# halismai/bpvo

Measured on AMD Instinct MI355X. Metric: GN iterations/s (1241x376 bit-planes 8ch, 4 levels, Tukey; linearise + solve + update = 1, the reference's _num_fun_evals), higher is better.
Workload: dtype f32 (+f64 projection/interpolation); 1 GPU; batch of 1024 independent 1241x376 stereo pairs (1024 per GPU), bitplanes descriptor, 4 pyramid levels, tukey loss, converge with AlgorithmParameters() tolerances; pairs_per_gpu=1024

## Files before the change

bpvo_amd/csrc/context.hip:

```cpp
#include "host_ctx.h"

using namespace bpvo_hip;
using namespace bpvo_hip_host;

namespace bpvo_hip_host {

std::atomic<int> g_live_ctx[64];
thread_local std::string g_create_error;

int fail(bpvo_hip_ctx* c, int code, const char* msg)
{
  c->err = msg;
  return code;
}


void gaussian_kernel5(double sigma, float k[3])
{
  float kk[5];
  const double sigmaX = sigma > 0 ? sigma : ((5 - 1) * 0.5 - 1) * 0.3 + 0.8;
  const double scale2X = -0.5 / (sigmaX * sigmaX);
  double sum = 0;
  for(int i = 0; i < 5; ++i) {
    const double x = i - 2.0;
    kk[i] = (float) std::exp(scale2X * x * x);
    sum += kk[i];
  }
  sum = 1. / sum;
  for(int i = 0; i < 5; ++i) kk[i] = (float) (kk[i] * sum);
  k[0] = kk[2]; k[1] = kk[3]; k[2] = kk[4];
}

void gaussian_taps(int n, double sigma, GaussTaps* g)
{
  *g = GaussTaps();
  if(!(sigma > 0) || n <= 0 || n > kMaxGaussTaps) return;
  g->n = n;
  const double scale2X = -0.5 / (sigma * sigma);
  double sum = 0;
  for(int i = 0; i < n; ++i) {
    const double x = i - (n - 1) * 0.5;
    g->k[i] = (float) std::exp(scale2X * x * x);
    sum += g->k[i];
  }
  sum = 1. / sum;
  for(int i = 0; i < n; ++i) {
    g->k[i] = (float) (g->k[i] * sum);
    g->ki[i] = (int) std::nearbyint((double) g->k[i] * 256.0);
  }
}
int imsmooth_taps(float sigma) { return std::max(5, 2 * (int) std::round((double) sigma) + 1); }
int auto_gauss_taps_f32(float sigma) { return ((int) std::nearbyint((double) sigma * 8.0 + 1.0)) | 1; }

void carve_frame_data(bpvo_hip_ctx* c, FrameSlot& f, unsigned char* base, size_t* total)
{
  Carver cv{base};
  for(int l = 0; l < c->L; ++l) f.img[l] = cv.take<uint8_t>(c->geom[l].npix);
  f.disp = cv.take<float>(c->geom[0].npix);
  for(int l = 0; l < c->L; ++l) f.desc[l] = cv.take<float>(c->geom[l].npix * c->C);
  for(int l = 0; l < c->L; ++l) f.cen[l] = (c->C == 8) ? cv.take<uint8_t>(c->geom[l].npix) : nullptr;
  for(int l = 0; l < c->L; ++l) f.ch0[l] = (c->C == 8) ? cv.take<float>(c->geom[l].npix) : nullptr;
  f.scratch = c->plane_scratch ? cv.take<float>((size_t) c->scratch_planes * c->geom[0].npix) : nullptr;
  if(total) *total = cv.off;
}

void carve_frame_tmpl(bpvo_hip_ctx* c, FrameSlot& f, unsigned char* base, size_t* total)
{
  Carver cv{base};
  for(int l = 0; l < c->L; ++l) {
    const LevelGeom& g = c->geom[l];
    f.sal[l] = cv.take<float>(g.npix);
    const size_t nwords = (size_t) g.rows * ((g.cols + 63) / 64);
    f.flag[l] = (uint8_t*) cv.take<unsigned long long>((std::max(g.npix, nwords * 8) + 7) / 8);
    f.blk_count[l] = cv.take<int>(std::max((size_t) g.nblk, nwords));
    f.pts[l] = cv.take<float4>(g.cap);
    f.ptc[l] = cv.take<float2>(g.cap);
    f.inds[l] = cv.take<int>(g.cap);
    f.pix[l] = cv.take<float>((size_t) g.cap * c->C);
    f.grad[l] = cv.take<float>((size_t) g.cap * c->C * 2);
  }
  f.nrm = cv.take<float>(4 * kMaxLevels);
  f.n_dev = cv.take<int>(kMaxLevels);
  if(total) *total = cv.off;
}

int ensure_template_storage(bpvo_hip_ctx* c, FrameSlot& f)
{
  if(f.tmpl_slab) return BPVO_OK;
  size_t total = 0;
  FrameSlot tmp;
  carve_frame_tmpl(c, tmp, nullptr, &total);
  HIP_CK(c, hipMalloc(&f.tmpl_slab, total));
  HIP_CK(c, hipMemsetAsync(f.tmpl_slab, 0, total, c->stream));
  carve_frame_tmpl(c, f, (unsigned char*) f.tmpl_slab, nullptr);
  return BPVO_OK;
}

FrameJob make_frame_job(bpvo_hip_ctx* c, FrameSlot& f, int l)
{
  const LevelGeom& g = slot_geom(c, f, l);
  FrameJob j;
  std::memset(&j, 0, sizeof(j));
  j.img = f.img[l];
  j.cen = f.cen[l];
  j.ch0 = f.ch0_valid ? f.ch0[l] : nullptr;
  j.scratch = f.scratch;
  j.desc = f.desc[l];
  j.sal = f.sal[l];
  j.flag = f.flag[l];
  j.words = reinterpret_cast<unsigned long long*>(f.flag[l]);
  j.blk_count = f.blk_count[l];
  j.n_out = f.n_dev ? f.n_dev + l : nullptr;
  j.disp = f.disp;
  j.pts = f.pts[l];
  j.ptc = f.ptc[l];
  j.inds = f.inds[l];
  j.pix = f.pix[l];
  j.grad = f.grad[l];
  j.nrm = f.nrm ? f.nrm + 4 * l : nullptr;
  j.rows = g.rows; j.cols = g.cols; j.level = l; j.disp_cols = slot_geom(c, f, 0).cols;
  j.cap = g.cap;
  j.nms_radius = g.nms_radius;
  std::memcpy(j.K, g.K, sizeof(j.K));
  j.b = g.b;
  j.dspace = c->dspace;
  j.lazy = f.lazy[l] ? 1 : 0;
  const bpvo_hip_params& sp = f.seq_params ? *f.seq_params : c->params;
  j.min_saliency = sp.minSaliency; j.min_disp = sp.minValidDisparity; j.max_disp = sp.maxValidDisparity;
  return j;
}

PairJob make_pair_job(bpvo_hip_ctx* c, int ws, int ref, int cur, int l)
{
  FrameSlot& fr = c->frames[ref];
  FrameSlot& fc = c->frames[cur];
  const LevelGeom& g = slot_geom(c, fr, l);
  PairJob j;
  std::memset(&j, 0, sizeof(j));
  j.pts = fr.pts[l];
  j.ptc = fr.ptc[l];
  j.pix = fr.pix[l];
  j.grad = fr.grad[l];
  j.nrm = fr.nrm + 4 * l;
  j.n = fr.n_host[l];
  j.desc = fc.desc[l];
  j.rows = g.rows; j.cols = g.cols;
  std::memcpy(j.K, g.K, sizeof(j.K));
  j.b = g.b;
  j.f_inv[0] = 1.0f / g.K[0]; j.f_inv[1] = 1.0f / g.K[4];
  j.dspace = c->dspace;
  j.r = c->ws[ws].r;
  j.valid = c->ws[ws].valid;
  j.cand = c->ws[ws].cand;
  j.tapkey = c->ws[ws].tapkey;
  j.tapcache_on = c->ws[ws].tapkey != nullptr;
  j.tapcache = c->ws[ws].tapcache;
  j.med_blk = c->ws[ws].med_blk;
  j.partials = c->ws[ws].partials;
  j.st = c->d_states + ws;
  j.cnt = c->d_counters + kWsCounters * (size_t) ws;
  j.ticket = c->d_tickets + ws;
  if(ws == c->trace_ws) { j.trace = c->d_trace; j.trace_cap = c->trace_cap; }
  j.pitch = c->C;
  j.n_groups = c->G;
  j.med_tot = (int) med_totals_at(c);
  pair_job_set_params(j, c->params);
  return j;
}
void pair_job_set_params(PairJob& j, const bpvo_hip_params& p)
{
  j.prm = GNParams{p.maxIterations, kMaxFunEvals, p.parameterTolerance, p.functionTolerance, p.gradientTolerance};
  j.loss = p.lossFunction;
  j.good_thr = p.goodPointThreshold;
}

PairJob group_pair_job(const bpvo_hip_ctx* c, const PairJob& whole, int k)
{
  PairJob j = whole;
  const size_t off = (size_t) k * c->Cg;
  const size_t nblk = (size_t) ((whole.n + kChunkPoints - 1) / kChunkPoints);
  const size_t ntiles = (size_t) std::max(1, (whole.n + gn_pts_per_block(c->Cg) - 1) / gn_pts_per_block(c->Cg));
  j.desc = whole.desc.get() + off;
  j.pix = whole.pix.get() + off;
  j.grad = whole.grad.get() + off;
  j.r = whole.r.get() + off;
  j.cand = whole.cand.get() + (size_t) k * nblk * kChunkPoints * c->Cg;
  j.med_blk = whole.med_blk.get() + (size_t) k * nblk * 4;
  j.partials = whole.partials.get() + (size_t) k * ntiles * kPartialStride;
  j.n_groups = 1;
  return j;
}

hipEvent_t take_event(Lane* ln)
{
  if(!ln->ev_pool.empty()) {
    hipEvent_t e = ln->ev_pool.back();
    ln->ev_pool.pop_back();
    return e;
  }
  hipEvent_t e;
  (void) hipEventCreate(&e);
  return e;
}
void resolve_events(bpvo_hip_ctx* c)
{
  for(auto& ln : c->lanes) {
    for(auto& ep : ln.ev_pending) {
      float ms = 0.0f;
      if(hipEventElapsedTime(&ms, ep.a, ep.b) == hipSuccess) {
        c->kc_ms[ep.kc] += ms;
        c->kc_units[ep.kc] += ep.units;
        c->kc_launches[ep.kc] += 1;
      }
      ln.ev_pool.push_back(ep.a);
      ln.ev_pool.push_back(ep.b);
    }
    ln.ev_pending.clear();
  }
}

int lanes_for(bpvo_hip_ctx* c, int n, int cap)
{
  if(g_live_ctx[c->device & 63].load() > 1) return 1;
  const int want = std::max(1, std::min(std::min(c->max_lanes_now, cap), n / kMinPairsPerLane));
  if(want > (int) c->lanes.size()) {
    const int rc = ensure_lanes(c, want);
    if(rc) return rc;
  }
  return want;
}
int ensure_lanes(bpvo_hip_ctx* c, int n)
{
  const int n_pairs = c->n_pairs;
  while((int) c->lanes.size() < n) {
    c->lanes.emplace_back();
    Lane& ln = c->lanes.back();
    const bool first = c->lanes.size() == 1;
    if(first) { ln.stream = c->stream; ln.owns_stream = false; }
    else { HIP_CK(c, hipStreamCreateWithFlags(&ln.stream, hipStreamNonBlocking)); ln.owns_stream = true; }
    HIP_CK(c, hipMalloc((void**) &ln.d_pjobs, sizeof(PairJob) * (size_t) c->L * n_pairs * job_tables(c)));
    HIP_CK(c, hipMalloc((void**) &ln.d_Tinit, sizeof(float) * 16 * n_pairs));
    HIP_CK(c, hipMalloc((void**) &ln.d_active, 8 * sizeof(int)));
    HIP_CK(c, hipMalloc((void**) &ln.d_list, 3 * sizeof(int) * (size_t) n_pairs));
    for(auto& e : ln.round_ev) HIP_CK(c, hipEventCreateWithFlags(&e, hipEventDisableTiming));
    HIP_CK(c, hipEventCreateWithFlags(&ln.selected_ev, hipEventDisableTiming));
    for(auto& e : ln.staging_ev) HIP_CK(c, hipEventCreateWithFlags(&e, hipEventDisableTiming));
    HIP_CK(c, hipHostMalloc((void**) &ln.h_pjobs, sizeof(PairJob) * std::max((size_t) c->L * n_pairs * job_tables(c), (size_t) (1 + kMaxGroups))));
    HIP_CK(c, hipHostMalloc((void**) &ln.h_T, sizeof(float) * 16 * n_pairs));
    HIP_CK(c, hipHostMalloc((void**) &ln.h_active, 8 * sizeof(int)));
    HIP_CK(c, hipMalloc((void**) &ln.d_pk_ctl, sizeof(unsigned) * kPkCtlWords * kMaxLevels));
    HIP_CK(c, hipHostMalloc((void**) &ln.h_pk_ctl, sizeof(unsigned) * kPkCtlWords * kMaxLevels));
    if(first) {
      HIP_CK(c, hipMalloc((void**) &ln.d_team_ctl, sizeof(unsigned) * (size_t) gn_team_ctl_words(kMaxTeams)));
      HIP_CK(c, hipHostMalloc((void**) &ln.h_team_ctl, sizeof(unsigned) * 64));
      std::memset(ln.h_team_ctl, 0, sizeof(unsigned) * 64);
    }
    HIP_CK(c, hipHostMalloc((void**) &ln.h_states, sizeof(GNState) * (n_pairs + n_pairs)));
  }
  return BPVO_OK;
}

const std::vector<OptionDef>& option_table()
{
#define OPT_INT(key_, field_, lo_, hi_) OptionDef{key_, lo_, hi_, [](bpvo_hip_ctx* c) { return (double) c->field_; }, \
                                                  [](bpvo_hip_ctx* c, double v) { c->field_ = (decltype(c->field_)) v; return BPVO_OK; }}
  static const std::vector<OptionDef> t = {
    OptionDef{"lanes", 1, 8, [](bpvo_hip_ctx* c) { return (double) std::max(1, std::min(c->max_lanes_now, std::max(1, c->n_pairs / kMinPairsPerLane))); },
              [](bpvo_hip_ctx* c, double v) {
                const int n = std::max(1, std::min((int) v, std::max(1, c->n_pairs / kMinPairsPerLane)));
                const int rc = ensure_lanes(c, n);
                if(rc == BPVO_OK) c->max_lanes_now = (int) v;
                return rc;
              }},
    OptionDef{"persistent", 0, 1, [](bpvo_hip_ctx* c) { return (double) c->persistent; },
              [](bpvo_hip_ctx* c, double v) { c->persistent = (int) v; if(c->persistent) c->persistent_failed.store(false); return BPVO_OK; }},
    OPT_INT("persist_max_ws", persist_max_ws, 1, kPersistMaxWs),
    OPT_INT("persist_grid", persist_grid, 1, 128),
    OPT_INT("persist_max_points", persist_max_points, 0, 1 << 30),
    OPT_INT("dense_candidates_from", dense_candidates_from, 0, 1 << 30),
    OPT_INT("persist_timeout_ticks", persist_timeout, 1, 1e15),
    OPT_INT("team", team_mode, 0, 1),
    OPT_INT("team_max_pairs", team_max_pairs, 0, 1 << 20),
    OPT_INT("team_full_pairs", team_full_pairs, 0, 1 << 20),
    OPT_INT("team_size", team_size_env, 0, 256),
    OptionDef{"team_cus", 1, 1 << 16, [](bpvo_hip_ctx* c) { return (double) c->num_cus; },
              [](bpvo_hip_ctx* c, double v) {
                if(c->device_cus > 0 && (int) v > c->device_cus) { c->err = "option team_cus: more CUs than the device has"; return BPVO_ERR_INVALID_ARG; }
                c->num_cus = (int) v;
                return BPVO_OK;
              }},
    OPT_INT("team_local_barriers", team_local_barriers, 0, 1),
    OPT_INT("team_join", team_join, 0, 2),
    OptionDef{"team_joins_seen", 0, 0, [](bpvo_hip_ctx* c) { return (double) c->team_joins.load(); },
              [](bpvo_hip_ctx* c, double) { c->team_joins.store(0); return BPVO_OK; }},
    OPT_INT("team_join_from_pairs", team_join_from_pairs, 0, 1 << 20),
    OPT_INT("team_spares", team_spares, 0, 1),
    OPT_INT("vo_disparity_late", vo_disparity_late, 0, 1),
    OPT_INT("stereo_frames_per_launch", stereo_frames_per_launch, 0, 65535),
    OptionDef{"stereo_frames_per_launch_seen", 0, 0, [](bpvo_hip_ctx* c) { return (double) c->st_frames_per_launch_seen; }, [](bpvo_hip_ctx*, double) { return BPVO_OK; }},
    OptionDef{"stereo_free_mib_seen", 0, 0, [](bpvo_hip_ctx* c) { return (double) (c->st_free_seen >> 20); }, [](bpvo_hip_ctx*, double) { return BPVO_OK; }},
    OPT_INT("normalization_side_stream", nrm_side_stream, 0, 1),
    OPT_INT("normalization_form", nrm_dpp_asm, 0, 4),
    OPT_INT("small_batch_fused", small_batch_fused, 0, 1),
    OPT_INT("levels_in_one_launch_max_frames", merge_levels_max_frames, 0, 1 << 20),
    OPT_INT("normalization_deferred", nrm_defer, 0, 1),
    OPT_INT("team_split_max_pairs", team_split_max_pairs, 0, 1 << 20),
    OPT_INT("fuse_frozen", fuse_frozen, 0, 1),
    OPT_INT("reference_reduction", reference_reduction, 0, 1),
    OPT_INT("step_in_reduce_max_pairs", step_in_reduce_max, 0, 1 << 20),
    OPT_INT("stagger", stagger, 0, 1),
    OPT_INT("stagger_min_pairs", stagger_min_pairs, 0, 1 << 20),
    OPT_INT("upload_workers", up_workers, 0, 32),
    OPT_INT("keep_current_disparity", keep_current_disparity, 0, 1),
    OptionDef{"pose_covariance", 0, 1, [](bpvo_hip_ctx* c) { return (double) c->pose_covariance; },
              [](bpvo_hip_ctx* c, double v) -> int {
                if((int) v) {
                  const int rc = pose_cov_ensure_scratch(c);
                  if(rc) return rc;
                }
                c->pose_covariance = (int) v;
                return BPVO_OK;
              }},
    OPT_INT("lazy_template_descriptor", lazy_template, 0, 1),
    OPT_INT("points_from_compact_stream", points_from_compact, 0, 1),
    OptionDef{"tapcache_max_density", 0.0, 1e9, [](bpvo_hip_ctx* c) { return c->tapcache_max_density; },
              [](bpvo_hip_ctx* c, double v) { c->tapcache_max_density = v; return BPVO_OK; }},
    OptionDef{"upload_plan_first", 0.0, 0.9, [](bpvo_hip_ctx* c) { return c->up_plan[0]; },
              [](bpvo_hip_ctx* c, double v) { if(v + c->up_plan[1] >= 1.0) return BPVO_ERR_INVALID_ARG; c->up_plan[0] = v; return BPVO_OK; }},
    OptionDef{"upload_plan_second", 0.01, 0.99, [](bpvo_hip_ctx* c) { return c->up_plan[1]; },
              [](bpvo_hip_ctx* c, double v) { if(v + c->up_plan[0] >= 1.0) return BPVO_ERR_INVALID_ARG; c->up_plan[1] = v; return BPVO_OK; }},
  };
#undef OPT_INT
  return t;
}
int set_option(bpvo_hip_ctx* c, const std::string& key, double v)
{
  for(const OptionDef& o : option_table())
    if(key == o.key) {
      if(!(v >= o.lo && v <= o.hi)) { c->err = "option " + key + ": value out of range"; return BPVO_ERR_INVALID_ARG; }
      const int rc = o.set(c, v);
      if(rc == BPVO_ERR_INVALID_ARG) c->err = "option " + key + ": invalid value";
      return rc;
    }
  c->err = "unknown option: " + key;
  return BPVO_ERR_INVALID_ARG;
}
int apply_options_string(bpvo_hip_ctx* c, const char* str)
{
  std::string s(str);
  size_t i = 0;
  while(i < s.size()) {
    size_t j = s.find(',', i);
    if(j == std::string::npos) j = s.size();
    const std::string kv = s.substr(i, j - i);
    i = j + 1;
    if(kv.empty()) continue;
    const size_t eq = kv.find('=');
    if(eq == std::string::npos) { c->err = "expected key=value: " + kv; return BPVO_ERR_INVALID_ARG; }
    char* end = nullptr;
    const double v = std::strtod(kv.c_str() + eq + 1, &end);
    if(end == kv.c_str() + eq + 1) { c->err = "not a number: " + kv; return BPVO_ERR_INVALID_ARG; }
    const int rc = set_option(c, kv.substr(0, eq), v);
    if(rc) return rc;
  }
  return BPVO_OK;
}

}

extern "C" {

void bpvo_hip_default_params(bpvo_hip_params* p)
{
  p->numPyramidLevels = -1;
  p->minImageDimensionForPyramid = 40;
  p->sigmaPriorToCensusTransform = -1.0f;
  p->sigmaBitPlanes = 0.5f;
  p->dfSigma1 = 0.75f;
  p->dfSigma2 = 1.75f;
  p->latchNumBytes = 1;
  p->latchRotationInvariance = 0;
  p->latchHalfSsdSize = 1;
  p->centralDifferenceRadius = 3;
  p->centralDifferenceSigmaBefore = 0.75f;
  p->centralDifferenceSigmaAfter = 1.75f;
  p->laplacianKernelSize = 1;
  p->maxIterations = 50;
  p->parameterTolerance = 1e-7f;
  p->functionTolerance = 1e-6f;
  p->gradientTolerance = 1e-8f;
  p->relaxTolerancesForCoarseLevels = 1;
  p->gradientEstimation = BPVO_GRAD_CD3;
  p->interp = BPVO_INTERP_LINEAR;
  p->lossFunction = BPVO_LOSS_TUKEY;
  p->descriptor = BPVO_DESC_INTENSITY;
  p->verbosity = BPVO_VERB_ITERATION;
  p->minTranslationMagToKeyFrame = 0.15f;
  p->minRotationMagToKeyFrame = 5.0f;
  p->maxFractionOfGoodPointsToKeyFrame = 0.6f;
  p->goodPointThreshold = 0.85f;
  p->minNumPixelsForNonMaximaSuppression = 320 * 240;
  p->nonMaxSuppRadius = 1;
  p->minNumPixelsToWork = 256;
  p->minSaliency = 0.1f;
  p->minValidDisparity = 0.001f;
  p->maxValidDisparity = 512.0f;
  p->maxTestLevel = 0;
  p->withNormalization = 1;
}

}

namespace bpvo_hip_host {

const char* level_geometry(const float K[9], float baseline, int rows, int cols, int L, const bpvo_hip_params& p, LevelGeom* geom)
{
  int r = rows, w = cols;
  float Kp[9];
  std::memcpy(Kp, K, sizeof(Kp));
  float bp = baseline;
  for(int l = 0; l < L; ++l) {
    if(l > 0) {
      r = (r + 1) / 2; w = (w + 1) / 2;
      for(int k = 0; k < 9; ++k) Kp[k] *= 0.5f;
      Kp[8] = 1.0f;
      bp *= 2.0f;
    }
    LevelGeom& g = geom[l];
    g.rows = r; g.cols = w; g.npix = (size_t) r * w;
    g.nblk = (int) ((g.npix + 255) / 256);
    const bool nms = (r * w >= p.minNumPixelsForNonMaximaSuppression) && p.nonMaxSuppRadius > 0;
    g.nms_radius = nms ? p.nonMaxSuppRadius : -1;
    const size_t cap = nms ? (size_t) ((r + 1) / 2) * ((w + 1) / 2) : g.npix;
    g.cap = (int) ((cap + kTile - 1) / kTile * kTile);
    std::memcpy(g.K, Kp, sizeof(Kp));
    g.b = bp;
    if(r < 8 || w < 8) return "pyramid level smaller than 8 pixels";
  }
  return nullptr;
}

int create_impl(bpvo_hip_ctx** out, const float K[9], float baseline, int rows, int cols, const bpvo_hip_params* p, int device, int n_frames, int n_pairs,
                const int* min_caps)
{
  if(!out || !K || !p || rows < 8 || cols < 8 || n_frames < 1 || n_pairs < 1) {
    g_create_error = "invalid argument";
    return BPVO_ERR_INVALID_ARG;
  }
  if(rows > 65535 || cols > 65535 || (long long) rows * cols * 8 > 0x7fffffffLL) {
    g_create_error = "image too large (at most 65535 x 65535 and 2^28 pixels)";
    return BPVO_ERR_INVALID_ARG;
  }
  int ndev = 0;
  if(hipGetDeviceCount(&ndev) != hipSuccess || ndev <= 0) {
    g_create_error = "no HIP device: libbpvo_hip has no CPU fallback";
    return BPVO_ERR_NO_DEVICE;
  }
  if(device < 0 || device >= ndev) {
    g_create_error = "bad device ordinal";
    return BPVO_ERR_INVALID_ARG;
  }
  std::unique_ptr<bpvo_hip_ctx> c(new bpvo_hip_ctx);
  pose_cov_none(&c->vo_cov);
  c->params = *p;
  std::memcpy(c->K, K, sizeof(c->K));
  c->baseline = baseline;
  c->rows = rows; c->cols = cols; c->device = device;
  c->n_frames = n_frames; c->n_pairs = n_pairs;
  c->auto_levels = c->params.numPyramidLevels <= 0;
  if(c->params.numPyramidLevels <= 0)
    c->params.numPyramidLevels = auto_pyramid_levels(rows, cols, p->minImageDimensionForPyramid);
  c->L = c->params.numPyramidLevels;
  auto unsupported = [&](const char* m) { g_create_error = m; return BPVO_ERR_UNSUPPORTED; };
  if(c->L < 1 || c->L > kMaxLevels) return unsupported("numPyramidLevels out of range (1..8)");
  if(c->params.maxTestLevel < 0 || c->params.maxTestLevel >= c->L) { g_create_error = "invalid maxTestLevel"; return BPVO_ERR_INVALID_ARG; }
  const bool desc_fields = c->params.descriptor == BPVO_DESC_FIELDS_FIRST_ORDER || c->params.descriptor == BPVO_DESC_FIELDS_SECOND_ORDER;
// ... 278 lines not shown
```

bpvo_amd/csrc/frame_common.h:

```cpp
#pragma once
#include "kernels.h"

namespace bpvo_hip {

__device__ __forceinline__ int reflect101(int p, int len)
{
  if(p < 0) p = -p;
  if(p >= len) p = 2 * len - 2 - p;
  if(p < 0) p = 0;
  return p;
}

__device__ __forceinline__ int reflect101_wide(int p, int len)
{
  if(len == 1) return 0;
  while(p < 0 || p >= len) p = p < 0 ? -p : 2 * len - 2 - p;
  return p;
}

static inline dim3 grid2d(int W, int R, int nz) { return dim3((W + 63) / 64, (R + 3) / 4, nz); }

}
```

bpvo_amd/csrc/frames.hip:

```cpp
#include "host_ctx.h"

using namespace bpvo_hip;
using namespace bpvo_hip_host;

namespace bpvo_hip_host {

FrameRun ctx_run(bpvo_hip_ctx* c) { return FrameRun{c->stream, &c->lanes[0], 0, false, nullptr, nullptr}; }

int upload_frame_jobs_slots(bpvo_hip_ctx* c, const int* slots, int count, const FrameRun& fr, int which, const FrameJob** tab)
{
  const size_t table = (size_t) which * c->L * c->n_frames;
  FR_CK(c, fr, hipEventSynchronize(fr.ln->staging_ev[which]));
  for(int l = 0; l < c->L; ++l) {
    FrameJob* row = c->h_fjobs + table + (size_t) l * c->n_frames + fr.tab;
    for(int i = 0; i < count; ++i) row[i] = make_frame_job(c, c->frames[slots[i]], l);
  }
  const size_t pitch = sizeof(FrameJob) * (size_t) c->n_frames;
  static_assert(sizeof(FrameJob) % 8 == 0 && sizeof(PairJob) % 8 == 0, "copy_rows_kernel moves 8-byte words");
  if(c->ctl_by_kernel.load() || count <= 512)
    launch_copy_rows(fr.stream, c->d_fjobs + table + fr.tab, c->h_fjobs + table + fr.tab, pitch, sizeof(FrameJob) * (size_t) count, c->L);
  else
    FR_CK(c, fr, hipMemcpy2DAsync(c->d_fjobs + table + fr.tab, pitch, c->h_fjobs + table + fr.tab, pitch, sizeof(FrameJob) * (size_t) count, (size_t) c->L,
                                  hipMemcpyHostToDevice, fr.stream));
  FR_CK(c, fr, hipEventRecord(fr.ln->staging_ev[which], fr.stream));
  *tab = c->d_fjobs + table + fr.tab;
  return BPVO_OK;
}
std::vector<int> strided_slots(int first, int stride, int count)
{
  std::vector<int> v((size_t) std::max(count, 0));
  for(int i = 0; i < count; ++i) v[i] = first + i * stride;
  return v;
}
int upload_frame_jobs(bpvo_hip_ctx* c, int first, int stride, int count, const FrameRun& fr, int which, const FrameJob** tab)
{
  const std::vector<int> slots = strided_slots(first, stride, count);
  return upload_frame_jobs_slots(c, slots.data(), count, fr, which, tab);
}

int frames_set_data_slots(bpvo_hip_ctx* c, const int* slots, int count, const uint8_t* images, const float* disps, bool on_device,
                          const FrameRun& fr, int skip_odd_disp, const size_t* offsets)
{
  if(count <= 0) return BPVO_OK;
  const LevelGeom* geom = c->frames[slots[0]].own_geom ? c->frames[slots[0]].geom : c->geom;
  for(int i = 1; i < count; ++i)
    if(slot_geom(c, c->frames[slots[i]], 0).rows != geom[0].rows || slot_geom(c, c->frames[slots[i]], 0).cols != geom[0].cols)
      return fail(c, BPVO_ERR_INVALID_ARG, "frame stage over slots of different sizes");
  const size_t npix = geom[0].npix;
  hipStream_t s = fr.stream;
  if(!on_device) {
    for(int i = 0; i < count; ++i) {
      FrameSlot& f = c->frames[slots[i]];
      const size_t at = offsets ? offsets[i] : (size_t) i * npix;
      FR_CK(c, fr, hipMemcpyAsync(f.img[0], images + at, npix, hipMemcpyHostToDevice, s));
      if(!(skip_odd_disp && (i & 1)) && !fr.skip_disparity_upload)
        FR_CK(c, fr, hipMemcpyAsync(f.disp, disps + at, npix * sizeof(float), hipMemcpyHostToDevice, s));
    }
  }
  for(int i = 0; i < count; ++i) c->frames[slots[i]].ch0_valid = !(skip_odd_disp && (i & 1));
  const bool lazy_ok = skip_odd_disp != 0 && c->lazy_template && c->params.descriptor == BPVO_DESC_BITPLANES && c->C == 8 &&
                       !(c->params.sigmaPriorToCensusTransform > 0.0f) && c->params.sigmaBitPlanes > 0.0f && c->params.gradientEstimation == BPVO_GRAD_CD3;
  for(int i = 0; i < count; ++i)
    for(int l = 0; l < c->L; ++l) c->frames[slots[i]].lazy[l] = lazy_ok && !(i & 1) && geom[l].nms_radius > 0;
  const FrameJob* tab = nullptr;
  int rc = upload_frame_jobs_slots(c, slots, count, fr, 0, &tab);
  if(rc) return rc;
  const int NF = c->n_frames;
  if(on_device && offsets) {
    size_t* h_off = c->h_seq_off + fr.tab;
    for(int i = 0; i < count; ++i) h_off[i] = offsets[i];
    FR_CK(c, fr, hipMemcpyAsync(c->d_seq_off + fr.tab, h_off, sizeof(size_t) * (size_t) count, hipMemcpyHostToDevice, s));
    launch_ingest_at(s, tab, images, disps, c->d_seq_off + fr.tab, npix, count);
  } else if(on_device) {
    launch_ingest(s, tab, images, disps, npix, count, skip_odd_disp);
  }
  {
    double px = 0;
    for(int l = 1; l < c->L; ++l) px += (double) geom[l].npix * count;
    ScopedTimer t(c, KC_PYRAMID, px, fr.ln);
    bool grouped = count <= c->merge_levels_max_frames;
    for(int l = 0; l < c->L; ++l) grouped = grouped && geom[l].cols >= 8 && geom[l].rows >= 8;
    for(int l = 1; l < c->L;) {
      const int steps = grouped ? std::min(3, c->L - l) : 0;
      if(steps >= 2) {
        launch_pyramid_levels(s, tab + (size_t) (l - 1) * NF, NF, steps, geom[l + steps - 1].cols, geom[l + steps - 1].rows, count);
        l += steps;
      } else {
        launch_pyrdown(s, tab + (size_t) (l - 1) * NF, tab + (size_t) l * NF, geom[l].cols, geom[l].rows, count);
        l += 1;
      }
    }
  }
  {
    double px = 0;
    for(int l = c->L - 1; l >= c->params.maxTestLevel; --l) px += (double) geom[l].npix * count;
    ScopedTimer t(c, KC_DESCRIPTOR, px, fr.ln);
    const bool fused_bp = c->C == 8 && c->params.descriptor == BPVO_DESC_BITPLANES && !(c->params.sigmaPriorToCensusTransform > 0.0f) && c->params.sigmaBitPlanes > 0.0f;
    const int l_lo = c->params.maxTestLevel;
    const bool smoothed_bp = c->C == 8 && c->params.descriptor == BPVO_DESC_BITPLANES && c->params.sigmaPriorToCensusTransform > 0.0f && c->params.sigmaBitPlanes > 0.0f;
    const bool plain_intensity = c->C == 1 && c->params.descriptor != BPVO_DESC_LAPLACIAN;
    const bool one_launch = (fused_bp || smoothed_bp || plain_intensity) && count <= c->merge_levels_max_frames && c->L - l_lo > 1;
    if(one_launch && fused_bp) {
      launch_bitplanes(s, tab + (size_t) l_lo * NF, geom[l_lo].cols, geom[l_lo].rows, count, c->params.sigmaBitPlanes, c->gauss_k, 1, c->L - l_lo, NF);
    } else if(one_launch && smoothed_bp) {
      launch_census(s, tab + (size_t) l_lo * NF, geom[l_lo].cols, geom[l_lo].rows, count, c->census_taps, c->L - l_lo, NF);
      launch_bitplanes(s, tab + (size_t) l_lo * NF, geom[l_lo].cols, geom[l_lo].rows, count, c->params.sigmaBitPlanes, c->gauss_k, 0, c->L - l_lo, NF);
    } else if(one_launch) {
      launch_intensity(s, tab + (size_t) l_lo * NF, geom[l_lo].cols, geom[l_lo].rows, count, c->L - l_lo, NF);
    }
    for(int l = c->L - 1; l >= c->params.maxTestLevel && !one_launch; --l) {
      const FrameJob* jobs = tab + (size_t) l * NF;
      const LevelGeom& g = geom[l];
      if(c->params.descriptor == BPVO_DESC_CENTRAL_DIFFERENCE) {
        launch_central_difference(s, jobs, g.cols, g.rows, count, c->params.centralDifferenceRadius, c->cd_before, c->cd_after);
      } else if(c->params.descriptor == BPVO_DESC_LATCH) {
        launch_latch(s, jobs, g.cols, g.rows, count, c->params.latchNumBytes, c->params.latchHalfSsdSize, c->d_latch_off, c->latch_taps[0], c->latch_taps[1],
                     c->latch_after);
      } else if(c->C == 5 || c->C == 10) {
        launch_descriptor_fields(s, jobs, g.cols, g.rows, count, c->C == 10, c->df_g1, c->df_g2);
      } else if(c->C == 3) {
        launch_gradient_descriptor(s, jobs, g.cols, g.rows, count, c->grad_pre);
      } else if(c->C == 1) {
        if(c->params.descriptor == BPVO_DESC_LAPLACIAN) launch_laplacian(s, jobs, g.cols, g.rows, count, c->params.laplacianKernelSize);
        else launch_intensity(s, jobs, g.cols, g.rows, count);
      } else {
        const bool fused_census = !(c->params.sigmaPriorToCensusTransform > 0.0f) && c->params.sigmaBitPlanes > 0.0f;
        if(!fused_census)
          launch_census(s, jobs, g.cols, g.rows, count, c->params.sigmaPriorToCensusTransform > 0.0f ? c->census_taps : nullptr);
        launch_bitplanes(s, jobs, g.cols, g.rows, count, c->params.sigmaBitPlanes, c->gauss_k, fused_census ? 1 : 0);
      }
    }
  }
  FR_CK(c, fr, hipGetLastError());
  for(int i = 0; i < count; ++i) {
    FrameSlot& f = c->frames[slots[i]];
    f.has_data = true;
    f.has_disp = !(skip_odd_disp && (i & 1));
  }
  return BPVO_OK;
}
int frames_set_data(bpvo_hip_ctx* c, int first, int stride, int count, const uint8_t* images, const float* disps, bool on_device,
                    const FrameRun& fr, int skip_odd_disp)
{
  const std::vector<int> slots = strided_slots(first, stride, count);
  return frames_set_data_slots(c, slots.data(), count, images, disps, on_device, fr, skip_odd_disp);
}
int upload_disparity(bpvo_hip_ctx* c, int slot, const float* disparity)
{
  if(!c->copy_stream) {
    HIP_CK(c, hipStreamCreateWithFlags(&c->copy_stream, hipStreamNonBlocking));
    HIP_CK(c, hipEventCreateWithFlags(&c->copy_ev, hipEventDisableTiming));
  }
  HIP_CK(c, hipMemcpyAsync(c->frames[slot].disp, disparity, slot_geom(c, c->frames[slot], 0).npix * sizeof(float), hipMemcpyHostToDevice, c->copy_stream));
  HIP_CK(c, hipEventRecord(c->copy_ev, c->copy_stream));
  HIP_CK(c, hipStreamWaitEvent(c->stream, c->copy_ev, 0));
  return BPVO_OK;
}
int frames_set_data(bpvo_hip_ctx* c, int first, int stride, int count, const uint8_t* images, const float* disps, bool on_device, int skip_odd_disp)
{
  if(count <= 0) return BPVO_OK;
  if(first < 0 || stride < 1 || first + (count - 1) * stride >= c->n_frames) return fail(c, BPVO_ERR_INVALID_ARG, "bad frame slot range");
  if(!images || !disps) return fail(c, BPVO_ERR_INVALID_ARG, "nullptr image/disparity");
  return frames_set_data(c, first, stride, count, images, disps, on_device, ctx_run(c), skip_odd_disp);
}

int frames_set_template_slots(bpvo_hip_ctx* c, const int* slots, int count, const FrameRun& fr)
{
  if(count <= 0) return BPVO_OK;
  const LevelGeom* geom = c->frames[slots[0]].own_geom ? c->frames[slots[0]].geom : c->geom;
  for(int i = 1; i < count; ++i)
    if(slot_geom(c, c->frames[slots[i]], 0).rows != geom[0].rows || slot_geom(c, c->frames[slots[i]], 0).cols != geom[0].cols)
      return fail(c, BPVO_ERR_INVALID_ARG, "frame stage over slots of different sizes");
  hipStream_t s = fr.stream;
  for(int i = 0; i < count; ++i) {
    FrameSlot& f = c->frames[slots[i]];
    if(f.tmpl_slab) continue;
    size_t total = 0;
    FrameSlot tmp;
    carve_frame_tmpl(c, tmp, nullptr, &total);
    FR_CK(c, fr, hipMalloc(&f.tmpl_slab, total));
    FR_CK(c, fr, hipMemsetAsync(f.tmpl_slab, 0, total, s));
    carve_frame_tmpl(c, f, (unsigned char*) f.tmpl_slab, nullptr);
  }
  const FrameJob* tab = nullptr;
  int rc = upload_frame_jobs_slots(c, slots, count, fr, 1, &tab);
  if(rc) return rc;
  const int NF = c->n_frames;
  int* const h_ints = c->h_ints + (size_t) fr.tab * kMaxLevels;
  int* const d_ints = c->d_ints + (size_t) fr.tab * kMaxLevels;
  const bpvo_hip_params& p = c->params;
  const int border = std::max(p.nonMaxSuppRadius, 3);
  bool tiled = true;
  for(int l = p.maxTestLevel; l < c->L; ++l) tiled = tiled && geom[l].nms_radius <= 1;
  const bool one_launch = tiled && count <= c->merge_levels_max_frames && c->L - p.maxTestLevel > 1;
  hipEvent_t counts_ev = fr.ln ? fr.ln->round_ev[0] : nullptr;
  hipStream_t side = nullptr;
  if(c->nrm_side_stream && !fr.own_thread && fr.ln == &c->lanes[0] && counts_ev) {
    if(!c->side_stream) {
      FR_CK(c, fr, hipStreamCreateWithFlags(&c->side_stream, hipStreamNonBlocking));
      FR_CK(c, fr, hipStreamCreateWithFlags(&c->side_stream2, hipStreamNonBlocking));
      for(auto& e : c->side_ev) FR_CK(c, fr, hipEventCreateWithFlags(&e, hipEventDisableTiming));
    }
    side = c->side_stream;
  }
  const int with_nrm = c->dspace ? 0 : p.withNormalization;
  const bool defer = side && fr.defer_finest_nrm && c->nrm_defer && c->L - p.maxTestLevel > 1 && !c->nrm_pending && !c->nrm_pending_finest;
  if(one_launch) {
    double px = 0;
    for(int l = p.maxTestLevel; l < c->L; ++l) px += (double) geom[l].npix * count;
    ScopedTimer t(c, KC_SALIENCY_SELECT, px, fr.ln);
    const LevelGeom& g = geom[p.maxTestLevel];
    launch_saliency_select(s, tab + (size_t) p.maxTestLevel * NF, c->C, g.cols, g.rows, count, 1, border,
                           c->L - p.maxTestLevel, NF);
  }
  for(int l = c->L - 1; l >= p.maxTestLevel && !one_launch; --l) {
    const FrameJob* jobs = tab + (size_t) l * NF;
    const LevelGeom& g = geom[l];
    ScopedTimer t(c, KC_SALIENCY_SELECT, (double) g.npix * count, fr.ln);
    launch_saliency_select(s, jobs, c->C, g.cols, g.rows, count, g.nms_radius, border);
  }
  if(side) {
    FR_CK(c, fr, hipEventRecord(c->side_ev[0], s));
    FR_CK(c, fr, hipStreamWaitEvent(side, c->side_ev[0], 0));
    if(defer && templates_may_be_dense(c)) {
      hipStream_t side2 = c->side_stream2;
      FR_CK(c, fr, hipStreamWaitEvent(side2, c->side_ev[0], 0));
      { ScopedTimer t(c, KC_NORMALIZATION, 0.0, fr.ln, true, side2); launch_normalization(side2, tab, NF, count, p.maxTestLevel, p.maxTestLevel + 1, with_nrm, c->nrm_dpp_asm); }
      FR_CK(c, fr, hipEventRecord(c->side_ev[3], side2));
      c->nrm_pending_finest = c->side_ev[3];
      { ScopedTimer t(c, KC_NORMALIZATION, 0.0, fr.ln, true, side); launch_normalization(side, tab, NF, count, c->L - 1, c->L, with_nrm, c->nrm_dpp_asm); }
      FR_CK(c, fr, hipEventRecord(c->side_ev[1], side));
      if(c->L - 1 > p.maxTestLevel + 1) {
        { ScopedTimer t(c, KC_NORMALIZATION, 0.0, fr.ln, true, side); launch_normalization(side, tab, NF, count, p.maxTestLevel + 1, c->L - 1, with_nrm, c->nrm_dpp_asm); }
        FR_CK(c, fr, hipEventRecord(c->side_ev[2], side));
        c->nrm_pending = c->side_ev[2];
      }
    } else if(defer) {
      { ScopedTimer t(c, KC_NORMALIZATION, 0.0, fr.ln, true, side); launch_normalization(side, tab, NF, count, c->L - 1, c->L, with_nrm, c->nrm_dpp_asm); }
      FR_CK(c, fr, hipEventRecord(c->side_ev[1], side));
      { ScopedTimer t(c, KC_NORMALIZATION, 0.0, fr.ln, true, side); launch_normalization(side, tab, NF, count, p.maxTestLevel, c->L - 1, with_nrm, c->nrm_dpp_asm); }
      FR_CK(c, fr, hipEventRecord(c->side_ev[2], side));
      c->nrm_pending = c->side_ev[2];
    } else {
      { ScopedTimer t(c, KC_NORMALIZATION, 0.0, fr.ln, true, side); launch_normalization(side, tab, NF, count, p.maxTestLevel, c->L, with_nrm, c->nrm_dpp_asm); }
      FR_CK(c, fr, hipEventRecord(c->side_ev[1], side));
    }
  }
  launch_gather_counts(s, tab, NF, count, p.maxTestLevel, c->L, d_ints);
  FR_CK(c, fr, hipMemcpyAsync(h_ints, d_ints, sizeof(int) * kMaxLevels * (size_t) count, hipMemcpyDeviceToHost, s));
  if(counts_ev) FR_CK(c, fr, hipEventRecord(counts_ev, s));
  if(fr.selected_ev) FR_CK(c, fr, hipEventRecord(fr.selected_ev, s));
  if(fr.on_selected) fr.on_selected();
  if(!side) {
    ScopedTimer t(c, KC_NORMALIZATION, 0.0, fr.ln);
    launch_normalization(s, tab, NF, count, p.maxTestLevel, c->L, with_nrm, c->nrm_dpp_asm);
  }
  if(counts_ev) FR_CK(c, fr, hipEventSynchronize(counts_ev));
  else FR_CK(c, fr, hipStreamSynchronize(s));
  std::vector<int> max_n(c->L, 0);
  double pts = 0;
  for(int i = 0; i < count; ++i) {
    FrameSlot& f = c->frames[slots[i]];
    for(int l = 0; l < c->L; ++l) {
      f.n_host[l] = (l >= p.maxTestLevel) ? h_ints[(size_t) i * kMaxLevels + l] : 0;
      max_n[l] = std::max(max_n[l], f.n_host[l]);
      pts += f.n_host[l];
    }
  }
  if(c->profiling) {
    std::lock_guard<std::mutex> lk(c->units_mu);
    c->kc_units[KC_TEMPLATE] += pts;
    c->kc_units[KC_NORMALIZATION] += pts;
  }
  if(count <= c->merge_levels_max_frames && c->L - p.maxTestLevel > 1) {
    ScopedTimer t(c, KC_TEMPLATE, 0.0, fr.ln);
    int most = 0;
    for(int l = p.maxTestLevel; l < c->L; ++l) most = std::max(most, max_n[l]);
    launch_template_build(s, tab + (size_t) p.maxTestLevel * NF, c->C, most, count, p.gradientEstimation == BPVO_GRAD_CD5, c->gauss_k, c->L - p.maxTestLevel, NF);
  } else {
    for(int l = c->L - 1; l >= p.maxTestLevel; --l) {
      ScopedTimer t(c, KC_TEMPLATE, 0.0, fr.ln);
      launch_template_build(s, tab + (size_t) l * NF, c->C, max_n[l], count, p.gradientEstimation == BPVO_GRAD_CD5, c->gauss_k);
    }
  }
  if(side) FR_CK(c, fr, hipStreamWaitEvent(s, c->side_ev[1], 0));
  if(!fr.own_thread && !fr.no_final_sync) {
    FR_CK(c, fr, hipStreamSynchronize(s));
    FR_CK(c, fr, hipGetLastError());
    resolve_events(c);
  }
  for(int i = 0; i < count; ++i) c->frames[slots[i]].has_template = true;
  return BPVO_OK;
}
int frames_set_template(bpvo_hip_ctx* c, int first, int stride, int count, const FrameRun& fr)
{
  const std::vector<int> slots = strided_slots(first, stride, count);
  return frames_set_template_slots(c, slots.data(), count, fr);
}
int frames_set_template(bpvo_hip_ctx* c, int first, int stride, int count)
{
  if(count <= 0) return BPVO_OK;
  if(first < 0 || stride < 1 || first + (count - 1) * stride >= c->n_frames) return fail(c, BPVO_ERR_INVALID_ARG, "bad frame slot range");
  for(int i = 0; i < count; ++i) {
    if(!c->frames[first + i * stride].has_data) return fail(c, BPVO_ERR_NO_DATA, "no data in frame");
    if(!c->frames[first + i * stride].has_disp) return fail(c, BPVO_ERR_NO_DATA, "no disparity in frame (the current frame of a pair batch)");
  }
  return frames_set_template(c, first, stride, count, ctx_run(c));
}

int ensure_dense_descriptor(bpvo_hip_ctx* c, int slot)
{
  FrameSlot& f = c->frames[slot];
  bool any = false;
  for(int l = 0; l < c->L; ++l) any = any || f.lazy[l];
  if(!any) return BPVO_OK;
  bool was[kMaxLevels];
  for(int l = 0; l < c->L; ++l) { was[l] = f.lazy[l]; f.lazy[l] = false; }
  auto restore = [&]() { for(int l = 0; l < c->L; ++l) f.lazy[l] = was[l]; };
  const FrameRun fr = ctx_run(c);
  const FrameJob* tab = nullptr;
  const int rc = upload_frame_jobs(c, slot, 1, 1, fr, 0, &tab);
  if(rc) { restore(); return rc; }
  for(int l = c->L - 1; l >= c->params.maxTestLevel; --l)
    launch_bitplanes(c->stream, tab + (size_t) l * c->n_frames, c->geom[l].cols, c->geom[l].rows, 1, c->params.sigmaBitPlanes, c->gauss_k, 1);
  if(hipGetLastError() != hipSuccess || hipStreamSynchronize(c->stream) != hipSuccess) {
    restore();
    return fail(c, BPVO_ERR_DEVICE, "ensure_dense_descriptor: descriptor kernels failed");
  }
  return BPVO_OK;
}

}

extern "C" {

int bpvo_hip_frame_set_data(bpvo_hip_ctx* c, int slot, const uint8_t* image, const float* disparity)
{
  CHECK_CTX(c); CHECK_SLOT(c, slot);
  (void) hipSetDevice(c->device);
  int rc = frames_set_data(c, slot, 1, 1, image, disparity, false);
  if(rc) return rc;
  HIP_CK(c, hipStreamSynchronize(c->stream));
  resolve_events(c);
  return BPVO_OK;
}
int bpvo_hip_frame_set_data_device(bpvo_hip_ctx* c, int slot, const uint8_t* d_image, const float* d_disparity)
{
  CHECK_CTX(c); CHECK_SLOT(c, slot);
  (void) hipSetDevice(c->device);
  int rc = frames_set_data(c, slot, 1, 1, d_image, d_disparity, true);
  if(rc) return rc;
  HIP_CK(c, hipStreamSynchronize(c->stream));
  resolve_events(c);
  return BPVO_OK;
}
int bpvo_hip_frames_set_data(bpvo_hip_ctx* c, int first_slot, int slot_stride, int count, const uint8_t* images,
                             const float* disparities, int on_device)
{
  CHECK_CTX(c);
  (void) hipSetDevice(c->device);
  int rc = frames_set_data(c, first_slot, slot_stride, count, images, disparities, on_device != 0);
  if(rc) return rc;
  HIP_CK(c, hipStreamSynchronize(c->stream));
  resolve_events(c);
  return BPVO_OK;
}
int bpvo_hip_frame_set_template(bpvo_hip_ctx* c, int slot)
{
  CHECK_CTX(c); CHECK_SLOT(c, slot);
  (void) hipSetDevice(c->device);
  return frames_set_template(c, slot, 1, 1);
}
int bpvo_hip_frames_set_template(bpvo_hip_ctx* c, int first_slot, int slot_stride, int count)
{
  CHECK_CTX(c);
  (void) hipSetDevice(c->device);
  return frames_set_template(c, first_slot, slot_stride, count);
}
int bpvo_hip_frame_clear(bpvo_hip_ctx* c, int slot)
{
  CHECK_CTX(c); CHECK_SLOT(c, slot);
  c->frames[slot].has_data = false;
  c->frames[slot].has_template = false;
  return BPVO_OK;
}
int bpvo_hip_frame_state(const bpvo_hip_ctx* c, int slot, int* has_data, int* has_template)
{
  if(!c || slot < 0 || slot >= c->n_frames) return BPVO_ERR_INVALID_ARG;
  *has_data = c->frames[slot].has_data;
  *has_template = c->frames[slot].has_template;
  return BPVO_OK;
}

int bpvo_hip_get_image(bpvo_hip_ctx* c, int slot, int level, uint8_t* out)
{
  CHECK_CTX(c); CHECK_SLOT(c, slot);
  if(level < 0 || level >= c->L) return fail(c, BPVO_ERR_INVALID_ARG, "bad level");
  if(!c->frames[slot].has_data) return fail(c, BPVO_ERR_NO_DATA, "no data in frame");
  (void) hipSetDevice(c->device);
  HIP_CK(c, hipMemcpyAsync(out, c->frames[slot].img[level], c->geom[level].npix, hipMemcpyDeviceToHost, c->stream));
  HIP_CK(c, hipStreamSynchronize(c->stream));
  return BPVO_OK;
}
int bpvo_hip_get_descriptor_channel(bpvo_hip_ctx* c, int slot, int level, int channel, float* out)
{
  CHECK_CTX(c); CHECK_SLOT(c, slot); CHECK_LEVEL(c, level);
  if(channel < 0 || channel >= c->C) return fail(c, BPVO_ERR_INVALID_ARG, "bad channel");
  if(!c->frames[slot].has_data) return fail(c, BPVO_ERR_NO_DATA, "no data in frame");
  (void) hipSetDevice(c->device);
  if(int rc = ensure_dense_descriptor(c, slot)) return rc;
  const size_t npix = c->geom[level].npix;
  HIP_CK(c, hipMemcpy2DAsync(out, sizeof(float), c->frames[slot].desc[level] + channel, sizeof(float) * c->C, sizeof(float), npix,
                             hipMemcpyDeviceToHost, c->stream));
  HIP_CK(c, hipStreamSynchronize(c->stream));
  return BPVO_OK;
}
int bpvo_hip_get_saliency(bpvo_hip_ctx* c, int slot, int level, float* out)
{
  CHECK_CTX(c); CHECK_SLOT(c, slot); CHECK_LEVEL(c, level);
  if(!c->frames[slot].has_template) return fail(c, BPVO_ERR_NO_TEMPLATE, "no template");
  (void) hipSetDevice(c->device);
  HIP_CK(c, hipMemcpyAsync(out, c->frames[slot].sal[level], c->geom[level].npix * sizeof(float), hipMemcpyDeviceToHost, c->stream));
  HIP_CK(c, hipStreamSynchronize(c->stream));
  return BPVO_OK;
}
#define TMPL(c, slot, level)                                                                    \
  CHECK_CTX(c); CHECK_SLOT(c, slot); CHECK_LEVEL(c, level);                                     \
  if(!(c)->frames[slot].has_template) return fail(c, BPVO_ERR_NO_TEMPLATE, "no template");      \
  (void) hipSetDevice((c)->device);                                                             \
  FrameSlot& f = (c)->frames[slot];                                                             \
  const int n = f.n_host[level]

int bpvo_hip_num_points(bpvo_hip_ctx* c, int slot, int level, int* n_out) { TMPL(c, slot, level); *n_out = n; return BPVO_OK; }
int bpvo_hip_get_points(bpvo_hip_ctx* c, int slot, int level, float* xyzw)
{
  TMPL(c, slot, level);
  if(n && c->points_from_compact) {
    float4* d_out = nullptr;
    HIP_CK(c, hipMalloc((void**) &d_out, sizeof(float4) * n));
    launch_rebuild_points(c->stream, make_pair_job(c, 0, slot, slot, level), d_out);
    hipError_t e = hipMemcpyAsync(xyzw, d_out, sizeof(float4) * n, hipMemcpyDeviceToHost, c->stream);
    if(e == hipSuccess) e = hipStreamSynchronize(c->stream);
    (void) hipFree(d_out);
    HIP_CK(c, e);
    return BPVO_OK;
  }
  if(n) HIP_CK(c, hipMemcpyAsync(xyzw, f.pts[level], sizeof(float4) * n, hipMemcpyDeviceToHost, c->stream));
  HIP_CK(c, hipStreamSynchronize(c->stream));
  return BPVO_OK;
}
int bpvo_hip_get_point_indices(bpvo_hip_ctx* c, int slot, int level, int* inds)
{
  TMPL(c, slot, level);
  if(n) HIP_CK(c, hipMemcpyAsync(inds, f.inds[level], sizeof(int) * n, hipMemcpyDeviceToHost, c->stream));
  HIP_CK(c, hipStreamSynchronize(c->stream));
  return BPVO_OK;
}
int bpvo_hip_get_pixels(bpvo_hip_ctx* c, int slot, int level, float* pixels)
{
  TMPL(c, slot, level);
  const int C = c->C;
  std::vector<float> t(tiled_floats(n, C));
  if(n) HIP_CK(c, hipMemcpyAsync(t.data(), f.pix[level], t.size() * sizeof(float), hipMemcpyDeviceToHost, c->stream));
  HIP_CK(c, hipStreamSynchronize(c->stream));
  detile_to_channel_major(t.data(), n, C, 1, C == 8 ? 4 : C, pixels);
  return BPVO_OK;
}
int bpvo_hip_get_jacobians(bpvo_hip_ctx* c, int slot, int level, float* J)
{
  TMPL(c, slot, level);
  if(n == 0) return BPVO_OK;
  const size_t bytes = sizeof(float) * 6 * (size_t) n * c->C;
  float* d_out = nullptr;
  HIP_CK(c, hipMalloc((void**) &d_out, bytes));
  HIP_CK(c, hipStreamSynchronize(c->stream));
  c->h_fjobs[0] = make_frame_job(c, f, level);
  hipError_t e = hipMemcpyAsync(c->d_fjobs, c->h_fjobs, sizeof(FrameJob), hipMemcpyHostToDevice, c->stream);
  if(e == hipSuccess) {
    launch_export_jacobians(c->stream, c->d_fjobs, c->C, n, d_out);
    e = hipMemcpyAsync(J, d_out, bytes, hipMemcpyDeviceToHost, c->stream);
  }
  if(e == hipSuccess) e = hipStreamSynchronize(c->stream);
  (void) hipFree(d_out);
  HIP_CK(c, e);
  return BPVO_OK;
}
int bpvo_hip_get_normalization(bpvo_hip_ctx* c, int slot, int level, float T[16], float T_inv[16])
{
  TMPL(c, slot, level);
  M44 t = m44_identity(), ti = m44_identity();
  if(!c->params.withNormalization || c->dspace || n == 0) {
    std::memcpy(T, t.m, 64);
    std::memcpy(T_inv, ti.m, 64);
    return BPVO_OK;
  }
  float nrm[4];
  HIP_CK(c, hipMemcpyAsync(nrm, f.nrm + 4 * level, sizeof(nrm), hipMemcpyDeviceToHost, c->stream));
  HIP_CK(c, hipStreamSynchronize(c->stream));
  t.m[0] = t.m[5] = t.m[10] = nrm[0];
  t.m[3] = -nrm[0] * nrm[1]; t.m[7] = -nrm[0] * nrm[2]; t.m[11] = -nrm[0] * nrm[3];
  ti.m[0] = ti.m[5] = ti.m[10] = 1.0f / nrm[0];
  ti.m[3] = nrm[1]; ti.m[7] = nrm[2]; ti.m[11] = nrm[3];
  std::memcpy(T, t.m, 64);
  std::memcpy(T_inv, ti.m, 64);
  return BPVO_OK;
}

}
```

bpvo_amd/csrc/host_ctx.h:

```cpp
#pragma once
#include <hip/hip_runtime.h>

#include <algorithm>
#include <atomic>
#include <chrono>
#include <cmath>
#include <cstdio>
#include <cstdlib>
#include <cstring>
#include <functional>
#include <condition_variable>
#include <memory>
#include <mutex>
#include <string>
#include <thread>
#include <vector>

#include "kernels.h"
#include "latch_table.h"
#include "rig_math.h"
#include "vo_state.h"

using namespace bpvo_hip;
#include "latch_table.h"

namespace bpvo_hip_host {

using namespace bpvo_hip;


extern std::atomic<int> g_live_ctx[64];
extern thread_local std::string g_create_error;

struct LevelGeom {
  int rows, cols;
  size_t npix;
  int nblk;
  int cap;
  int nms_radius;
  float K[9];
  float b;
};

struct FrameSlot {
  bool has_data = false, has_template = false;
  bool has_disp = false;
  void* data_slab = nullptr;
  void* tmpl_slab = nullptr;
  uint8_t* img[kMaxLevels] = {};
  uint8_t* cen[kMaxLevels] = {};
  float* ch0[kMaxLevels] = {};
  bool lazy[kMaxLevels] = {};
  bool ch0_valid = true;
  float* desc[kMaxLevels] = {};
  float* disp = nullptr;
  float* scratch = nullptr;
  float* sal[kMaxLevels] = {};
  uint8_t* flag[kMaxLevels] = {};
  int* blk_count[kMaxLevels] = {};
  float4* pts[kMaxLevels] = {};
  float2* ptc[kMaxLevels] = {};
  int* inds[kMaxLevels] = {};
  float* pix[kMaxLevels] = {};
  float* grad[kMaxLevels] = {};
  float* nrm = nullptr;
  int* n_dev = nullptr;
  int n_host[kMaxLevels] = {};
  bool own_geom = false;
  LevelGeom geom[kMaxLevels];
  const bpvo_hip_params* seq_params = nullptr;
};

struct Workspace {
  float* r = nullptr;
  uint8_t* valid = nullptr;
  uint32_t* cand = nullptr;
  uint32_t* med_blk = nullptr;
  uint32_t* tapkey = nullptr;
  float* tapcache = nullptr;
  float* partials = nullptr;
  int last_ref = -1, last_cur = -1, last_level = -1;
  bool has_estimate = false;
};

struct CovScratch {
  int group = 0;
  void* d_slab = nullptr;
  float* d_r = nullptr; size_t r_floats = 0;
  uint8_t* d_valid = nullptr; size_t valid_bytes = 0;
  float* d_partials = nullptr; size_t partial_floats = 0;
  unsigned long long* d_cnt = nullptr;
  GNState* d_states = nullptr;
  unsigned char* d_tables = nullptr;
  unsigned char* h_tables = nullptr;
  size_t tables_bytes = 0, off_members = 0, off_T = 0, off_sigma = 0, off_X = 0;
  bpvo_hip_pose_covariance* d_out = nullptr;
  bpvo_hip_pose_covariance* h_out = nullptr;
  float* d_sums = nullptr;
};

enum KernelClass { KC_PYRAMID = 0, KC_DESCRIPTOR, KC_SALIENCY_SELECT, KC_NORMALIZATION, KC_TEMPLATE, KC_WARP_RESIDUAL, KC_MEDIAN,
                   KC_IRLS_REDUCE, KC_GN_STEP, KC_COUNT };
static const char* const kKernelNames[KC_COUNT] = {"pyramid", "descriptor", "saliency_select", "normalization", "template_build", "warp_residual",
                                      "median", "irls_reduce", "gn_step"};

struct EventPair { hipEvent_t a, b; int kc; double units; };

struct Lane {
  hipStream_t stream = nullptr;
  bool owns_stream = false;
  PairJob* h_pjobs = nullptr;
  PairJob* d_pjobs = nullptr;
  float* h_T = nullptr;
  float* d_Tinit = nullptr;
  int* d_active = nullptr;
  int* d_list = nullptr;
  int* h_active = nullptr;
  hipEvent_t round_ev[3] = {};
  hipEvent_t staging_ev[2] = {};
  hipEvent_t selected_ev = nullptr;
  unsigned* d_pk_ctl = nullptr;
  unsigned* h_pk_ctl = nullptr;
  unsigned* d_team_ctl = nullptr;
  unsigned* h_team_ctl = nullptr;
  GNState* h_states = nullptr;
  std::vector<EventPair> ev_pending;
  std::vector<hipEvent_t> ev_pool;
  unsigned k6_seq = 0;
  std::string err;
};
constexpr int kDefaultLanes = 3;
constexpr int kDefaultLanesNarrow = 2;
constexpr int kMinPairsPerLane = 8;
constexpr int kPkCtlWords = 32;
constexpr int kMaxTeams = 1024;
constexpr int kMaxFunEvals = 6 * 200;

}

using namespace bpvo_hip;
using namespace bpvo_hip_host;

struct bpvo_hip_ctx {

  bpvo_hip_params params;
  float K[9];
  float baseline;
  int rows, cols, L, C, device;
  bool auto_levels = false;
  int n_frames, n_pairs;
  LevelGeom geom[kMaxLevels];
  float gauss_k[3];
  GaussTaps df_g1, df_g2;
  GaussTaps cd_before, cd_after;
  GaussTaps grad_pre;
  GaussTaps latch_after;
  int latch_taps[2] = {0, 0};
  signed char* d_latch_off = nullptr;
  int scratch_planes = kDfPlanes;
  bool plane_scratch = false;
  hipStream_t stream = nullptr;
  std::vector<FrameSlot> frames;
  std::vector<Workspace> ws;
  GNState* d_states = nullptr;
  FrameJob* d_fjobs = nullptr;
  std::vector<Lane> lanes;
  PairJob* d_job1 = nullptr;
  float* d_records = nullptr;
  float* d_wtmp = nullptr;
  unsigned int* d_count = nullptr;
  unsigned* d_tickets = nullptr;
  unsigned long long* d_counters = nullptr;
  FrameJob* h_fjobs = nullptr;
  int* h_ints = nullptr;
  int* d_ints = nullptr;
  int cap_max = 0;
  SeqState vo;
  bpvo_hip_point_with_info* d_cloud = nullptr;
  size_t d_cloud_cap = 0;
  int vo_mode = 0;
  std::vector<SeqState> seqs;
  bpvo_hip_point_with_info* d_seq_cloud = nullptr;
  PairJob* h_seq_jobs = nullptr;
  PairJob* d_seq_jobs = nullptr;
  CloudJob* h_cloud_jobs = nullptr;
  CloudJob* d_cloud_jobs = nullptr;
  unsigned* h_seq_cnt = nullptr;
  unsigned* d_seq_cnt = nullptr;
  size_t* h_seq_off = nullptr;
  size_t* d_seq_off = nullptr;
  std::vector<RigState> rigs;
  float* d_rig_X = nullptr;
  char* d_rig_stage = nullptr; char* h_rig_stage = nullptr;
  int* d_rig_active = nullptr; int* h_rig_active = nullptr;
  int pose_covariance = 0;
  CovScratch cov;
  bpvo_hip_pose_covariance vo_cov;
  std::vector<bpvo_hip_pose_covariance> seq_cov;
  double points_fused = 0;
  int fast_warp = 0;
  int dspace = 0;
  int fuse_frozen = 1;
  int G = 1, Cg = 0;
  int reference_reduction = 0;
  int step_in_reduce_max = 128;
  int persistent = 1, persist_max_ws = 1, persist_grid = 64;
  int persist_max_points = 32768;
  int dense_candidates_from = 32768;
  long long persist_timeout = 50000000ll;
  int team_mode = 1, team_max_pairs = 128, team_full_pairs = 80, team_size_env = 0, num_cus = 0, device_cus = 0;
  int team_join = 2;
  int merge_levels_max_frames = 8;
  int small_batch_fused = 1;
  int nrm_dpp_asm = 4;
  int nrm_side_stream = 1;
  int nrm_defer = 1;
  int team_split_max_pairs = 4;
  hipStream_t side_stream = nullptr, side_stream2 = nullptr;
  hipStream_t copy_stream = nullptr;
  hipEvent_t copy_ev = nullptr;
  std::function<int()> before_final_sync;
  int vo_disparity_late = 1;
  hipEvent_t side_ev[4] = {nullptr, nullptr, nullptr, nullptr};
  hipEvent_t nrm_pending = nullptr;
  hipEvent_t nrm_pending_finest = nullptr;
  int team_spares = 1;
  int team_join_from_pairs = 48;
  int team_local_barriers = 1;
  std::atomic<uint64_t> team_launches{0};
  std::atomic<uint64_t> team_joins{0};
  std::atomic<bool> persistent_failed{false};
  std::atomic<uint64_t> persistent_levels{0};
  float* d_trace = nullptr;
  int trace_cap = 0, trace_ws = -1;
  int max_lanes_now = 1 << 30;
  uint8_t* st_left = nullptr; uint8_t* st_right = nullptr; uint8_t* st_left_pre = nullptr; uint8_t* st_right_pre = nullptr;
  float* st_disp = nullptr;
  size_t st_pixels = 0;
  void* st_sgm = nullptr;
  size_t st_sgm_bytes = 0;
  StereoFrame* h_st_frames = nullptr; StereoFrame* d_st_frames = nullptr;
  int st_tab_cap = 0;
  hipEvent_t st_tab_ev = nullptr;
  int stereo_frames_per_launch = 0;
  size_t st_sgm_budget = 0, st_free_seen = 0;
  int st_frames_per_launch_seen = 0;
  int up_workers = 6;
  std::atomic<bool> ctl_by_kernel{false};
  std::vector<hipStream_t> up_streams;
  std::vector<uint8_t*> up_pinned;
  std::vector<hipEvent_t> up_slot_free;
  std::vector<hipEvent_t> up_chunk_done;
  size_t up_slot_bytes = 0;
  uint8_t* up_d_img = nullptr;
  float* up_d_disp = nullptr;
  int up_cap_pairs = 0;
  double up_plan[2] = {0.19, 0.50};
  int points_from_compact = 0;
  int lazy_template = 1;
  int keep_current_disparity = 0;
  double up_last_seconds = 0.0;
  size_t up_last_bytes = 0;
  bool counted_live = false;
  float prefetch_frac_thr = -1.0f;
  bool frac_valid = false; int frac_ws = -1; float frac_thr = 0.0f; unsigned frac_cnt = 0; int frac_n = 0;
  double tapcache_max_density = 0.5;
  bool stagger = true;
  int stagger_min_pairs = 192;
  int census_taps[2] = {0, 0};
  bool profiling = false;
  bool profile_all = false;
  bool profile_k6_all = false;
  double kc_ms[KC_COUNT] = {};
  double kc_units[KC_COUNT] = {};
  uint64_t kc_launches[KC_COUNT] = {};
  uint64_t total_lin = 0, median_bracketed = 0, median_full = 0;
  uint64_t tap_counts[4] = {};
  std::mutex units_mu;
  std::string err;
};

namespace bpvo_hip_host {

#define HIP_CK(ctx_, expr)                                                                  \
  do {                                                                                      \
    hipError_t e_ = (expr);                                                                 \
    if(e_ != hipSuccess) {                                                                  \
      (ctx_)->err = std::string(#expr) + ": " + hipGetErrorString(e_);                      \
      return BPVO_ERR_DEVICE;                                                               \
    }                                                                                       \
  } while(0)

#define LANE_CK(ln_, expr)                                                                  \
  do {                                                                                      \
    hipError_t e_ = (expr);                                                                 \
    if(e_ != hipSuccess) {                                                                  \
      (ln_)->err = std::string(#expr) + ": " + hipGetErrorString(e_);                       \
      (void) hipStreamSynchronize((ln_)->stream);                                           \
      return BPVO_ERR_DEVICE;                                                               \
    }                                                                                       \
  } while(0)

inline size_t align_up(size_t v, size_t a = 256) { return (v + a - 1) / a * a; }
inline int auto_pyramid_levels(int rows, int cols, int minImageDimensionForPyramid)
{
  return 1 + (int) std::round(std::log2(std::min(rows, cols) / (double) minImageDimensionForPyramid));
}

struct Carver {
  unsigned char* base;
  size_t off = 0;
  template <typename T>
  T* take(size_t count)
  {
    T* p = base ? reinterpret_cast<T*>(base + off) : nullptr;
    off += align_up(count * sizeof(T));
    return p;
  }
};

hipEvent_t take_event(Lane* ln);
struct ScopedTimer {
  Lane* ln;
  EventPair ep;
  bool on;
  hipStream_t st;
  ScopedTimer(bpvo_hip_ctx* c_, int kc, double units, Lane* lane = nullptr, bool sampled = true, hipStream_t stream = nullptr)
      : ln(lane ? lane : &c_->lanes[0]), on(c_->profiling && sampled), st(stream ? stream : (lane ? lane : &c_->lanes[0])->stream)
  {
    if(!on) return;
    ep.kc = kc; ep.units = units;
    ep.a = take_event(ln); ep.b = take_event(ln);
    (void) hipEventRecord(ep.a, st);
  }
  ~ScopedTimer()
  {
    if(!on) return;
    (void) hipEventRecord(ep.b, st);
    ln->ev_pending.push_back(ep);
  }
};

struct FrameRun {
  hipStream_t stream;
  Lane* ln;
  int tab;
  bool own_thread;
  hipEvent_t selected_ev;
  std::function<void()> on_selected;
  bool defer_finest_nrm = false;
  bool no_final_sync = false;
  bool skip_disparity_upload = false;
};
#define FR_CK(c_, fr_, expr)                                                                \
  do {                                                                                      \
    hipError_t e_ = (expr);                                                                 \
    if(e_ != hipSuccess) {                                                                  \
      ((fr_).own_thread ? (fr_).ln->err : (c_)->err) = std::string(#expr) + ": " + hipGetErrorString(e_); \
      return BPVO_ERR_DEVICE;                                                               \
    }                                                                                       \
  } while(0)

const char* level_geometry(const float K[9], float baseline, int rows, int cols, int L, const bpvo_hip_params& p, LevelGeom* g);
int create_impl(bpvo_hip_ctx** out, const float K[9], float baseline, int rows, int cols, const bpvo_hip_params* p, int device, int n_frames, int n_pairs,
                const int* min_caps);
inline const LevelGeom& slot_geom(const bpvo_hip_ctx* c, const FrameSlot& f, int l) { return f.own_geom ? f.geom[l] : c->geom[l]; }

int fail(bpvo_hip_ctx* c, int code, const char* msg);
void gaussian_kernel5(double sigma, float k[3]);
void gaussian_taps(int n, double sigma, GaussTaps* g);
int imsmooth_taps(float sigma);
int auto_gauss_taps_f32(float sigma);
void carve_frame_data(bpvo_hip_ctx* c, FrameSlot& f, unsigned char* base, size_t* total);
void carve_frame_tmpl(bpvo_hip_ctx* c, FrameSlot& f, unsigned char* base, size_t* total);
int ensure_template_storage(bpvo_hip_ctx* c, FrameSlot& f);
FrameJob make_frame_job(bpvo_hip_ctx* c, FrameSlot& f, int l);
PairJob make_pair_job(bpvo_hip_ctx* c, int ws, int ref, int cur, int l);
void pair_job_set_params(PairJob& j, const bpvo_hip_params& p);
void resolve_events(bpvo_hip_ctx* c);
FrameRun ctx_run(bpvo_hip_ctx* c);
int upload_frame_jobs(bpvo_hip_ctx* c, int first, int stride, int count, const FrameRun& fr, int which, const FrameJob** tab);
std::vector<int> strided_slots(int first, int stride, int count);
int upload_frame_jobs_slots(bpvo_hip_ctx* c, const int* slots, int count, const FrameRun& fr, int which, const FrameJob** tab);
int frames_set_data_slots(bpvo_hip_ctx* c, const int* slots, int count, const uint8_t* images, const float* disps, bool on_device, const FrameRun& fr,
                          int skip_odd_disp = 0, const size_t* offsets = nullptr);
int frames_set_template_slots(bpvo_hip_ctx* c, const int* slots, int count, const FrameRun& fr);
int frames_set_data(bpvo_hip_ctx* c, int first, int stride, int count, const uint8_t* images, const float* disps, bool on_device, const FrameRun& fr,
                    int skip_odd_disp = 0);
int frames_set_data(bpvo_hip_ctx* c, int first, int stride, int count, const uint8_t* images, const float* disps, bool on_device, int skip_odd_disp = 0);
int frames_set_template(bpvo_hip_ctx* c, int first, int stride, int count, const FrameRun& fr);
int upload_disparity(bpvo_hip_ctx* c, int slot, const float* disparity);
int frames_set_template(bpvo_hip_ctx* c, int first, int stride, int count);
bool team_serves(const bpvo_hip_ctx* c, int n);
PairJob group_pair_job(const bpvo_hip_ctx* c, const PairJob& whole, int k);
inline int job_tables(const bpvo_hip_ctx* c) { return c->G > 1 ? 1 + c->G : 1; }
template <class F>
inline void for_each_group(const bpvo_hip_ctx* c, const bpvo_hip::GNLaunch& g, size_t stride, F&& f)
{
  if(c->G <= 1) { f(g); return; }
  for(int k = 0; k < c->G; ++k) {
    bpvo_hip::GNLaunch gg = g;
    gg.jobs = g.jobs + (size_t) (1 + k) * stride;
    gg.C = c->Cg;
    f(gg);
  }
}
inline size_t med_totals_at(const bpvo_hip_ctx* c) { return (((size_t) ((c->cap_max + bpvo_hip::kChunkPoints - 1) / bpvo_hip::kChunkPoints) * (size_t) c->G) + 7) / 8 * 8; }
inline hipError_t join_pending_normalization(bpvo_hip_ctx* c, hipStream_t s)
{
  hipError_t e = hipSuccess;
  if(c->nrm_pending) { e = hipStreamWaitEvent(s, c->nrm_pending, 0); c->nrm_pending = nullptr; }
  if(c->nrm_pending_finest) { const hipError_t e2 = hipStreamWaitEvent(s, c->nrm_pending_finest, 0); c->nrm_pending_finest = nullptr; if(e == hipSuccess) e = e2; }
  return e;
}
inline bool templates_may_be_dense(const bpvo_hip_ctx* c)
{
  for(int l = c->params.maxTestLevel; l < c->L; ++l)
    if(c->geom[l].nms_radius <= 0 && c->geom[l].npix > (size_t) std::max(0, c->persist_max_points)) return true;
  return false;
}
inline bool single_pair_is_queued_at_once(const bpvo_hip_ctx* c)
{
  return c->persistent && !c->persistent_failed.load() && !c->profile_all && !c->reference_reduction && (c->C == 8 || c->C == 1) &&
         c->params.interp == BPVO_INTERP_LINEAR && !c->fast_warp && !templates_may_be_dense(c);
}
inline int dense_candidates(const bpvo_hip_ctx* c, int max_points) { return (c->G == 1 && max_points >= c->dense_candidates_from) ? 1 : 0; }
inline bpvo_hip::GNLaunch median_launch(const bpvo_hip_ctx* c, bpvo_hip::GNLaunch g) { if(c->G > 1) g.C = c->Cg; return g; }
int estimate_group(bpvo_hip_ctx* c, Lane* ln, int n, const int* wss, const int* refs, const int* curs, const float* T_init, float* poses,
                   bpvo_hip_stats* stats, float* d_records_out, bool allow_persistent, const bpvo_hip_params* const* prms = nullptr);
int estimate_batch(bpvo_hip_ctx* c, int n, const int* wss, const int* refs, const int* curs, const float* T_init, float* poses, bpvo_hip_stats* stats,
                   const bpvo_hip_params* const* prms = nullptr);
int estimate_rig(bpvo_hip_ctx* c, int n, const int* wss, const int* refs, const int* curs, const float* X, const float* T_init, float* T_est, bpvo_hip_stats* stats);
struct RigProblem {
  int n;
  const int* wss; const int* refs; const int* curs;
  const float* X;
  const float* T_init;
  float* T_est;
  bpvo_hip_stats* stats;
  const bpvo_hip_params* prm;
};
int estimate_rigs(bpvo_hip_ctx* c, int R, const RigProblem* rigs);
inline size_t rig_stage_X_at(const bpvo_hip_ctx* c) { return (sizeof(bpvo_hip::RigEntry) * (size_t) c->n_pairs + 63) / 64 * 64; }
inline size_t rig_stage_bytes(const bpvo_hip_ctx* c) { return rig_stage_X_at(c) + 2 * sizeof(float) * 16 * (size_t) c->n_pairs; }
void detile_to_channel_major(const float* src, int n, int C, int E, int V, float* out);
size_t tiled_floats(int n, int floats_per_point);
int refresh_counters(bpvo_hip_ctx* c);
int upload_single_job(bpvo_hip_ctx* c, int ws, int ref, int cur, int level);
int ensure_residuals(bpvo_hip_ctx* c, int ws);
int fraction_good(bpvo_hip_ctx* c, int ws, float thr, float* frac);
int get_weights_host(bpvo_hip_ctx* c, int ws, std::vector<float>& w_cm, int* n_out);
int check_template_not_empty(bpvo_hip_ctx* c, int ref_slot);
int ensure_lanes(bpvo_hip_ctx* c, int n);
int lanes_for(bpvo_hip_ctx* c, int n, int cap);
int ensure_dense_descriptor(bpvo_hip_ctx* c, int slot);
int pose_cov_pass(bpvo_hip_ctx* c, int n_records, int members, const int* wss, const int* refs, const int* curs, const float* X, int level,
                  const float* T, const float* sigma, const bpvo_hip_params* const* prms, bpvo_hip_pose_covariance* out);
int pose_cov_ensure_scratch(bpvo_hip_ctx* c);
void pose_cov_none(bpvo_hip_pose_covariance* r);
void pose_cov_free(bpvo_hip_ctx* c);
int set_option(bpvo_hip_ctx* c, const std::string& key, double v);
int apply_options_string(bpvo_hip_ctx* c, const char* str);
struct OptionDef { const char* key; double lo, hi; std::function<double(bpvo_hip_ctx*)> get; std::function<int(bpvo_hip_ctx*, double)> set; };
const std::vector<OptionDef>& option_table();

}

#define CHECK_CTX(c) if(!(c)) return BPVO_ERR_INVALID_ARG
#define CHECK_SLOT(c, s) if((s) < 0 || (s) >= (c)->n_frames) return fail(c, BPVO_ERR_INVALID_ARG, "bad frame slot")
#define CHECK_WS(c, w) if((w) < 0 || (w) >= (c)->n_pairs) return fail(c, BPVO_ERR_INVALID_ARG, "bad workspace")
#define CHECK_LEVEL(c, l) if((l) < (c)->params.maxTestLevel || (l) >= (c)->L) return fail(c, BPVO_ERR_INVALID_ARG, "bad level")
```

bpvo_amd/csrc/kernels.h:

```cpp
#pragma once

#include <hip/hip_runtime.h>

#include "types.h"

#include <type_traits>

template <class F>
static inline void dispatch_channels(int C, F&& f)
{
  switch(C) {
    case 1: f(std::integral_constant<int, 1>()); break;
    case 3: f(std::integral_constant<int, 3>()); break;
    case 5: f(std::integral_constant<int, 5>()); break;
    case 10: f(std::integral_constant<int, 10>()); break;
    case 16: f(std::integral_constant<int, 16>()); break;
    case 32: f(std::integral_constant<int, 32>()); break;
    case 24: f(std::integral_constant<int, 24>()); break;
    case 48: f(std::integral_constant<int, 48>()); break;
    default: f(std::integral_constant<int, 8>()); break;
  }
}

template <class F>
static inline bool dispatch_wide_channels(int C, F&& f)
{
  switch(C) {
    case 64: f(std::integral_constant<int, 64>()); return true;
    case 80: f(std::integral_constant<int, 80>()); return true;
    case 120: f(std::integral_constant<int, 120>()); return true;
    case 128: f(std::integral_constant<int, 128>()); return true;
    case 168: f(std::integral_constant<int, 168>()); return true;
    case 224: f(std::integral_constant<int, 224>()); return true;
    case 256: f(std::integral_constant<int, 256>()); return true;
    case 288: f(std::integral_constant<int, 288>()); return true;
    case 360: f(std::integral_constant<int, 360>()); return true;
    case 512: f(std::integral_constant<int, 512>()); return true;
    default: return false;
  }
}

namespace bpvo_hip {

constexpr int kMaxGaussTaps = 31;
struct GaussTaps { int n = 0; float k[kMaxGaussTaps] = {}; int ki[kMaxGaussTaps] = {}; };

void launch_ingest(hipStream_t s, const FrameJob* jobs_level0, const uint8_t* d_images, const float* d_disps, size_t npix, int nframes, int skip_odd_disp = 0);
void launch_ingest_at(hipStream_t s, const FrameJob* jobs_level0, const uint8_t* d_images, const float* d_disps, const size_t* d_offsets, size_t npix, int nframes);
void launch_pyrdown(hipStream_t s, const FrameJob* src, const FrameJob* dst, int dW, int dR, int nframes);
void launch_pyramid_levels(hipStream_t s, const FrameJob* src_row, int job_pitch, int steps, int dW, int dR, int nframes);
void launch_intensity(hipStream_t s, const FrameJob* jobs, int W, int R, int nframes, int nlevels = 1, int job_pitch = 0);
void launch_gradient_descriptor(hipStream_t s, const FrameJob* jobs, int W, int R, int nframes, const GaussTaps& pre);
void launch_descriptor_fields(hipStream_t s, const FrameJob* jobs, int W, int R, int nframes, int second_order, const GaussTaps& g1,
                              const GaussTaps& g2);
void launch_central_difference(hipStream_t s, const FrameJob* jobs, int W, int R, int nframes, int radius, const GaussTaps& before,
                               const GaussTaps& after);
void launch_latch(hipStream_t s, const FrameJob* jobs, int W, int R, int nframes, int bytes, int half_ssd, const signed char* d_offsets, int kc, int ks,
                  const GaussTaps& after);
void launch_laplacian(hipStream_t s, const FrameJob* jobs, int W, int R, int nframes, int ksize );
void launch_census(hipStream_t s, const FrameJob* jobs, int W, int R, int nframes, const int* blur_taps , int nlevels = 1, int job_pitch = 0);
void launch_bitplanes(hipStream_t s, const FrameJob* jobs, int W, int R, int nframes, float sigma, const float k[3], int from_image, int nlevels = 1,
                      int job_pitch = 0);
void launch_saliency_select(hipStream_t s, const FrameJob* jobs, int C, int W, int R, int nframes, int nms_radius, int border, int nlevels = 1, int job_pitch = 0);
void launch_copy_rows(hipStream_t s, void* dst, const void* src_host_pinned, size_t pitch_bytes, size_t width_bytes, int rows);
void launch_gather_counts(hipStream_t s, const FrameJob* jobs , int job_pitch, int nframes, int first_level, int num_levels,
                          int* out );
void launch_normalization(hipStream_t s, const FrameJob* jobs , int job_pitch, int nframes, int first_level,
                          int num_levels, int with_normalization, int form = 1);
void launch_export_jacobians(hipStream_t s, const FrameJob* job , int C, int n, float* out );
void launch_template_build(hipStream_t s, const FrameJob* jobs, int C, int max_points, int nframes, int grad_cd5, const float gauss_k[3], int nlevels = 1,
                           int job_pitch = 0);

struct StereoFrame { int rows, cols; size_t offset; };
struct StereoLaunch {
  const uint8_t* left_pre;
  const uint8_t* right_pre;
  float* disp;
  int rows, cols, nframes;
  const StereoFrame* frames = nullptr;
  size_t total_pixels = 0;
  int wsz, ndisp, mindisp, cap, texture_threshold, uniqueness_ratio;
};
void launch_stereo_prefilter(hipStream_t s, const uint8_t* src, uint8_t* dst, int rows, int cols, int cap, int nframes);
void launch_stereo_prefilter_frames(hipStream_t s, const uint8_t* src, uint8_t* dst, const StereoFrame* frames , int max_rows, int max_cols,
                                    int cap, int nframes);
bool launch_stereo_bm(hipStream_t s, const StereoLaunch& g);

struct SgmLaunch {
  const uint8_t* left;
  const uint8_t* right;
  float* disp;
  void* scratch;
  int rows, cols, nframes;
  int frames_per_launch = 1;
  int ndisp, sobel_cap, census_radius, window_radius, P1, P2, consistency_threshold;
  double disparity_factor, census_weight;
};
size_t sgm_scratch_bytes(int rows, int cols, int ndisp);
bool launch_stereo_sgm(hipStream_t s, const SgmLaunch& g);
void launch_speckle_filter_u16(hipStream_t s, uint16_t* img, int* lab, int* size, int rows, int cols, int max_diff, int max_size, int nframes = 1,
                               size_t frame_bytes = 0);

struct SgbmLaunch {
  const uint8_t* left; const uint8_t* right;
  float* disp;
  void* scratch;
  int rows, cols, nframes;
  int min_disp, ndisp, sad_window, P1, P2, disp12_max_diff, pre_filter_cap, uniqueness_ratio, speckle_window, speckle_range, full_dp;
};
size_t sgbm_scratch_bytes(int rows, int cols, int min_disp, int ndisp);
bool sgbm_serves(const SgbmLaunch& g, const char** why);
bool launch_stereo_sgbm(hipStream_t s, const SgbmLaunch& g);

constexpr int kDenseRuns = 64;
constexpr int kChunkPoints = 256;
struct ActiveSet {
  const int* list = nullptr;
};

struct GNLaunch {
  const PairJob* jobs;
  int npairs;
  ActiveSet active;
  int max_points;
  int C;
  int loss;
  int interp = 0;
  int fuse_frozen = 0;
  int dense_candidates = 0;
  int fast_warp = 0;
  int step_in_reduce = 0;
  int begin_level = -1, begin_moot = 0;
  const PairJob* next_jobs = nullptr;
  int reference_reduction = 0;
};
int  gn_num_blocks(int max_points);
void launch_set_pose(hipStream_t s, const PairJob* jobs, const float* T_init, int n, unsigned* clear = nullptr, int clear_words = 0);
void launch_level_begin(hipStream_t s, const PairJob* jobs, int npairs, int max_points, int level, int scale_is_moot = 0);
void launch_reset_tapkeys(hipStream_t s, const GNLaunch& g);
void launch_compact_active(hipStream_t s, const PairJob* jobs, ActiveSet in, int n_in, int* out_list, int* out_count);
void launch_warp_residual(hipStream_t s, const GNLaunch& g);
void launch_refresh_residuals(hipStream_t s, const GNLaunch& g);
void launch_median(hipStream_t s, const GNLaunch& g);
void launch_irls_reduce(hipStream_t s, const GNLaunch& g);
void launch_reference_reduce(hipStream_t s, const GNLaunch& g);
void launch_gn_step(hipStream_t s, const GNLaunch& g, int mode);
constexpr int kPersistMaxWs = 8;
bool gn_persistent_serves(const GNLaunch& g);
int  gn_persistent_grid(const GNLaunch& g, int max_grid);
hipError_t launch_gn_persistent(hipStream_t s, const GNLaunch& g, unsigned* ctl, int grid, long long timeout_ticks);
struct GNTeamLaunch {
  const PairJob* jobs_all;
  int job_pitch, n_pairs, level_hi, level_lo;
  int C, loss, fuse_frozen, scale_is_moot;
  int team_size, n_teams;
  unsigned* ctl;
  long long timeout_ticks;
  int local_barriers = 1;
  int spare_workgroups = 0;
  int join_mode = 2;
};
int  gn_team_ctl_words(int n_teams);
void launch_team_ctl_reset_keep_abort(hipStream_t s, unsigned* ctl, int n_teams);
int  gn_team_max_size();
hipError_t launch_gn_team(hipStream_t s, const GNTeamLaunch& t);
struct RigStepArgs {
  const PairJob* jobs;
  int n;
  const float* X;
  GNState* body;
  int mode, level;
  const float* T_init;
  int reference;
};
void launch_rig_step(hipStream_t s, const RigStepArgs& a);
struct RigEntry {
  int first, n;
  const float* X;
  GNState* body;
  const float* T_init;
};
struct RigStepsArgs {
  const PairJob* jobs;
  const RigEntry* rigs;
  int n_rigs;
  int mode, level;
  int with_init;
  int reference;
  int* active_out;
};
void launch_rig_steps(hipStream_t s, const RigStepsArgs& b);
struct CovMember {
  const GNState* src;
  float* sums;
};
struct CovLaunch {
  const PairJob* jobs;
  const CovMember* members_tab;
  int n_records, members;
  const float* T;
  const float* sigma;
  const float* X;
  int level;
  int max_points, C, loss;
  bpvo_hip_pose_covariance* out;
};
int  pose_cov_partials_floats(int cap, int C);
void launch_pose_cov_prepare(hipStream_t s, const CovLaunch& g);
void launch_pose_cov_reduce(hipStream_t s, const CovLaunch& g);
void launch_pose_cov_finish(hipStream_t s, const CovLaunch& g);
void launch_prepare_linearize(hipStream_t s, const PairJob* job, const float* T , int reset_scale, int level, float given_scale = 0.0f);
int  gn_pts_per_block(int C);
int  gn_partials_entries(int cap, int C);
void launch_weights(hipStream_t s, const PairJob* job, int n, int C, int loss, float* w_out );
void launch_count_good(hipStream_t s, const PairJob* job, int n, int C, int loss, float thr, unsigned int* count);
void launch_rebuild_points(hipStream_t s, const PairJob& job, float4* out);
// ... 20 lines not shown
```

bpvo_amd/csrc/kernels_frame.hip:

```cpp
#include <algorithm>
#include <cstdlib>

#include "frame_common.h"

namespace bpvo_hip {

__device__ __forceinline__ const FrameJob& level_job(const FrameJob* jobs, unsigned z, int nframes, int job_pitch)
{
  const unsigned lvl = z / (unsigned) nframes;
  return jobs[(size_t) lvl * job_pitch + (z - lvl * (unsigned) nframes)];
}

template <bool AT>
__global__ __launch_bounds__(256) void ingest_kernel(const FrameJob* jobs, const uint8_t* images, const float* disps, size_t npix, int skip_odd_disp,
                                                     const size_t* __restrict__ offs)
{
  const FrameJob& j = jobs[blockIdx.z];
  const uint8_t* __restrict__ si = images + (AT ? offs[blockIdx.z] : (size_t) blockIdx.z * npix);
  const float* __restrict__ sd = disps + (AT ? offs[blockIdx.z] : (size_t) (skip_odd_disp == 2 ? blockIdx.z / 2 : blockIdx.z) * npix);
  uint8_t* __restrict__ di = const_cast<uint8_t*>(j.img.get());
  float* __restrict__ dd = const_cast<float*>(j.disp.get());
  const size_t t = (size_t) blockIdx.x * 256 + threadIdx.x, stride = (size_t) gridDim.x * 256;
  const bool w4 = (npix % 4 == 0) && (((uintptr_t) si | (uintptr_t) di) % 4 == 0);
  if(w4) {
    const uint32_t* s4 = reinterpret_cast<const uint32_t*>(si);
    uint32_t* d4 = reinterpret_cast<uint32_t*>(di);
    for(size_t k = t; k < npix / 4; k += stride) d4[k] = s4[k];
  } else {
    for(size_t k = t; k < npix; k += stride) di[k] = si[k];
  }
  if(skip_odd_disp && (blockIdx.z & 1)) return;
  const bool f4 = (npix % 4 == 0) && (((uintptr_t) sd | (uintptr_t) dd) % 16 == 0);
  if(f4) {
    const float4* s4 = reinterpret_cast<const float4*>(sd);
    float4* d4 = reinterpret_cast<float4*>(dd);
    for(size_t k = t; k < npix / 4; k += stride) d4[k] = load_stream(s4 + k);
  } else {
    for(size_t k = t; k < npix; k += stride) dd[k] = sd[k];
  }
}

constexpr int PDT_W = 64, PDT_H = 16;
constexpr int PDS_W = 2 * PDT_W + 3, PDS_H = 2 * PDT_H + 3;
constexpr int PDS_DW = (PDS_W + 3 + 3) / 4;
constexpr int PDS_PITCH = 4 * (PDS_DW + 2);
constexpr int PD_STACK = 4;
constexpr int PD_NPRE = (PDS_H * PDS_DW + 255) / 256;
__global__ __launch_bounds__(256) void pyrdown_u8_lds_kernel(const FrameJob* src_jobs, const FrameJob* dst_jobs)
{
  __shared__ __attribute__((aligned(16))) uint8_t s_src[PDS_H][PDS_PITCH];
  __shared__ __attribute__((aligned(8))) uint16_t s_h[PDS_H][PDT_W];
  __shared__ int s_off[PDS_H];
  const FrameJob& sj = src_jobs[blockIdx.z];
  const FrameJob& dj = dst_jobs[blockIdx.z];
  const int sw = sj.cols, sh = sj.rows, dw = dj.cols, dh = dj.rows;
  const int dx0 = blockIdx.x * PDT_W;
  const int lane = threadIdx.x & 63, wave = threadIdx.x >> 6;
  const uint8_t* __restrict__ s = sj.img;
  uint8_t* __restrict__ const d = const_cast<uint8_t*>(dj.img.get());
  const int c_first = 2 * dx0 - 2;
  const bool fast = c_first >= 3 && c_first + PDS_W + 3 <= sw;
  auto row_ptr = [&](int dy0, int r) { return s + (size_t) reflect101(min(2 * dy0 - 2 + r, sh + 1), sh) * sw + c_first; };
  uint32_t pre[PD_NPRE];
  auto prefetch = [&](int dy0) {
#pragma unroll
    for(int k = 0; k < PD_NPRE; ++k) {
      const int i = min((int) threadIdx.x + k * 256, PDS_H * PDS_DW - 1);
      const int r = i / PDS_DW, l = i - r * PDS_DW;
      const uintptr_t a = reinterpret_cast<uintptr_t>(row_ptr(dy0, r));
      const unsigned ll = min((unsigned) l, ((unsigned) (a & 3u) + PDS_W - 1) / 4u);
      pre[k] = *reinterpret_cast<const uint32_t*>(a - (a & 3u) + 4u * ll);
    }
  };
  const int dy_first = blockIdx.y * (PDT_H * PD_STACK);
  if(fast) prefetch(dy_first);
  for(int t = 0; t < PD_STACK; ++t) {
    const int dy0 = dy_first + t * PDT_H;
    if(dy0 >= dh) break;
    if(fast) {
#pragma unroll
      for(int k = 0; k < PD_NPRE; ++k) {
        const int i = (int) threadIdx.x + k * 256;
        if(i < PDS_H * PDS_DW) { const int r = i / PDS_DW, l = i - r * PDS_DW; reinterpret_cast<uint32_t*>(&s_src[r][0])[l] = pre[k]; }
      }
      if(t + 1 < PD_STACK && dy0 + PDT_H < dh) prefetch(dy0 + PDT_H);
    } else {
      for(int r = wave; r < PDS_H; r += 4) {
        const uint8_t* row = s + (size_t) reflect101(min(2 * dy0 - 2 + r, sh + 1), sh) * sw;
#pragma unroll
        for(int c0 = 0; c0 < PDS_W; c0 += 64) {
          const int c = c0 + lane;
          if(c < PDS_W) s_src[r][c] = row[reflect101(min(c_first + c, sw + 1), sw)];
        }
      }
    }
    if(threadIdx.x < PDS_H) s_off[threadIdx.x] = fast ? (int) (reinterpret_cast<uintptr_t>(row_ptr(dy0, threadIdx.x)) & 3u) : 0;
    __syncthreads();
    for(int idx = threadIdx.x; idx < PDS_H * (PDT_W / 4); idx += 256) {
      const int r = idx >> 4, xq = idx & 15;
      const uint2* q = reinterpret_cast<const uint2*>(&s_src[r][8 * xq]);
      const uint2 lo = q[0], hi = q[1];
      const unsigned off = (unsigned) s_off[r];
      const unsigned d0 = __builtin_amdgcn_alignbyte(lo.y, lo.x, off), d1 = __builtin_amdgcn_alignbyte(hi.x, lo.y, off),
                     d2 = __builtin_amdgcn_alignbyte(hi.y, hi.x, off);
      const unsigned kW = 0x04060401u;
      const unsigned h0 = __builtin_amdgcn_udot4(d0, kW, d1 & 0xffu, false);
      const unsigned h1 = __builtin_amdgcn_udot4(__builtin_amdgcn_alignbyte(d1, d0, 2), kW, (d1 >> 16) & 0xffu, false);
      const unsigned h2 = __builtin_amdgcn_udot4(d1, kW, d2 & 0xffu, false);
      const unsigned h3 = __builtin_amdgcn_udot4(__builtin_amdgcn_alignbyte(d2, d1, 2), kW, (d2 >> 16) & 0xffu, false);
      *reinterpret_cast<uint2*>(&s_h[r][4 * xq]) = make_uint2(h0 | (h1 << 16), h2 | (h3 << 16));
    }
    __syncthreads();
    const int ty = threadIdx.x >> 4, xq = threadIdx.x & 15;
    const int y = dy0 + ty, x = dx0 + 4 * xq;
    if(y < dh && x < dw) {
      unsigned v[4];
      uint2 tt[5];
#pragma unroll
      for(int k = 0; k < 5; ++k) tt[k] = *reinterpret_cast<const uint2*>(&s_h[2 * ty + k][4 * xq]);
#pragma unroll
      for(int e = 0; e < 4; ++e) {
        unsigned a[5];
#pragma unroll
        for(int k = 0; k < 5; ++k) { const unsigned w = (e < 2) ? tt[k].x : tt[k].y; a[k] = (e & 1) ? (w >> 16) : (w & 0xffffu); }
        v[e] = (a[0] + 4u * a[1] + 6u * a[2] + 4u * a[3] + a[4] + 128u) >> 8;
      }
      uint8_t* o = d + (size_t) y * dw + x;
      if(x + 3 < dw) {
        typedef uint32_t __attribute__((aligned(1))) u32_unaligned;
        *reinterpret_cast<u32_unaligned*>(o) = v[0] | (v[1] << 8) | (v[2] << 16) | (v[3] << 24);
      } else {
        for(int e = 0; e < 4 && x + e < dw; ++e) o[e] = (uint8_t) v[e];
      }
    }
    __syncthreads();
  }
}

constexpr int PA_T = 8;
constexpr int pa_edge(int steps) { return steps == 0 ? PA_T : 2 * pa_edge(steps - 1) + 3; }
template <int NL>
__global__ __launch_bounds__(256) void pyramid_levels_kernel(const FrameJob* jobs , int job_pitch)
{
  constexpr int E0 = pa_edge(NL), E1 = pa_edge(NL - 1);
  __shared__ uint8_t s_a[E0 * E0];
  __shared__ uint8_t s_b[E1 * E1];
  __shared__ uint16_t s_h[E0 * E1];
  int W[NL + 1], H[NL + 1], xlo[NL + 1], xhi[NL + 1], ylo[NL + 1], yhi[NL + 1];
#pragma unroll
  for(int k = 0; k <= NL; ++k) { const FrameJob& j = jobs[(size_t) k * job_pitch + blockIdx.z]; W[k] = j.cols; H[k] = j.rows; }
  xlo[NL] = blockIdx.x * PA_T; xhi[NL] = min(xlo[NL] + PA_T, W[NL]) - 1;
  ylo[NL] = blockIdx.y * PA_T; yhi[NL] = min(ylo[NL] + PA_T, H[NL]) - 1;
#pragma unroll
  for(int k = NL - 1; k >= 0; --k) {
    xlo[k] = max(0, 2 * xlo[k + 1] - 2); xhi[k] = min(W[k] - 1, 2 * xhi[k + 1] + 2);
    ylo[k] = max(0, 2 * ylo[k + 1] - 2); yhi[k] = min(H[k] - 1, 2 * yhi[k + 1] + 2);
  }
  const int tid = threadIdx.x;
  {
    const uint8_t* __restrict__ src = jobs[blockIdx.z].img;
    const int nx = xhi[0] - xlo[0] + 1, ny = yhi[0] - ylo[0] + 1;
    for(int i = tid; i < nx * ny; i += 256) {
      const int r = i / nx, c = i - r * nx;
      s_a[r * E0 + c] = src[(size_t) (ylo[0] + r) * W[0] + xlo[0] + c];
    }
  }
  __syncthreads();
  uint8_t* cur = s_a;
  uint8_t* nxt = s_b;
  int pc = E0, pn = E1;
#pragma unroll
  for(int k = 0; k < NL; ++k) {
    const int snx = xhi[k] - xlo[k] + 1, sny = yhi[k] - ylo[k] + 1;
    const int dnx = xhi[k + 1] - xlo[k + 1] + 1, dny = yhi[k + 1] - ylo[k + 1] + 1;
    (void) snx;
    for(int i = tid; i < sny * dnx; i += 256) {
      const int r = i / dnx, c = i - r * dnx;
      const int x2 = 2 * (xlo[k + 1] + c);
      const uint8_t* row = cur + r * pc - xlo[k];
      const unsigned a0 = row[reflect101(x2 - 2, W[k])], a1 = row[reflect101(x2 - 1, W[k])], a2 = row[x2], a3 = row[reflect101(x2 + 1, W[k])],
                     a4 = row[reflect101(x2 + 2, W[k])];
      s_h[r * E1 + c] = (uint16_t) (a0 + 4u * a1 + 6u * a2 + 4u * a3 + a4);
    }
    __syncthreads();
    const int sh = NL - (k + 1);
    const int ox0 = (blockIdx.x * PA_T) << sh, ox1 = min(((blockIdx.x + 1) * PA_T) << sh, W[k + 1]);
    const int oy0 = (blockIdx.y * PA_T) << sh, oy1 = min(((blockIdx.y + 1) * PA_T) << sh, H[k + 1]);
    uint8_t* __restrict__ dst = const_cast<uint8_t*>(jobs[(size_t) (k + 1) * job_pitch + blockIdx.z].img.get());
    for(int i = tid; i < dny * dnx; i += 256) {
      const int r = i / dnx, c = i - r * dnx;
      const int y = ylo[k + 1] + r, x = xlo[k + 1] + c, y2 = 2 * y;
      const uint16_t* col = s_h + c - ylo[k] * E1;
      const unsigned b0 = col[reflect101(y2 - 2, H[k]) * E1], b1 = col[reflect101(y2 - 1, H[k]) * E1], b2 = col[y2 * E1],
                     b3 = col[reflect101(y2 + 1, H[k]) * E1], b4 = col[reflect101(y2 + 2, H[k]) * E1];
      const uint8_t v = (uint8_t) ((b0 + 4u * b1 + 6u * b2 + 4u * b3 + b4 + 128u) >> 8);
      nxt[r * pn + c] = v;
      if(x >= ox0 && x < ox1 && y >= oy0 && y < oy1) dst[(size_t) y * W[k + 1] + x] = v;
    }
    __syncthreads();
    { uint8_t* t = cur; cur = nxt; nxt = t; }
    { const int t = pc; pc = pn; pn = t; }
  }
}
void launch_pyramid_levels(hipStream_t s, const FrameJob* src_row, int job_pitch, int steps, int dW, int dR, int nframes)
{
  const dim3 grid((dW + PA_T - 1) / PA_T, (dR + PA_T - 1) / PA_T, nframes);
  if(steps == 3) hipLaunchKernelGGL(pyramid_levels_kernel<3>, grid, dim3(256), 0, s, src_row, job_pitch);
  else if(steps == 2) hipLaunchKernelGGL(pyramid_levels_kernel<2>, grid, dim3(256), 0, s, src_row, job_pitch);
  else hipLaunchKernelGGL(pyramid_levels_kernel<1>, grid, dim3(256), 0, s, src_row, job_pitch);
}

__global__ __launch_bounds__(256) void intensity_kernel(const FrameJob* jobs, int nframes, int job_pitch)
{
  const FrameJob& j = level_job(jobs, blockIdx.z, nframes, job_pitch);
  const int n = j.rows * j.cols;
  const int i = (blockIdx.x * 256 + threadIdx.x) * 4;
  if(i >= n) return;
  if(i + 3 < n && ((uintptr_t) (j.img + i) & 3) == 0) {
    const uchar4 v = *reinterpret_cast<const uchar4*>(j.img + i);
    *reinterpret_cast<float4*>(j.desc + i) = make_float4((float) v.x, (float) v.y, (float) v.z, (float) v.w);
  } else {
    for(int k = i; k < n && k < i + 4; ++k) j.desc[k] = (float) j.img[k];
  }
}

constexpr int ROWS_PER_THREAD = 4;
constexpr int CENSUS_ROWS = 8;
__global__ __launch_bounds__(256) void census_kernel(const FrameJob* jobs)
{
  const FrameJob& j = jobs[blockIdx.z];
  const int x = blockIdx.x * 64 + (threadIdx.x & 63);
  const int y0 = (blockIdx.y * 4 + (threadIdx.x >> 6)) * CENSUS_ROWS;
  const int W = j.cols, R = j.rows;
  if(x >= W || y0 >= R) return;
  const bool xin = x > 0 && x < W - 1;
  const int xm = max(x - 1, 0), xp = min(x + 1, W - 1);
  uint8_t w[CENSUS_ROWS + 2][3];
#pragma unroll
  for(int k = 0; k < CENSUS_ROWS + 2; ++k) {
    const uint8_t* p = j.img + (size_t) min(max(y0 - 1 + k, 0), R - 1) * W;
    w[k][0] = p[xm]; w[k][1] = p[x]; w[k][2] = p[xp];
  }
#pragma unroll
  for(int k = 0; k < CENSUS_ROWS; ++k) {
    const int y = y0 + k;
    if(y < R) {
      uint8_t out = 0;
      if(xin && y > 0 && y < R - 1) {
        const uint8_t ctr = w[k + 1][1];
        out = (uint8_t) (((w[k][0] >= ctr) << 0) | ((w[k][1] >= ctr) << 1) | ((w[k][2] >= ctr) << 2) | ((w[k + 1][0] >= ctr) << 3) |
                         ((w[k + 1][2] >= ctr) << 4) | ((w[k + 2][0] >= ctr) << 5) | ((w[k + 2][1] >= ctr) << 6) | ((w[k + 2][2] >= ctr) << 7));
      }
      j.cen[(size_t) y * W + x] = out;
    }
  }
}

constexpr int CB_TW = 64, CB_TH = 4;
__global__ __launch_bounds__(256) void census_blur_kernel(const FrameJob* jobs, int kc, int ks, int nframes, int job_pitch)
{
  __shared__ uint8_t s_src[(CB_TH + 4) * (CB_TW + 4)];
  __shared__ int s_tmp[(CB_TH + 4) * (CB_TW + 2)];
  __shared__ uint8_t s_b[(CB_TH + 2) * (CB_TW + 2)];
  const FrameJob& j = level_job(jobs, blockIdx.z, nframes, job_pitch);
  const int W = j.cols, R = j.rows;
  const int x0 = blockIdx.x * CB_TW, y0 = blockIdx.y * CB_TH;
  if(x0 >= W || y0 >= R) return;
  const int tid = threadIdx.x;
  for(int i = tid; i < (CB_TH + 4) * (CB_TW + 4); i += 256) {
    const int ly = i / (CB_TW + 4), lx = i - ly * (CB_TW + 4);
    const int gy = reflect101(min(y0 + ly - 2, R + 1), R), gx = reflect101(min(x0 + lx - 2, W + 1), W);
    s_src[i] = j.img[(size_t) gy * W + gx];
  }
  __syncthreads();
  for(int i = tid; i < (CB_TH + 4) * (CB_TW + 2); i += 256) {
    const int ly = i / (CB_TW + 2), lx = i - ly * (CB_TW + 2);
    const uint8_t* p = s_src + ly * (CB_TW + 4) + lx + 1;
    s_tmp[i] = (int) p[0] * kc + ((int) p[-1] + (int) p[1]) * ks;
  }
  __syncthreads();
  for(int i = tid; i < (CB_TH + 2) * (CB_TW + 2); i += 256) {
    const int ly = i / (CB_TW + 2), lx = i - ly * (CB_TW + 2);
    const int* t = s_tmp + (ly + 1) * (CB_TW + 2) + lx;
    const int v = (t[0] * kc + (t[-(CB_TW + 2)] + t[CB_TW + 2]) * ks + (1 << 15)) >> 16;
    s_b[i] = (uint8_t) min(255, max(0, v));
  }
  __syncthreads();
  const int lx = tid & 63, ly = tid >> 6;
  const int x = x0 + lx, y = y0 + ly;
  if(x >= W || y >= R) return;
  uint8_t out = 0;
  if(x > 0 && x < W - 1 && y > 0 && y < R - 1) {
    constexpr int P = CB_TW + 2;
    const uint8_t* p = s_b + (ly + 1) * P + lx + 1;
    const uint8_t c = p[0];
    out = (uint8_t) (((p[-P - 1] >= c) << 0) | ((p[-P] >= c) << 1) | ((p[-P + 1] >= c) << 2) | ((p[-1] >= c) << 3) |
                     ((p[1] >= c) << 4) | ((p[P - 1] >= c) << 5) | ((p[P] >= c) << 6) | ((p[P + 1] >= c) << 7));
  }
  j.cen[(size_t) y * W + x] = out;
}

#ifndef BP_TW_VALUE
#define BP_TW_VALUE 64
#define BP_TH_VALUE 8
#endif
constexpr int BP_TW = BP_TW_VALUE, BP_TH = BP_TH_VALUE, BP_HALO = 2;
constexpr int BP_PLANE = (BP_TH + 2 * BP_HALO) * BP_TW + 8;
__device__ __forceinline__ uint2 spread_planes(unsigned c)
{
  unsigned lo = c & 0xFu, hi = (c >> 4) & 0xFu;
  lo = (lo | (lo << 14)) & 0x00030003u; lo = (lo | (lo << 7)) & 0x01010101u;
  hi = (hi | (hi << 14)) & 0x00030003u; hi = (hi | (hi << 7)) & 0x01010101u;
  return make_uint2(lo, hi);
}

template <bool FROM_IMAGE>
__global__ __launch_bounds__(256) void bitplanes_blur_kernel(const FrameJob* jobs, float k0, float k1, float k2, int stack, int nframes, int job_pitch)
{
  constexpr int CR = BP_TH + 2 * BP_HALO, CC = BP_TW + 2 * BP_HALO;
  constexpr int CW = CC + 4;
  constexpr int IR = CR + 2, IC = CC + 2, IW = IC + 2;
  constexpr int NSRC = FROM_IMAGE ? IR * IC : CR * CC;
  constexpr int NPRE = (NSRC + 255) / 256;
  __shared__ uint2 s_cen[CR * CW];
  __shared__ uint8_t s_img[FROM_IMAGE ? IR * IW : 4];
  __shared__ float s_row[(BP_PLANE + CR * BP_TW) * 4];
  __shared__ float s_lut[18];
  const FrameJob& j = level_job(jobs, blockIdx.z, nframes, job_pitch);
  const int W = j.cols, R = j.rows;
  const int x0 = blockIdx.x * BP_TW;
  if(x0 >= W || (int) blockIdx.y * BP_TH * stack >= R) return;
  const int tid = threadIdx.x;
  const uint8_t* __restrict__ cen = FROM_IMAGE ? j.img : j.cen;
  float* __restrict__ const desc = j.desc;
  float* __restrict__ const ch0 = j.ch0;
  const bool lazy_level = FROM_IMAGE && j.lazy != 0;
  const bool lazy = lazy_level && x0 + BP_TW + 8 <= (W & ~3) && !(x0 == 0 && (W & 3) == 0);
  uint8_t* __restrict__ const cen_out = j.cen;
  if(tid < 18) {
    const float S0 = (float) (tid / 9), A = (float) (tid % 3), B = (float) ((tid / 3) % 3);
    s_lut[tid] = S0 * k0 + A * k1 + B * k2;
  }

  uint8_t pre[NPRE];
  auto prefetch = [&](int y0) {
#pragma unroll
    for(int k = 0; k < NPRE; ++k) {
      const int i = min(tid + k * 256, NSRC - 1);
      if constexpr(FROM_IMAGE) {
        const int ly = i / IC, lx = i - ly * IC;
        const int gy = min(max(y0 + ly - BP_HALO - 1, 0), R - 1), gx = min(max(x0 + lx - BP_HALO - 1, 0), W - 1);
        pre[k] = cen[(size_t) gy * W + gx];
      } else {
        const int ly = i / CC, lx = i - ly * CC;
        const int gy = reflect101(min(y0 + ly - BP_HALO, R + 1), R), gx = reflect101(min(x0 + lx - BP_HALO, W + 1), W);
        pre[k] = cen[(size_t) gy * W + gx];
      }
    }
  };
  auto stage = [&]() {
#pragma unroll
    for(int k = 0; k < NPRE; ++k) {
      const int i = tid + k * 256;
      if constexpr(FROM_IMAGE) {
        if(i < IR * IC) { const int ly = i / IC, lx = i - ly * IC; s_img[ly * IW + lx] = pre[k]; }
      } else {
        if(i < CR * CC) { const int ly = i / CC, lx = i - ly * CC; s_cen[ly * CW + lx] = spread_planes(pre[k]); }
      }
    }
  };
  const int ybase = blockIdx.y * BP_TH * stack;
  prefetch(ybase);
  stage();
  __syncthreads();
  for(int t = 0; t < stack; ++t) {
    const int y0 = ybase + t * BP_TH;
    if(y0 >= R) break;
    if constexpr(FROM_IMAGE) {
      for(int i = tid; i < CR * CC; i += 256) {
        const int ly = i / CC, lx = i - ly * CC;
        const int gy = reflect101(min(y0 + ly - BP_HALO, R + 1), R), gx = reflect101(min(x0 + lx - BP_HALO, W + 1), W);
        uint8_t out = 0;
        if(gx > 0 && gx < W - 1 && gy > 0 && gy < R - 1) {
          const uint8_t* p = s_img + (gy - (y0 - BP_HALO - 1)) * IW + (gx - (x0 - BP_HALO - 1));
          const uint8_t c = p[0];
          out = (uint8_t) (((p[-IW - 1] >= c) << 0) | ((p[-IW] >= c) << 1) | ((p[-IW + 1] >= c) << 2) | ((p[-1] >= c) << 3) |
                           ((p[1] >= c) << 4) | ((p[IW - 1] >= c) << 5) | ((p[IW] >= c) << 6) | ((p[IW + 1] >= c) << 7));
        }
        s_cen[ly * CW + lx] = spread_planes(out);
        if(lazy_level && ly >= BP_HALO && ly < BP_HALO + BP_TH && lx >= BP_HALO && lx < BP_HALO + BP_TW && y0 + ly - BP_HALO < R && x0 + lx - BP_HALO < W)
          cen_out[(size_t) (y0 + ly - BP_HALO) * W + (x0 + lx - BP_HALO)] = out;
      }
      __syncthreads();
    }
    const bool more = t + 1 < stack && y0 + BP_TH < R;
    if(more) prefetch(y0 + BP_TH);

    if(lazy) {
      for(int i = tid; i < CR * BP_TW; i += 256) {
        const int ly = i / BP_TW, lx = i - ly * BP_TW;
        const uint2* c = s_cen + ly * CW + lx;
        const unsigned ilo = (c[1].x + c[3].x) + 3u * (c[0].x + c[4].x) + 9u * c[2].x;
        s_row[i] = s_lut[ilo & 0xffu];
      }
      __syncthreads();
      if(more) stage();
      for(int i = tid; i < BP_TH * BP_TW; i += 256) {
        const int ly = i / BP_TW, lx = i - ly * BP_TW;
        const int gx = x0 + lx, gy = y0 + ly;
        if(gx >= W || gy >= R) continue;
        const float* Th = s_row + ly * BP_TW + lx;
        constexpr int pitch = BP_TW;
        float o = k0 * Th[2 * pitch]; o += k1 * (Th[3 * pitch] + Th[pitch]); o += k2 * (Th[4 * pitch] + Th[0]);
        ch0[(size_t) gy * W + gx] = o;
      }
      __syncthreads();
      continue;
    }
    for(int i = tid; i < CR * BP_TW; i += 256) {
      const int ly = i / BP_TW, lx = i - ly * BP_TW;
      const uint2* c = s_cen + ly * CW + lx;
      const uint2 cm2 = c[0], cm1 = c[1], c0 = c[2], cp1 = c[3], cp2 = c[4];
      const unsigned ilo = (cm1.x + cp1.x) + 3u * (cm2.x + cp2.x) + 9u * c0.x;
      const unsigned ihi = (cm1.y + cp1.y) + 3u * (cm2.y + cp2.y) + 9u * c0.y;
      float tt[8];
#pragma unroll
      for(int b = 0; b < 4; ++b) {
        tt[b] = s_lut[(ilo >> (8 * b)) & 0xffu];
        tt[4 + b] = s_lut[(ihi >> (8 * b)) & 0xffu];
      }
      float4* o = reinterpret_cast<float4*>(s_row);
      o[i] = make_float4(tt[0], tt[1], tt[2], tt[3]);
      o[BP_PLANE + i] = make_float4(tt[4], tt[5], tt[6], tt[7]);
    }
    __syncthreads();
    if(more) stage();

    for(int u = tid; u < 2 * BP_TH * BP_TW; u += 256) {
      const int i = u >> 1, h = u & 1;
      const int ly = i / BP_TW, lx = i - ly * BP_TW;
      const int gx = x0 + lx, gy = y0 + ly;
      if(gx >= W || gy >= R) continue;
      const float4* Th = reinterpret_cast<const float4*>(s_row) + h * BP_PLANE + ly * BP_TW + lx;
      constexpr int pitch = BP_TW;
      const float4 Tm2 = Th[0], Tm1 = Th[pitch], T0 = Th[2 * pitch], Tp1 = Th[3 * pitch], Tp2 = Th[4 * pitch];
      float4 o4;
      o4.x = k0 * T0.x; o4.x += k1 * (Tp1.x + Tm1.x); o4.x += k2 * (Tp2.x + Tm2.x);
      o4.y = k0 * T0.y; o4.y += k1 * (Tp1.y + Tm1.y); o4.y += k2 * (Tp2.y + Tm2.y);
      o4.z = k0 * T0.z; o4.z += k1 * (Tp1.z + Tm1.z); o4.z += k2 * (Tp2.z + Tm2.z);
      o4.w = k0 * T0.w; o4.w += k1 * (Tp1.w + Tm1.w); o4.w += k2 * (Tp2.w + Tm2.w);
      store_stream(reinterpret_cast<float4*>(desc + ((size_t) gy * W + gx) * 8) + h, o4);
      if(h == 0 && ch0) ch0[(size_t) gy * W + gx] = o4.x;
    }
    __syncthreads();
  }
}

__global__ __launch_bounds__(256) void bitplanes_noblur_kernel(const FrameJob* jobs)
{
  const FrameJob& j = jobs[blockIdx.z];
  const int n = j.rows * j.cols;
  const int i = blockIdx.x * 256 + threadIdx.x;
  if(i >= n) return;
  const unsigned c = j.cen[i];
  float4* d = reinterpret_cast<float4*>(j.desc + (size_t) i * 8);
  if(j.ch0) j.ch0[i] = (float) (c & 1u);
  d[0] = make_float4((float) (c & 1u), (float) ((c >> 1) & 1u), (float) ((c >> 2) & 1u), (float) ((c >> 3) & 1u));
  d[1] = make_float4((float) ((c >> 4) & 1u), (float) ((c >> 5) & 1u), (float) ((c >> 6) & 1u), (float) ((c >> 7) & 1u));
}

template <int C>
__device__ __forceinline__ float grad_abs(const float* __restrict__ I, size_t p, int W, int c)
{
  const float Ix = fabsf(I[(p - 1) * C + c] - I[(p + 1) * C + c]);
  const float Iy = fabsf(I[(p - W) * C + c] - I[(p + W) * C + c]);
  return Ix + Iy;
}
template <int C>
__device__ __forceinline__ float grad_tail(const float* __restrict__ I, size_t p, int W, int c)
{
  return fabsf(I[(p + 1) * C + c] - I[(p - 1) * C + c]) + fabsf(I[(p + W) * C + c] + I[(p - W) * C + c]);
}

template <int C>
__global__ __launch_bounds__(256) void saliency_kernel(const FrameJob* jobs)
{
  const FrameJob& j = jobs[blockIdx.z];
  const int W = j.cols, R = j.rows;
  const int x = blockIdx.x * 64 + (threadIdx.x & 63);
  const int y0 = (blockIdx.y * 4 + (threadIdx.x >> 6)) * ROWS_PER_THREAD;
  if(x >= W || y0 >= R) return;
  const float* __restrict__ I = j.desc;
  const int n = W & ~3;
#pragma unroll
  for(int k = 0; k < ROWS_PER_THREAD; ++k) {
    const int y = min(y0 + k, R - 1);
    float S = 0.0f;
    if(y >= 1 && y <= R - 2 && x != W - 1) {
      const size_t row = (size_t) y * W;
      if(x >= n) {
        S = grad_tail<C>(I, row + x, W, 0);
        for(int c = 1; c < C; ++c) S += grad_tail<C>(I, row + x, W, c);
      } else if(C == 1) {
        S = grad_abs<C>(I, row + x, W, 0);
      } else if(x >= 4) {
        if(C == 8 && j.ch0) S = grad_abs<1>(j.ch0, row + x, W, 0);
        else S = grad_abs<C>(I, row + x, W, 0);
      } else {
        const int xs = n - 4 + x;
        const float S0 = (xs == W - 1) ? 0.0f : grad_abs<C>(I, row + xs, W, 0);
        S = S0 + grad_abs<C>(I, row + xs, W, C - 1);
      }
    }
    j.sal[(size_t) y * W + x] = S;
  }
}

__device__ __forceinline__ bool is_local_max(const float* __restrict__ S, int W, int radius, int y, int x)
{
  if(radius <= 0) return true;
  const float* p = S + (size_t) y * W + x;
  const float v = p[0];
  if(radius == 1) {
    float a[4], b[4], c[4];
#pragma unroll
    for(int k = 0; k < 4; ++k) { a[k] = p[k - 1 - W]; b[k] = p[k - 1]; c[k] = p[k - 1 + W]; }
    bool ok = true;
#pragma unroll
    for(int k = 0; k < 4; ++k) {
      if(k != 1) ok = ok & (v > b[k]);
      ok = ok & (v > a[k]) & (v > c[k]);
    }
    return ok;
  }
  for(int r = -radius; r <= radius; ++r)
    for(int c = -radius; c <= radius; ++c)
      if(!(r == 0 && c == 0) && p[r * W + c] >= v) return false;
  return true;
}

#ifndef SEL_PX_VALUE
#define SEL_PX_VALUE 4
#endif
constexpr int SEL_PX = SEL_PX_VALUE;
constexpr int SEL_BLOCK_PX = 256 * SEL_PX;
constexpr int SEL_GROUP = 256 / SEL_PX;
__global__ __launch_bounds__(256) void select_flag_kernel(const FrameJob* jobs, int border)
{
  const FrameJob& j = jobs[blockIdx.z];
  const float min_saliency = j.min_saliency, min_disp = j.min_disp, max_disp = j.max_disp;
  const int W = j.cols, R = j.rows;
  const int npix = W * R;
  const int p0 = blockIdx.x * SEL_BLOCK_PX + threadIdx.x * SEL_PX;
  const float* __restrict__ S = j.sal;
  bool f[SEL_PX];
#pragma unroll
  for(int e = 0; e < SEL_PX; ++e) f[e] = false;
  if(p0 < npix) {
    const int y0 = p0 / W, x0 = p0 - y0 * W;
    const bool one_row = x0 + SEL_PX <= W && p0 + SEL_PX <= npix;
    const bool inner = one_row && j.nms_radius == 1 && y0 >= border && y0 < R - border - 1 && x0 >= border && x0 + SEL_PX - 1 < W - border - 1;
    if(inner) {
      float a[SEL_PX + 3], b[SEL_PX + 3], c[SEL_PX + 3];
      const float* q = S + (size_t) y0 * W + x0 - 1;
#pragma unroll
      for(int k = 0; k < SEL_PX + 3; ++k) { a[k] = q[k - W]; b[k] = q[k]; c[k] = q[k + W]; }
#pragma unroll
      for(int e = 0; e < SEL_PX; ++e) {
        const float v = b[e + 1];
        bool ok = v >= min_saliency;
#pragma unroll
        for(int k = 0; k < 4; ++k) {
          if(k != 1) ok = ok & (v > b[e + k]);
          ok = ok & (v > a[e + k]) & (v > c[e + k]);
        }
        f[e] = ok;
      }
    } else {
#pragma unroll
      for(int e = 0; e < SEL_PX; ++e) {
        const int p = p0 + e;
        if(p < npix) {
          const int y = p / W, x = p - y * W;
          if(y >= border && y < R - border - 1 && x >= border && x < W - border - 1)
            f[e] = S[p] >= min_saliency && is_local_max(S, W, j.nms_radius, y, x);
        }
      }
    }
#pragma unroll
    for(int e = 0; e < SEL_PX; ++e) {
      if(!f[e]) continue;
      const int p = p0 + e;
      const int y = p / W, x = p - y * W;
      const float d = j.disp[(size_t) (1 << j.level) * ((size_t) y * j.disp_cols + x)];
      f[e] = (d >= min_disp && d <= max_disp);
    }
    if(p0 + SEL_PX <= npix) {
#pragma unroll
      for(int e = 0; e < SEL_PX; e += 4)
        *reinterpret_cast<uchar4*>(j.flag + p0 + e) = make_uchar4(f[e], f[e + 1], f[e + 2], f[e + 3]);
    } else {
      for(int e = 0; e < SEL_PX && p0 + e < npix; ++e) j.flag[p0 + e] = f[e] ? 1 : 0;
    }
  }
  int cnt = 0;
#pragma unroll
  for(int e = 0; e < SEL_PX; ++e) cnt += (int) f[e];
#pragma unroll
  for(int o = SEL_GROUP / 2; o >= 1; o >>= 1) cnt += __shfl_xor(cnt, o);
  const int chunk = p0 / 256;
  if((threadIdx.x & (SEL_GROUP - 1)) == 0 && chunk * 256 < npix) j.blk_count[chunk] = cnt;
}

__global__ __launch_bounds__(1024) void select_scan_kernel(const FrameJob* jobs)
{
  const FrameJob& j = jobs[blockIdx.x];
  const int nblk = (j.rows * j.cols + 255) / 256;
  __shared__ int s_wave[16];
  __shared__ int s_carry;
  if(threadIdx.x == 0) s_carry = 0;
  __syncthreads();
  const int lane = threadIdx.x & 63, wave = threadIdx.x >> 6;
  for(int base = 0; base < nblk; base += 1024) {
    const int i = base + threadIdx.x;
    const int v = (i < nblk) ? j.blk_count[i] : 0;
    int incl = v;
#pragma unroll
    for(int o = 1; o < 64; o <<= 1) {
      const int t = __shfl_up(incl, o);
      if(lane >= o) incl += t;
    }
    if(lane == 63) s_wave[wave] = incl;
    __syncthreads();
    int woff = 0;
    for(int w = 0; w < wave; ++w) woff += s_wave[w];
    const int carry = s_carry;
    if(i < nblk) j.blk_count[i] = carry + woff + incl - v;
    __syncthreads();
    if(threadIdx.x == 1023) s_carry = carry + woff + incl;
    __syncthreads();
  }
  if(threadIdx.x == 0) {
    int total = s_carry;
    if(total > j.cap) total = j.cap;
    *j.n_out = total & ~15;
  }
}

__global__ __launch_bounds__(256) void select_write_kernel(const FrameJob* jobs)
{
  const FrameJob& j = jobs[blockIdx.z];
  const int W = j.cols;
  const int npix = W * j.rows;
  const int p0 = blockIdx.x * SEL_BLOCK_PX + threadIdx.x * SEL_PX;
  const int wave_p0 = blockIdx.x * SEL_BLOCK_PX + (threadIdx.x & ~63) * SEL_PX;
  if(wave_p0 >= npix) return;
  const int chunk = p0 / 256;
  unsigned char fe[SEL_PX];
#pragma unroll
  for(int e = 0; e < SEL_PX; ++e) fe[e] = 0;
  if(p0 + SEL_PX <= npix) {
#pragma unroll
    for(int e = 0; e < SEL_PX; e += 4) {
      const uchar4 v = *reinterpret_cast<const uchar4*>(j.flag + p0 + e);
      fe[e] = v.x; fe[e + 1] = v.y; fe[e + 2] = v.z; fe[e + 3] = v.w;
    }
  } else {
    for(int e = 0; e < SEL_PX && p0 + e < npix; ++e) fe[e] = j.flag[p0 + e];
  }
  int mine = 0;
#pragma unroll
  for(int e = 0; e < SEL_PX; ++e) mine += (int) fe[e];
  const int gl = threadIdx.x & (SEL_GROUP - 1);
  int incl = mine;
#pragma unroll
  for(int o = 1; o < SEL_GROUP; o <<= 1) {
    const int t = __shfl_up(incl, o);
    if(gl >= o) incl += t;
  }
  if(!mine) return;
  int rank = j.blk_count[chunk] + incl - mine;
  const int N = *j.n_out;
  const float fx = j.K[0], fy = j.K[4], cx = j.K[2], cy = j.K[5];
  const float Bf = j.b * fx;
#pragma unroll
  for(int e = 0; e < SEL_PX; ++e) {
    if(!fe[e]) continue;
    const int r = rank++;
    if(r >= N) break;
    const int p = p0 + e;
    const int y = p / W, x = p - y * W;
    const float d = j.disp[(size_t) (1 << j.level) * ((size_t) y * j.disp_cols + x)];
    const float Z = (float) ((double) Bf * (1.0 / (double) d));
    const float X = ((float) x - cx) * Z * (1.0f / fx);
    const float Y = ((float) y - cy) * Z * (1.0f / fy);
    j.pts[r] = j.dspace ? make_float4((float) x - cx, (float) y - cy, d, 1.0f) : make_float4(X, Y, Z, 1.0f);
    j.ptc[r] = compact_point(j.dspace ? d : Z, x, y);
    j.inds[r] = p;
  }
}

constexpr int ST_W = 64, ST_H = 32, ST_ROWS_PER_WAVE = ST_H / 4;
constexpr int ST_CH_ROWS = ST_H + 4, ST_CH_COLS = ST_W + 5, ST_CH_PITCH = 72;
constexpr int ST_S_ROWS = ST_H + 2, ST_S_COLS = ST_W + 3, ST_S_PITCH = 68;

template <int C>
__device__ __forceinline__ float saliency_generic(const FrameJob& j, int x, int y)
{
  const int W = j.cols, R = j.rows, n = W & ~3;
  if(!(y >= 1 && y <= R - 2 && x != W - 1)) return 0.0f;
  const float* __restrict__ I = j.desc;
  const size_t row = (size_t) y * W;
  if(x >= n) {
    float S = grad_tail<C>(I, row + x, W, 0);
    for(int c = 1; c < C; ++c) S += grad_tail<C>(I, row + x, W, c);
    return S;
  }
  if(C == 1 || x >= 4) return grad_abs<C>(I, row + x, W, 0);
  const int xs = n - 4 + x;
  const float S0 = (xs == W - 1) ? 0.0f : grad_abs<C>(I, row + xs, W, 0);
  return S0 + grad_abs<C>(I, row + xs, W, C - 1);
}

template <int C>
__global__ __launch_bounds__(256) void saliency_select_tile_kernel(const FrameJob* jobs, int border, int nframes, int job_pitch)
{
  __shared__ float s_ch[ST_CH_ROWS][ST_CH_PITCH];
  __shared__ float s_sal[ST_S_ROWS][ST_S_PITCH];
  const FrameJob& j = level_job(jobs, blockIdx.z, nframes, job_pitch);
  const int W = j.cols, R = j.rows, n = W & ~3;
  const int x0 = blockIdx.x * ST_W, y0 = blockIdx.y * ST_H;
  if(x0 >= W || y0 >= R) return;
  const int lane = threadIdx.x & 63, wave = threadIdx.x >> 6;
  const bool compact = C == 8 && j.ch0;
  const float* __restrict__ ch = compact ? j.ch0.get() : j.desc.get();
  const int CS = compact ? 1 : C;
  for(int i = threadIdx.x; i < ST_CH_ROWS * ST_CH_PITCH; i += 256) {
    const int r = i / ST_CH_PITCH, cc = i - r * ST_CH_PITCH;
    if(cc < ST_CH_COLS) {
      const int y = min(max(y0 - 2 + r, 0), R - 1), xx = min(max(x0 - 2 + cc, 0), W - 1);
      s_ch[r][cc] = ch[((size_t) y * W + xx) * CS];
    }
  }
  __syncthreads();
  for(int i = threadIdx.x; i < ST_S_ROWS * ST_S_PITCH; i += 256) {
    const int r = i / ST_S_PITCH, cc = i - r * ST_S_PITCH;
    if(cc >= ST_S_COLS) continue;
    const int y = y0 - 1 + r, xx = x0 - 1 + cc;
    float S = fabsf(s_ch[r + 1][cc] - s_ch[r + 1][cc + 2]) + fabsf(s_ch[r][cc + 1] - s_ch[r + 2][cc + 1]);
    const bool inside = xx >= 0 && xx < W && y >= 0 && y < R;
    if(!(xx >= 4 && xx < n && xx != W - 1 && y >= 1 && y <= R - 2)) S = (inside && (xx < 4 || xx >= n)) ? saliency_generic<C>(j, xx, y) : 0.0f;
    s_sal[r][cc] = S;
  }
  __syncthreads();
  const int x = x0 + lane, c = lane + 1;
  const int radius = j.nms_radius;
  const bool col_ok = x >= border && x < W - border - 1;
  const int ry0 = wave * ST_ROWS_PER_WAVE;
  float vrow[ST_ROWS_PER_WAVE + 2], side[ST_ROWS_PER_WAVE + 2], full[ST_ROWS_PER_WAVE + 2];
#pragma unroll
  for(int q = 0; q < ST_ROWS_PER_WAVE + 2; ++q) {
    const float* t = &s_sal[ry0 + q][c - 1];
    vrow[q] = t[1];
    side[q] = fmaxf(fmaxf(t[0], t[2]), t[3]);
    full[q] = fmaxf(side[q], t[1]);
  }
  bool ok[ST_ROWS_PER_WAVE];
  const float min_saliency = j.min_saliency;
#pragma unroll
  for(int q = 0; q < ST_ROWS_PER_WAVE; ++q) {
    const int y = y0 + ry0 + q;
    const float v = vrow[q + 1];
    bool t = col_ok && y >= border && y < R - border - 1 && v >= min_saliency;
    if(radius == 1) t = t & (v > fmaxf(fmaxf(full[q], side[q + 1]), full[q + 2]));
    ok[q] = t;
  }
  float dv[ST_ROWS_PER_WAVE];
#pragma unroll
  for(int q = 0; q < ST_ROWS_PER_WAVE; ++q)
    dv[q] = ok[q] ? j.disp[(size_t) (1 << j.level) * ((size_t) (y0 + ry0 + q) * j.disp_cols + x)] : 0.0f;
  unsigned long long words = 0;
  const float min_disp = j.min_disp, max_disp = j.max_disp;
#pragma unroll
  for(int q = 0; q < ST_ROWS_PER_WAVE; ++q) {
    const unsigned long long m = __ballot(ok[q] && dv[q] >= min_disp && dv[q] <= max_disp);
    if(lane == q) words = m;
  }
  const int y = y0 + ry0 + lane;
  if(lane < ST_ROWS_PER_WAVE && y < R) j.words[(size_t) y * ((W + 63) / 64) + blockIdx.x] = words;
  if(x < W) {
    float* __restrict__ sal_out = j.sal;
#pragma unroll
    for(int q = 0; q < ST_ROWS_PER_WAVE; ++q) {
      const int yy = y0 + ry0 + q;
      if(yy < R) sal_out[(size_t) yy * W + x] = vrow[q + 1];
    }
  }
}

__global__ __launch_bounds__(1024) void select_words_scan_kernel(const FrameJob* jobs, int nframes, int job_pitch)
{
  const FrameJob& j = level_job(jobs, blockIdx.x, nframes, job_pitch);
  const int nw = j.rows * ((j.cols + 63) / 64);
  __shared__ int s_wave[16];
  __shared__ int s_carry;
  if(threadIdx.x == 0) s_carry = 0;
  __syncthreads();
  const int lane = threadIdx.x & 63, wave = threadIdx.x >> 6;
  for(int base = 0; base < nw; base += 1024) {
    const int i = base + threadIdx.x;
    const int v = (i < nw) ? __popcll(j.words[i]) : 0;
    int incl = v;
#pragma unroll
    for(int o = 1; o < 64; o <<= 1) {
      const int t = __shfl_up(incl, o);
      if(lane >= o) incl += t;
    }
    if(lane == 63) s_wave[wave] = incl;
    __syncthreads();
    int woff = 0;
    for(int w = 0; w < wave; ++w) woff += s_wave[w];
    const int carry = s_carry;
    if(i < nw) j.blk_count[i] = carry + woff + incl - v;
    __syncthreads();
    if(threadIdx.x == 1023) s_carry = carry + woff + incl;
    __syncthreads();
  }
  if(threadIdx.x == 0) {
    int total = s_carry;
    if(total > j.cap) total = j.cap;
    *j.n_out = total & ~15;
  }
}

constexpr int SW_WORDS = 8;
__device__ __forceinline__ int nth_set_bit(unsigned long long m, int n)
{
  int pos = 0;
#pragma unroll
  for(int w = 32; w >= 1; w >>= 1) {
    const int cnt = __popcll(m & ((1ull << w) - 1ull));
    if(n >= cnt) { n -= cnt; m >>= w; pos += w; }
  }
  return pos;
}
__global__ __launch_bounds__(256) void select_words_write_kernel(const FrameJob* jobs, int nframes, int job_pitch)
{
  const FrameJob& j = level_job(jobs, blockIdx.z, nframes, job_pitch);
  const int W = j.cols, WPR = (W + 63) / 64;
  const int nw = j.rows * WPR;
  const int lane = threadIdx.x & 63;
  const int w0 = (blockIdx.x * 4 + (threadIdx.x >> 6)) * SW_WORDS;
  if(w0 >= nw) return;
  unsigned long long m[SW_WORDS];
  int before[SW_WORDS + 1];
  before[0] = 0;
#pragma unroll
  for(int k = 0; k < SW_WORDS; ++k) {
    m[k] = (w0 + k < nw) ? j.words[w0 + k] : 0ull;
    before[k + 1] = before[k] + __popcll(m[k]);
  }
  const int total = before[SW_WORDS];
  if(total == 0) return;
  const int off = j.blk_count[w0];
  const int N = *j.n_out;
  const float fx = j.K[0], fy = j.K[4], cx = j.K[2], cy = j.K[5];
  const float Bf = j.b * fx;
  int px[SW_WORDS], py[SW_WORDS];
  float dd[SW_WORDS];
#pragma unroll
  for(int it = 0; it < SW_WORDS; ++it) {
    const int t = lane + 64 * it;
    px[it] = -1; py[it] = 0; dd[it] = 1.0f;
    if(t < total && off + t < N) {
      int k = 0;
      unsigned long long mk = m[0];
      int first = 0;
#pragma unroll
      for(int q = 1; q < SW_WORDS; ++q)
        if(t >= before[q]) { k = q; mk = m[q]; first = before[q]; }
      const int bit = nth_set_bit(mk, t - first);
      const int w = w0 + k;
      py[it] = w / WPR; px[it] = (w - py[it] * WPR) * 64 + bit;
      dd[it] = j.disp[(size_t) (1 << j.level) * ((size_t) py[it] * j.disp_cols + px[it])];
    }
  }
#pragma unroll
  for(int it = 0; it < SW_WORDS; ++it) {
    if(px[it] < 0) continue;
    const int r = off + lane + 64 * it, x = px[it], y = py[it];
    const float d = dd[it];
    const float Z = (float) ((double) Bf * (1.0 / (double) d));
    const float X = ((float) x - cx) * Z * (1.0f / fx);
    const float Y = ((float) y - cy) * Z * (1.0f / fy);
    j.pts[r] = j.dspace ? make_float4((float) x - cx, (float) y - cy, d, 1.0f) : make_float4(X, Y, Z, 1.0f);
    j.ptc[r] = compact_point(j.dspace ? d : Z, x, y);
    j.inds[r] = y * W + x;
  }
}

#ifndef NRM_DPP_ASM
#if defined(__gfx950__) || !defined(__HIP_DEVICE_COMPILE__)
#define NRM_DPP_ASM 1
#else
#define NRM_DPP_ASM 0
#endif
#endif
#define NRM_ROW_(I) \
  "v_add_f32_dpp %0, %1, %0 row_shl:" #I " row_mask:0xf bank_mask:0xf bound_ctrl:0\n" \
  "v_add_f32_dpp %0, %2, %0 row_shl:" #I " row_mask:0xf bank_mask:0xf bound_ctrl:0\n" \
  "v_add_f32_dpp %0, %3, %0 row_shl:" #I " row_mask:0xf bank_mask:0xf bound_ctrl:0\n" \
  "v_add_f32_dpp %0, %4, %0 row_shl:" #I " row_mask:0xf bank_mask:0xf bound_ctrl:0\n"
template <int I>
__device__ __forceinline__ float nrm_row_lane(float v)
{
  if constexpr(I == 0) return v;
  else return __int_as_float(__builtin_amdgcn_update_dpp(0, __float_as_int(v), 0x100 + I , 0xf, 0xf, true));
}
template <int I>
__device__ __forceinline__ void nrm_add_row_c(float& acc, const float (&v)[4])
{
  if constexpr(I < 16) {
#pragma unroll
    for(int q = 0; q < 4; ++q) acc += nrm_row_lane<I>(v[q]);
    nrm_add_row_c<I + 1>(acc, v);
  }
}
template <bool ASM>
__device__ __forceinline__ void nrm_add_batch(float& acc, const float (&v)[4])
{
#if NRM_DPP_ASM
  if constexpr(ASM) {
  asm volatile("v_add_f32 %0, %0, %1\n v_add_f32 %0, %0, %2\n v_add_f32 %0, %0, %3\n v_add_f32 %0, %0, %4\n"
               NRM_ROW_(1) NRM_ROW_(2) NRM_ROW_(3) NRM_ROW_(4) NRM_ROW_(5) NRM_ROW_(6) NRM_ROW_(7) NRM_ROW_(8)
               NRM_ROW_(9) NRM_ROW_(10) NRM_ROW_(11) NRM_ROW_(12) NRM_ROW_(13) NRM_ROW_(14) NRM_ROW_(15)
               : "+v"(acc) : "v"(v[0]), "v"(v[1]), "v"(v[2]), "v"(v[3]));
  return;
  }
#endif
  nrm_add_row_c<0>(acc, v);
}
constexpr int NRM_THREADS = 256, NRM_CHUNK = 512;
template <int FORM>
__device__ __forceinline__ void nrm_chain_b128(float& acc, const float4* __restrict__ sp, int n4)
// ... 65 lines not shown
  const int wt = tid - W0;
  auto mine = [&](int q) { return wt >= 0 && q * NW + wt < NRM_CHUNK; };
  const int nchunks = (N + NRM_CHUNK - 1) / NRM_CHUNK;
  const int row = (tid >> 4) & 3, li = tid & 15;
  float4 pre[PER];
  auto fetch = [&](int chunk) {
    const int base = chunk * NRM_CHUNK;
#pragma unroll
    for(int q = 0; q < PER; ++q) {
      const int k = base + q * NW + wt;
      pre[q] = (mine(q) && k < N) ? j.pts[k] : make_float4(0.0f, 0.0f, 0.0f, 0.0f);
    }
  };
  fetch(0);
#pragma unroll
  for(int q = 0; q < PER; ++q) if(mine(q)) stage(0, q * NW + wt, pre[q]);
  __syncthreads();
  float c = 0.0f;
  float4 pa[PER], pb[PER];
  auto fetch_to = [&](int chunk, float4 (&dst)[PER]) {
    const int base = chunk * NRM_CHUNK;
#pragma unroll
    for(int q = 0; q < PER; ++q) {
      const int k = base + q * NW + wt;
      dst[q] = (mine(q) && k < N) ? j.pts[k] : make_float4(0.0f, 0.0f, 0.0f, 0.0f);
    }
  };
  auto chunk_cnt = [&](int chunk) { return min(NRM_CHUNK, N - chunk * NRM_CHUNK); };
  if constexpr(FORM == 3) {
    auto stage_from = [&](int buf, const float4 (&src)[PER]) {
#pragma unroll
      for(int q = 0; q < PER; ++q) if(mine(q)) stage(buf, q * NW + wt, src[q]);
    };
    fetch_to(1, pa);
    for(int ch = 0; ch < nchunks; ch += 2) {
      fetch_to(ch + 2, pb);
      if(tid < 64) nrm_chain_asm(c, reinterpret_cast<const float4*>(s_comp[0][row]), chunk_cnt(ch));
      if(ch + 1 < nchunks) stage_from(1, pa);
      __syncthreads();
      if(ch + 1 >= nchunks) break;
      fetch_to(ch + 3, pa);
      if(tid < 64) nrm_chain_asm(c, reinterpret_cast<const float4*>(s_comp[1][row]), chunk_cnt(ch + 1));
      if(ch + 2 < nchunks) stage_from(0, pb);
      __syncthreads();
    }
  }
  for(int ch = 0; ch < nchunks && FORM != 3; ++ch) {
    const int cur = ch & 1;
    const int cnt = min(NRM_CHUNK, N - ch * NRM_CHUNK);
    if(ch + 1 < nchunks) fetch(ch + 1);
    if constexpr(FORM == 2) {
      if(tid < 64) nrm_chain_b128<FORM>(c, reinterpret_cast<const float4*>(s_comp[cur][row]), cnt / 4);
    } else if(tid < 64) {
      const float* sp = reinterpret_cast<const float*>(s_pts[cur]) + row + 16 * li;
      float v[4], nx[4] = {0.0f, 0.0f, 0.0f, 0.0f};
#pragma unroll
      for(int q = 0; q < 4; ++q) v[q] = sp[4 * q];
      __builtin_amdgcn_s_waitcnt(0xc07f);
      for(int b = 0; b < cnt; b += 64) {
        if(b + 64 < cnt) {
#pragma unroll
          for(int q = 0; q < 4; ++q) nx[q] = sp[4 * (b + 64 + q)];
        }
        nrm_add_batch<ASM>(c, v);
#pragma unroll
        for(int q = 0; q < 4; ++q) v[q] = nx[q];
      }
    }
    if(ch + 1 < nchunks) {
#pragma unroll
      for(int q = 0; q < PER; ++q) if(mine(q)) stage(cur ^ 1, q * NW + wt, pre[q]);
    }
    __syncthreads();
  }
  const float fN = (float) N;
  if(tid < 64 && li == 0) s_c[row] = c / fN;
  __syncthreads();
  const float c0 = s_c[0], c1 = s_c[1], c2 = s_c[2], c3 = s_c[3];
  float dpre[PER];
  auto dists = [&](int chunk) {
    const int base = chunk * NRM_CHUNK;
#pragma unroll
    for(int q = 0; q < PER; ++q) {
      const int k = base + q * NW + wt;
      const bool in = mine(q) && k < N;
      const float4 p = in ? j.pts[k] : make_float4(0.0f, 0.0f, 0.0f, 0.0f);
      const float d0 = p.x - c0, d1 = p.y - c1, d2 = p.z - c2, d3 = p.w - c3;
      dpre[q] = in ? sqrtf((d0 * d0 + d1 * d1) + (d2 * d2 + d3 * d3)) : 0.0f;
    }
  };
  dists(0);
#pragma unroll
  for(int q = 0; q < PER; ++q) if(mine(q)) s_dist[0][q * NW + wt] = dpre[q];
  __syncthreads();
  float m = 0.0f;
  if constexpr(FORM == 3) {
    auto dist_store = [&](int buf, const float4 (&src)[PER], int chunk) {
      const int base = chunk * NRM_CHUNK;
#pragma unroll
      for(int q = 0; q < PER; ++q) {
        if(!mine(q)) continue;
        const float4 p = src[q];
        const float d0 = p.x - c0, d1 = p.y - c1, d2 = p.z - c2, d3 = p.w - c3;
        s_dist[buf][q * NW + wt] = (base + q * NW + wt < N) ? sqrtf((d0 * d0 + d1 * d1) + (d2 * d2 + d3 * d3)) : 0.0f;
      }
    };
    fetch_to(1, pa);
    for(int ch = 0; ch < nchunks; ch += 2) {
      fetch_to(ch + 2, pb);
      if(tid < 64) nrm_chain_asm(m, reinterpret_cast<const float4*>(s_dist[0]), chunk_cnt(ch));
      if(ch + 1 < nchunks) dist_store(1, pa, ch + 1);
      __syncthreads();
      if(ch + 1 >= nchunks) break;
      fetch_to(ch + 3, pa);
      if(tid < 64) nrm_chain_asm(m, reinterpret_cast<const float4*>(s_dist[1]), chunk_cnt(ch + 1));
      if(ch + 2 < nchunks) dist_store(0, pb, ch + 2);
      __syncthreads();
    }
  }
  for(int ch = 0; ch < nchunks && FORM != 3; ++ch) {
    const int cur = ch & 1;
    const int cnt = min(NRM_CHUNK, N - ch * NRM_CHUNK);
    if(ch + 1 < nchunks) dists(ch + 1);
    if constexpr(FORM == 2) {
      if(tid < 64) nrm_chain_b128<FORM>(m, reinterpret_cast<const float4*>(s_dist[cur]), cnt / 4);
    } else if(tid < 64) {
      float4 d4 = *reinterpret_cast<const float4*>(&s_dist[cur][4 * li]), n4 = make_float4(0.0f, 0.0f, 0.0f, 0.0f);
      __builtin_amdgcn_s_waitcnt(0xc07f);
      for(int b = 0; b < cnt; b += 64) {
        if(b + 64 < cnt) n4 = *reinterpret_cast<const float4*>(&s_dist[cur][b + 64 + 4 * li]);
        const float v[4] = {d4.x, d4.y, d4.z, d4.w};
        nrm_add_batch<ASM>(m, v);
        d4 = n4;
      }
    }
    if(ch + 1 < nchunks) {
#pragma unroll
      for(int q = 0; q < PER; ++q) if(mine(q)) s_dist[cur ^ 1][q * NW + wt] = dpre[q];
    }
    __syncthreads();
  }
  if(tid == 0) {
    m /= fN;
    const float s = (float) (sqrt(3.0) / (double) fmaxf(m, 1e-6f));
    j.nrm[0] = s; j.nrm[1] = c0; j.nrm[2] = c1; j.nrm[3] = c2;
  }
}

__device__ __forceinline__ void bp_row_from_census(const uint8_t* __restrict__ cen, int W, int R, int px, int r, const float* __restrict__ lut, float (&T)[8])
{
  const uint8_t* row = cen + (size_t) reflect101(r, R) * W;
  const uint2 cm2 = spread_planes(row[reflect101(px - 2, W)]), cm1 = spread_planes(row[reflect101(px - 1, W)]), c0 = spread_planes(row[reflect101(px, W)]),
              cp1 = spread_planes(row[reflect101(px + 1, W)]), cp2 = spread_planes(row[reflect101(px + 2, W)]);
  const unsigned ilo = (cm1.x + cp1.x) + 3u * (cm2.x + cp2.x) + 9u * c0.x;
  const unsigned ihi = (cm1.y + cp1.y) + 3u * (cm2.y + cp2.y) + 9u * c0.y;
#pragma unroll
  for(int b = 0; b < 4; ++b) {
    T[b] = lut[(ilo >> (8 * b)) & 0xffu];
    T[4 + b] = lut[(ihi >> (8 * b)) & 0xffu];
  }
}
__device__ __forceinline__ void bp_col_pass(const float (&Tm2)[8], const float (&Tm1)[8], const float (&T0)[8], const float (&Tp1)[8], const float (&Tp2)[8],
                                            float k0, float k1, float k2, float (&out)[8])
{
#pragma unroll
  for(int c = 0; c < 8; ++c) {
    float o = k0 * T0[c];
    o += k1 * (Tp1[c] + Tm1[c]);
    o += k2 * (Tp2[c] + Tm2[c]);
    out[c] = o;
  }
}

template <int C>
__global__ __launch_bounds__(256) void template_build_kernel(const FrameJob* jobs, int grad_cd5, float k0, float k1, float k2, int nframes, int job_pitch)
{
  const FrameJob& j = level_job(jobs, blockIdx.z, nframes, job_pitch);
  __shared__ float s_lut[18];
  if(C == 8 && j.lazy) {
    if(threadIdx.x < 18) {
      const float S0 = (float) (threadIdx.x / 9), A = (float) (threadIdx.x % 3), B = (float) ((threadIdx.x / 3) % 3);
      s_lut[threadIdx.x] = S0 * k0 + A * k1 + B * k2;
    }
    __syncthreads();
  }
  const int N = *j.n_out;
  const int i = blockIdx.x * 256 + threadIdx.x;
  if(i >= N) return;
  const int W = j.cols;
  const int ii = j.inds[i];
  const float fx = j.dspace ? 1.0f : j.K[0], fy = j.dspace ? 1.0f : j.K[4];
  const float* __restrict__ D = j.desc;
  float pixv[C], Ix[C], Iy[C];
  const float NN = 1.0f / 18.0f;
  if constexpr(C == 8) {
    const float4* __restrict__ rec = reinterpret_cast<const float4*>(D) + (size_t) ii * 2;
    const ptrdiff_t rs = (ptrdiff_t) W * 2;
    auto load8 = [&](ptrdiff_t off, float (&v)[8]) {
      const float4 a = rec[off], b = rec[off + 1];
      v[0] = a.x; v[1] = a.y; v[2] = a.z; v[3] = a.w; v[4] = b.x; v[5] = b.y; v[6] = b.z; v[7] = b.w;
    };
    float xp[8], xm[8], yp[8], ym[8];
    if(j.lazy) {
      const int R = j.rows, x = ii % W, y = ii / W;
      const uint8_t* __restrict__ cen = j.cen;
      {
        float Tc[7][8];
#pragma unroll
        for(int r = 0; r < 7; ++r) bp_row_from_census(cen, W, R, x, y - 3 + r, s_lut, Tc[r]);
        bp_col_pass(Tc[0], Tc[1], Tc[2], Tc[3], Tc[4], k0, k1, k2, ym);
        bp_col_pass(Tc[1], Tc[2], Tc[3], Tc[4], Tc[5], k0, k1, k2, pixv);
        bp_col_pass(Tc[2], Tc[3], Tc[4], Tc[5], Tc[6], k0, k1, k2, yp);
      }
#pragma unroll
      for(int side = 0; side < 2; ++side) {
        float Ts[5][8];
#pragma unroll
        for(int r = 0; r < 5; ++r) bp_row_from_census(cen, W, R, x + (side ? 1 : -1), y - 2 + r, s_lut, Ts[r]);
        if(side) bp_col_pass(Ts[0], Ts[1], Ts[2], Ts[3], Ts[4], k0, k1, k2, xp);
        else bp_col_pass(Ts[0], Ts[1], Ts[2], Ts[3], Ts[4], k0, k1, k2, xm);
      }
    } else {
      load8(0, pixv);
      load8(2, xp); load8(-2, xm); load8(rs, yp); load8(-rs, ym);
    }
    if(!grad_cd5) {
#pragma unroll
      for(int c = 0; c < 8; ++c) {
        Ix[c] = fx * (0.5f * (xp[c] - xm[c]));
        Iy[c] = fy * (0.5f * (yp[c] - ym[c]));
      }
    } else {
      float xp2[8], xm2[8], yp2[8], ym2[8];
      load8(4, xp2); load8(-4, xm2); load8(2 * rs, yp2); load8(-2 * rs, ym2);
#pragma unroll
      for(int c = 0; c < 8; ++c) {
        Ix[c] = fx * (NN * (1.0f * xm2[c] - 8.0f * xm[c] + 8.0f * xp[c] - 1.0f * xp2[c]));
        Iy[c] = fy * (NN * (1.0f * ym2[c] - 8.0f * ym[c] + 8.0f * yp[c] - 1.0f * yp2[c]));
      }
    }
  } else {
#pragma unroll
    for(int c = 0; c < C; ++c) {
      const float* cc = D + (size_t) ii * C + c;
      float gx, gy;
      if(!grad_cd5) {
        gx = 0.5f * (cc[C] - cc[-C]);
        gy = 0.5f * (cc[(size_t) W * C] - cc[-(ptrdiff_t) W * C]);
      } else {
        gx = NN * (1.0f * cc[-2 * C] - 8.0f * cc[-C] + 8.0f * cc[C] - 1.0f * cc[2 * C]);
        gy = NN * (1.0f * cc[-2 * (ptrdiff_t) W * C] - 8.0f * cc[-(ptrdiff_t) W * C] + 8.0f * cc[(ptrdiff_t) W * C] - 1.0f * cc[2 * (ptrdiff_t) W * C]);
      }
      pixv[c] = cc[0];
      Ix[c] = fx * gx;
      Iy[c] = fy * gy;
    }
  }
  if constexpr(C == 8) {
    float4* pv = reinterpret_cast<float4*>(j.pix.get());
    store_stream(pv + tile_index<2>(i, 0), make_float4(pixv[0], pixv[1], pixv[2], pixv[3]));
    store_stream(pv + tile_index<2>(i, 1), make_float4(pixv[4], pixv[5], pixv[6], pixv[7]));
    float4* gv = reinterpret_cast<float4*>(j.grad.get());
    store_stream(gv + tile_index<4>(i, 0), make_float4(Ix[0], Ix[1], Ix[2], Ix[3]));
    store_stream(gv + tile_index<4>(i, 1), make_float4(Ix[4], Ix[5], Ix[6], Ix[7]));
    store_stream(gv + tile_index<4>(i, 2), make_float4(Iy[0], Iy[1], Iy[2], Iy[3]));
    store_stream(gv + tile_index<4>(i, 3), make_float4(Iy[4], Iy[5], Iy[6], Iy[7]));
  } else {
#pragma unroll
    for(int c = 0; c < C; ++c) {
      j.pix[(size_t) i * C + c] = pixv[c];
      j.grad[((size_t) i * 2 + 0) * C + c] = Ix[c];
      j.grad[((size_t) i * 2 + 1) * C + c] = Iy[c];
    }
  }
}

__global__ __launch_bounds__(256) void template_build_wide_kernel(const FrameJob* jobs, int C, int grad_cd5, int nframes, int job_pitch)
{
  const FrameJob& j = level_job(jobs, blockIdx.z, nframes, job_pitch);
  const int N = *j.n_out;
  const int i = blockIdx.x * 256 + threadIdx.x;
  if(i >= N) return;
  const int W = j.cols;
  const int ii = j.inds[i];
  const float fx = j.dspace ? 1.0f : j.K[0], fy = j.dspace ? 1.0f : j.K[4];
  const float* __restrict__ D = j.desc;
  const float NN = 1.0f / 18.0f;
  const ptrdiff_t sx = C, sy = (ptrdiff_t) W * C;
#pragma unroll 4
  for(int c = 0; c < C; ++c) {
    const float* cc = D + (size_t) ii * C + c;
    float gx, gy;
    if(!grad_cd5) {
      gx = 0.5f * (cc[sx] - cc[-sx]);
      gy = 0.5f * (cc[sy] - cc[-sy]);
    } else {
      gx = NN * (1.0f * cc[-2 * sx] - 8.0f * cc[-sx] + 8.0f * cc[sx] - 1.0f * cc[2 * sx]);
      gy = NN * (1.0f * cc[-2 * sy] - 8.0f * cc[-sy] + 8.0f * cc[sy] - 1.0f * cc[2 * sy]);
    }
    j.pix[(size_t) i * C + c] = cc[0];
    j.grad[((size_t) i * 2 + 0) * C + c] = fx * gx;
    j.grad[((size_t) i * 2 + 1) * C + c] = fy * gy;
  }
}

__global__ void gather_counts_kernel(const FrameJob* jobs, int job_pitch, int nframes, int first_level, int num_levels, int* out )
{
  const int t = blockIdx.x * blockDim.x + threadIdx.x;
  if(t >= nframes * kMaxLevels) return;
  const int i = t / kMaxLevels, l = t - i * kMaxLevels;
  out[t] = (l >= first_level && l < num_levels) ? *jobs[(size_t) l * job_pitch + i].n_out : 0;
}

template <int C>
__global__ __launch_bounds__(256) void export_jacobians_kernel(const FrameJob* job, float* out)
{
  const FrameJob& j = *job;
  const int N = *j.n_out;
  const int i = blockIdx.x * 256 + threadIdx.x;
  if(i >= N) return;
  const float4 P = j.pts[i];
  const JacPoint jp = jac_point(P.x, P.y, P.z, j.nrm);
  float Ix[C], Iy[C];
  if constexpr(C == 8) {
    const float4* gv = reinterpret_cast<const float4*>(j.grad.get());
    const float4 a = gv[tile_index<4>(i, 0)], b = gv[tile_index<4>(i, 1)], c = gv[tile_index<4>(i, 2)], d = gv[tile_index<4>(i, 3)];
    Ix[0] = a.x; Ix[1] = a.y; Ix[2] = a.z; Ix[3] = a.w; Ix[4] = b.x; Ix[5] = b.y; Ix[6] = b.z; Ix[7] = b.w;
    Iy[0] = c.x; Iy[1] = c.y; Iy[2] = c.z; Iy[3] = c.w; Iy[4] = d.x; Iy[5] = d.y; Iy[6] = d.z; Iy[7] = d.w;
  } else {
#pragma unroll
    for(int c = 0; c < C; ++c) { Ix[c] = j.grad[((size_t) i * 2 + 0) * C + c]; Iy[c] = j.grad[((size_t) i * 2 + 1) * C + c]; }
  }
#pragma unroll
  for(int c = 0; c < C; ++c) {
    float J[6];
    if(j.dspace) dspace_jac_row(P.x, P.y, P.z, j.K[0], j.K[4], 1.0f / j.K[0], 1.0f / j.K[4], 1.0f / j.b, Ix[c], Iy[c], J);
    else jac_row(jp, Ix[c], Iy[c], J);
    float* o = out + ((size_t) c * N + i) * 6;
#pragma unroll
    for(int k = 0; k < 6; ++k) o[k] = J[k];
  }
}

__global__ __launch_bounds__(256) void export_jacobians_wide_kernel(const FrameJob* job, int C, float* out)
{
  const FrameJob& j = *job;
  const int N = *j.n_out;
  const size_t k = (size_t) blockIdx.x * 256 + threadIdx.x;
  if(k >= (size_t) N * C) return;
  const int c = (int) (k / N), i = (int) (k - (size_t) c * N);
  const float4 P = j.pts[i];
  const float Ix = j.grad[((size_t) i * 2 + 0) * C + c], Iy = j.grad[((size_t) i * 2 + 1) * C + c];
  float J[6];
  if(j.dspace) dspace_jac_row(P.x, P.y, P.z, j.K[0], j.K[4], 1.0f / j.K[0], 1.0f / j.K[4], 1.0f / j.b, Ix, Iy, J);
  else jac_row(jac_point(P.x, P.y, P.z, j.nrm), Ix, Iy, J);
  float* o = out + k * 6;
#pragma unroll
  for(int q = 0; q < 6; ++q) o[q] = J[q];
}

static inline dim3 grid2d_rows(int W, int R, int nz) { return dim3((W + 63) / 64, (R + 4 * ROWS_PER_THREAD - 1) / (4 * ROWS_PER_THREAD), nz); }

void launch_ingest(hipStream_t s, const FrameJob* jobs_level0, const uint8_t* d_images, const float* d_disps, size_t npix, int nframes, int skip_odd_disp)
{
  const int blocks = (int) std::min<size_t>(256, (npix / 4 + 255) / 256);
  hipLaunchKernelGGL(ingest_kernel<false>, dim3(blocks, 1, nframes), dim3(256), 0, s, jobs_level0, d_images, d_disps, npix, skip_odd_disp, nullptr);
}
void launch_ingest_at(hipStream_t s, const FrameJob* jobs_level0, const uint8_t* d_images, const float* d_disps, const size_t* d_offsets, size_t npix, int nframes)
{
  const int blocks = (int) std::min<size_t>(256, (npix / 4 + 255) / 256);
  hipLaunchKernelGGL(ingest_kernel<true>, dim3(blocks, 1, nframes), dim3(256), 0, s, jobs_level0, d_images, d_disps, npix, 0, d_offsets);
}
void launch_pyrdown(hipStream_t s, const FrameJob* src, const FrameJob* dst, int dW, int dR, int nframes)
{
  hipLaunchKernelGGL(pyrdown_u8_lds_kernel, dim3((dW + PDT_W - 1) / PDT_W, (dR + PDT_H * PD_STACK - 1) / (PDT_H * PD_STACK), nframes), dim3(256), 0, s, src, dst);
}
void launch_intensity(hipStream_t s, const FrameJob* jobs, int W, int R, int nframes, int nlevels, int job_pitch)
{
  hipLaunchKernelGGL(intensity_kernel, dim3((W * R + 1023) / 1024, 1, nframes * nlevels), dim3(256), 0, s, jobs, nframes, job_pitch);
}
void launch_census(hipStream_t s, const FrameJob* jobs, int W, int R, int nframes, const int* blur_taps, int nlevels, int job_pitch)
{
  if(blur_taps)
    hipLaunchKernelGGL(census_blur_kernel, dim3((W + CB_TW - 1) / CB_TW, (R + CB_TH - 1) / CB_TH, nframes * nlevels), dim3(256), 0, s,
                       jobs, blur_taps[0], blur_taps[1], nframes, job_pitch);
  else
    hipLaunchKernelGGL(census_kernel, dim3((W + 63) / 64, (R + 4 * CENSUS_ROWS - 1) / (4 * CENSUS_ROWS), nframes), dim3(256), 0, s, jobs);
}
void launch_bitplanes(hipStream_t s, const FrameJob* jobs, int W, int R, int nframes, float sigma, const float k[3], int from_image, int nlevels,
                      int job_pitch)
{
  const int stack = nframes >= 16 ? 8 : (nframes > 4 ? 4 : 1);
  const dim3 grid((W + BP_TW - 1) / BP_TW, (R + BP_TH * stack - 1) / (BP_TH * stack), nframes * nlevels);
  if(sigma > 0.0f && from_image)
    hipLaunchKernelGGL(bitplanes_blur_kernel<true>, grid, dim3(256), 0, s, jobs, k[0], k[1], k[2], stack, nframes, job_pitch);
  else if(sigma > 0.0f)
    hipLaunchKernelGGL(bitplanes_blur_kernel<false>, grid, dim3(256), 0, s, jobs, k[0], k[1], k[2], stack, nframes, job_pitch);
  else
    hipLaunchKernelGGL(bitplanes_noblur_kernel, dim3((W * R + 255) / 256, 1, nframes), dim3(256), 0, s, jobs);
}
void launch_saliency_select(hipStream_t s, const FrameJob* jobs, int C, int W, int R, int nframes, int nms_radius, int border, int nlevels, int job_pitch)
{
  if(nms_radius <= 1) {
    const int WPR = (W + 63) / 64, nw = R * WPR;
    auto tile = [&](auto c) {
      hipLaunchKernelGGL(saliency_select_tile_kernel<decltype(c)::value>, dim3(WPR, (R + ST_H - 1) / ST_H, nframes * nlevels), dim3(256), 0, s, jobs,
                         border, nframes, job_pitch);
    };
    if(C <= 48 || !dispatch_wide_channels(C, tile)) dispatch_channels(C, tile);
    hipLaunchKernelGGL(select_words_scan_kernel, dim3(nframes * nlevels), dim3(1024), 0, s, jobs, nframes, job_pitch);
    hipLaunchKernelGGL(select_words_write_kernel, dim3((nw + 4 * SW_WORDS - 1) / (4 * SW_WORDS), 1, nframes * nlevels), dim3(256), 0, s, jobs, nframes,
                       job_pitch);
    return;
  }
  auto plain = [&](auto c) { hipLaunchKernelGGL(saliency_kernel<decltype(c)::value>, grid2d_rows(W, R, nframes), dim3(256), 0, s, jobs); };
  if(C <= 48 || !dispatch_wide_channels(C, plain)) dispatch_channels(C, plain);
  const int nblk = (W * R + SEL_BLOCK_PX - 1) / SEL_BLOCK_PX;
  hipLaunchKernelGGL(select_flag_kernel, dim3(nblk, 1, nframes), dim3(256), 0, s, jobs, border);
  hipLaunchKernelGGL(select_scan_kernel, dim3(nframes), dim3(1024), 0, s, jobs);
  hipLaunchKernelGGL(select_write_kernel, dim3(nblk, 1, nframes), dim3(256), 0, s, jobs);
}
__global__ __launch_bounds__(256) void copy_rows_kernel(unsigned long long* __restrict__ dst, const unsigned long long* __restrict__ src, size_t pitch8,
                                                        size_t width8, int rows)
{
  const size_t n = width8 * (size_t) rows;
  for(size_t i = (size_t) blockIdx.x * 256 + threadIdx.x; i < n; i += (size_t) gridDim.x * 256) {
    const size_t r = i / width8, k = i - r * width8;
    dst[r * pitch8 + k] = src[r * pitch8 + k];
  }
}
void launch_copy_rows(hipStream_t s, void* dst, const void* src_host_pinned, size_t pitch_bytes, size_t width_bytes, int rows)
{
  const size_t n = width_bytes / 8 * (size_t) rows;
  if(n == 0) return;
  hipLaunchKernelGGL(copy_rows_kernel, dim3((unsigned) std::min<size_t>(64, (n + 255) / 256)), dim3(256), 0, s, (unsigned long long*) dst,
                     (const unsigned long long*) src_host_pinned, pitch_bytes / 8, width_bytes / 8, rows);
}
void launch_normalization(hipStream_t s, const FrameJob* jobs, int job_pitch, int nframes, int first_level, int num_levels,
                          int with_normalization, int form)
{
  const dim3 grid(nframes, num_levels - first_level);
  if(form == 4) form = (nframes * (num_levels - first_level) <= 1024) ? 3 : 1;
  if(form == 3) hipLaunchKernelGGL(normalization_kernel<3>, grid, dim3(NRM_THREADS), 0, s, jobs, job_pitch, first_level, with_normalization);
  else if(form == 2) hipLaunchKernelGGL(normalization_kernel<2>, grid, dim3(NRM_THREADS), 0, s, jobs, job_pitch, first_level, with_normalization);
  else if(form == 1) hipLaunchKernelGGL(normalization_kernel<1>, grid, dim3(NRM_THREADS), 0, s, jobs, job_pitch, first_level, with_normalization);
  else hipLaunchKernelGGL(normalization_kernel<0>, grid, dim3(NRM_THREADS), 0, s, jobs, job_pitch, first_level, with_normalization);
}
void launch_gather_counts(hipStream_t s, const FrameJob* jobs, int job_pitch, int nframes, int first_level, int num_levels, int* out)
{
  hipLaunchKernelGGL(gather_counts_kernel, dim3((nframes * kMaxLevels + 255) / 256), dim3(256), 0, s, jobs, job_pitch, nframes, first_level,
                     num_levels, out);
}
void launch_template_build(hipStream_t s, const FrameJob* jobs, int C, int max_points, int nframes, int grad_cd5, const float gauss_k[3], int nlevels,
                           int job_pitch)
{
  if(max_points <= 0) return;
  const dim3 g((max_points + 255) / 256, 1, nframes * nlevels);
  if(C > 48) { hipLaunchKernelGGL(template_build_wide_kernel, g, dim3(256), 0, s, jobs, C, grad_cd5, nframes, job_pitch); return; }
  dispatch_channels(C, [&](auto c) {
    hipLaunchKernelGGL(template_build_kernel<decltype(c)::value>, g, dim3(256), 0, s, jobs, grad_cd5, gauss_k[0], gauss_k[1], gauss_k[2], nframes, job_pitch);
  });
}

void launch_export_jacobians(hipStream_t s, const FrameJob* job, int C, int n, float* out)
{
  if(n <= 0) return;
  const dim3 g((n + 255) / 256);
  if(C > 48) { hipLaunchKernelGGL(export_jacobians_wide_kernel, dim3((unsigned) (((size_t) n * C + 255) / 256)), dim3(256), 0, s, job, C, out); return; }
  dispatch_channels(C, [&](auto c) { hipLaunchKernelGGL(export_jacobians_kernel<decltype(c)::value>, g, dim3(256), 0, s, job, out); });
}

}
```

Baseline: 1.322 million GN iterations/s.

## Skip storing template descriptor and saliency on NMS-radius-1 levels; recompute from census

Adds a census-only lazy mode for template frames on levels with NMS radius 1. Those levels store only the census bytes, skip the dense descriptor and saliency map, and recompute saliency in the select tile kernel from the census via a LUT and Gaussian taps. A new census_templates kernel and a paired bitplanes launch split current and template frames. This removes descriptor writes for templates, and saliency is rebuilt on demand only if a caller asks for it.

```diff
diff --git a/bpvo_amd/csrc/context.hip b/bpvo_amd/csrc/context.hip
--- a/bpvo_amd/csrc/context.hip
+++ b/bpvo_amd/csrc/context.hip
@@ -103,10 +103,10 @@
   std::memset(&j, 0, sizeof(j));
   j.img = f.img[l];
   j.cen = f.cen[l];
-  j.ch0 = f.ch0_valid ? f.ch0[l] : nullptr;
+  j.ch0 = (f.ch0_valid && f.lazy[l] != 2) ? f.ch0[l] : nullptr;
   j.scratch = f.scratch;
   j.desc = f.desc[l];
-  j.sal = f.sal[l];
+  j.sal = f.sal_state[l] == FrameSlot::SAL_STORED ? f.sal[l] : nullptr;
   j.flag = f.flag[l];
   j.words = reinterpret_cast<unsigned long long*>(f.flag[l]);
   j.blk_count = f.blk_count[l];
@@ -124,7 +124,7 @@
   std::memcpy(j.K, g.K, sizeof(j.K));
   j.b = g.b;
   j.dspace = c->dspace;
-  j.lazy = f.lazy[l] ? 1 : 0;
+  j.lazy = f.lazy[l];
   const bpvo_hip_params& sp = f.seq_params ? *f.seq_params : c->params;
   j.min_saliency = sp.minSaliency; j.min_disp = sp.minValidDisparity; j.max_disp = sp.maxValidDisparity;
   return j;
@@ -322,6 +322,7 @@
                 return BPVO_OK;
               }},
     OPT_INT("lazy_template_descriptor", lazy_template, 0, 1),
+    OPT_INT("lazy_template_saliency", lazy_saliency, 0, 1),
     OPT_INT("points_from_compact_stream", points_from_compact, 0, 1),
     OptionDef{"tapcache_max_density", 0.0, 1e9, [](bpvo_hip_ctx* c) { return c->tapcache_max_density; },
               [](bpvo_hip_ctx* c, double v) { c->tapcache_max_density = v; return BPVO_OK; }},
diff --git a/bpvo_amd/csrc/frame_common.h b/bpvo_amd/csrc/frame_common.h
--- a/bpvo_amd/csrc/frame_common.h
+++ b/bpvo_amd/csrc/frame_common.h
@@ -18,6 +18,36 @@
   return p;
 }
 
+__device__ __forceinline__ uint2 spread_planes(unsigned c)
+{
+  unsigned lo = c & 0xFu, hi = (c >> 4) & 0xFu;
+  lo = (lo | (lo << 14)) & 0x00030003u; lo = (lo | (lo << 7)) & 0x01010101u;
+  hi = (hi | (hi << 14)) & 0x00030003u; hi = (hi | (hi << 7)) & 0x01010101u;
+  return make_uint2(lo, hi);
+}
+__device__ __forceinline__ unsigned bp_row_index(unsigned cm2, unsigned cm1, unsigned c0, unsigned cp1, unsigned cp2)
+{
+  return (cm1 + cp1) + 3u * (cm2 + cp2) + 9u * c0;
+}
+__device__ __forceinline__ float bp_row_entry(int e, float k0, float k1, float k2)
+{
+  const float S0 = (float) (e / 9), A = (float) (e % 3), B = (float) ((e / 3) % 3);
+  return S0 * k0 + A * k1 + B * k2;
+}
+__device__ __forceinline__ float bp_col(float Tm2, float Tm1, float T0, float Tp1, float Tp2, float k0, float k1, float k2)
+{
+  float o = k0 * T0;
+  o += k1 * (Tp1 + Tm1);
+  o += k2 * (Tp2 + Tm2);
+  return o;
+}
+__device__ __forceinline__ int bp_census_coord(int p, int len) { return reflect101(min(p, len + 1), len); }
+
+__host__ __device__ __forceinline__ bool bp_tile_column_is_lazy(int x0, int W)
+{
+  return x0 + 64 + 8 <= (W & ~3) && !(x0 == 0 && (W & 3) == 0);
+}
+
 static inline dim3 grid2d(int W, int R, int nz) { return dim3((W + 63) / 64, (R + 3) / 4, nz); }
 
 }
diff --git a/bpvo_amd/csrc/frames.hip b/bpvo_amd/csrc/frames.hip
--- a/bpvo_amd/csrc/frames.hip
+++ b/bpvo_amd/csrc/frames.hip
@@ -60,8 +60,17 @@
   for(int i = 0; i < count; ++i) c->frames[slots[i]].ch0_valid = !(skip_odd_disp && (i & 1));
   const bool lazy_ok = skip_odd_disp != 0 && c->lazy_template && c->params.descriptor == BPVO_DESC_BITPLANES && c->C == 8 &&
                        !(c->params.sigmaPriorToCensusTransform > 0.0f) && c->params.sigmaBitPlanes > 0.0f && c->params.gradientEstimation == BPVO_GRAD_CD3;
-  for(int i = 0; i < count; ++i)
-    for(int l = 0; l < c->L; ++l) c->frames[slots[i]].lazy[l] = lazy_ok && !(i & 1) && geom[l].nms_radius > 0;
+  const bool census_only_ok = lazy_ok && c->lazy_saliency;
+  bool census_only[kMaxLevels] = {};
+  bool any_census_only = false;
+  for(int l = c->params.maxTestLevel; l < c->L; ++l) any_census_only |= census_only[l] = census_only_ok && geom[l].nms_radius == 1;
+  for(int i = 0; i < count; ++i) {
+    FrameSlot& f = c->frames[slots[i]];
+    for(int l = 0; l < c->L; ++l) {
+      f.lazy[l] = (lazy_ok && !(i & 1) && geom[l].nms_radius > 0) ? (census_only[l] ? 2 : 1) : 0;
+      if(f.sal_state[l] == FrameSlot::SAL_ON_DEMAND) f.sal_state[l] = FrameSlot::SAL_GONE;
+    }
+  }
   const FrameJob* tab = nullptr;
   int rc = upload_frame_jobs_slots(c, slots, count, fr, 0, &tab);
   if(rc) return rc;
@@ -101,6 +110,7 @@
     const bool plain_intensity = c->C == 1 && c->params.descriptor != BPVO_DESC_LAPLACIAN;
     const bool one_launch = (fused_bp || smoothed_bp || plain_intensity) && count <= c->merge_levels_max_frames && c->L - l_lo > 1;
     if(one_launch && fused_bp) {
+      if(any_census_only) launch_census_templates(s, tab + (size_t) l_lo * NF, geom[l_lo].cols, geom[l_lo].rows, count, c->L - l_lo, NF);
       launch_bitplanes(s, tab + (size_t) l_lo * NF, geom[l_lo].cols, geom[l_lo].rows, count, c->params.sigmaBitPlanes, c->gauss_k, 1, c->L - l_lo, NF);
     } else if(one_launch && smoothed_bp) {
       launch_census(s, tab + (size_t) l_lo * NF, geom[l_lo].cols, geom[l_lo].rows, count, c->census_taps, c->L - l_lo, NF);
@@ -125,6 +135,11 @@
         else launch_intensity(s, jobs, g.cols, g.rows, count);
       } else {
         const bool fused_census = !(c->params.sigmaPriorToCensusTransform > 0.0f) && c->params.sigmaBitPlanes > 0.0f;
+        if(census_only[l]) {
+          launch_census_templates(s, jobs, g.cols, g.rows, count);
+          launch_bitplanes_pairs(s, jobs, g.cols, g.rows, count, c->gauss_k);
+          continue;
+        }
         if(!fused_census)
           launch_census(s, jobs, g.cols, g.rows, count, c->params.sigmaPriorToCensusTransform > 0.0f ? c->census_taps : nullptr);
         launch_bitplanes(s, jobs, g.cols, g.rows, count, c->params.sigmaBitPlanes, c->gauss_k, fused_census ? 1 : 0);
@@ -181,6 +196,10 @@
     FR_CK(c, fr, hipMalloc(&f.tmpl_slab, total));
     FR_CK(c, fr, hipMemsetAsync(f.tmpl_slab, 0, total, s));
     carve_frame_tmpl(c, f, (unsigned char*) f.tmpl_slab, nullptr);
+  }
+  for(int i = 0; i < count; ++i) {
+    FrameSlot& f = c->frames[slots[i]];
+    for(int l = 0; l < c->L; ++l) f.sal_state[l] = f.lazy[l] == 2 ? FrameSlot::SAL_ON_DEMAND : FrameSlot::SAL_STORED;
   }
   const FrameJob* tab = nullptr;
   int rc = upload_frame_jobs_slots(c, slots, count, fr, 1, &tab);
@@ -210,14 +229,14 @@
     for(int l = p.maxTestLevel; l < c->L; ++l) px += (double) geom[l].npix * count;
     ScopedTimer t(c, KC_SALIENCY_SELECT, px, fr.ln);
     const LevelGeom& g = geom[p.maxTestLevel];
-    launch_saliency_select(s, tab + (size_t) p.maxTestLevel * NF, c->C, g.cols, g.rows, count, 1, border,
+    launch_saliency_select(s, tab + (size_t) p.maxTestLevel * NF, c->C, g.cols, g.rows, count, 1, border, c->gauss_k,
                            c->L - p.maxTestLevel, NF);
   }
   for(int l = c->L - 1; l >= p.maxTestLevel && !one_launch; --l) {
     const FrameJob* jobs = tab + (size_t) l * NF;
     const LevelGeom& g = geom[l];
     ScopedTimer t(c, KC_SALIENCY_SELECT, (double) g.npix * count, fr.ln);
-    launch_saliency_select(s, jobs, c->C, g.cols, g.rows, count, g.nms_radius, border);
+    launch_saliency_select(s, jobs, c->C, g.cols, g.rows, count, g.nms_radius, border, c->gauss_k);
   }
   if(side) {
     FR_CK(c, fr, hipEventRecord(c->side_ev[0], s));
@@ -314,8 +333,8 @@
   bool any = false;
   for(int l = 0; l < c->L; ++l) any = any || f.lazy[l];
   if(!any) return BPVO_OK;
-  bool was[kMaxLevels];
-  for(int l = 0; l < c->L; ++l) { was[l] = f.lazy[l]; f.lazy[l] = false; }
+  uint8_t was[kMaxLevels];
+  for(int l = 0; l < c->L; ++l) { was[l] = f.lazy[l]; f.lazy[l] = 0; }
   auto restore = [&]() { for(int l = 0; l < c->L; ++l) f.lazy[l] = was[l]; };
   const FrameRun fr = ctx_run(c);
   const FrameJob* tab = nullptr;
@@ -330,6 +349,27 @@
   return BPVO_OK;
 }
 
+
+int ensure_saliency(bpvo_hip_ctx* c, int slot, int level)
+{
+  FrameSlot& f = c->frames[slot];
+  if(f.sal_state[level] == FrameSlot::SAL_STORED) return BPVO_OK;
+  if(f.sal_state[level] == FrameSlot::SAL_GONE)
+    return fail(c, BPVO_ERR_NO_DATA, "the saliency map of a pair batch's template frame is formed on demand from the frame's data, which has been replaced");
+  if(int rc = ensure_dense_descriptor(c, slot)) return rc;
+  f.sal_state[level] = FrameSlot::SAL_STORED;
+  const FrameRun fr = ctx_run(c);
+  const FrameJob* tab = nullptr;
+  int rc = upload_frame_jobs(c, slot, 1, 1, fr, 1, &tab);
+  if(rc == BPVO_OK) {
+    const LevelGeom& g = slot_geom(c, f, level);
+    launch_saliency(c->stream, tab + (size_t) level * c->n_frames, c->C, g.cols, g.rows, 1);
+    if(hipGetLastError() != hipSuccess || hipStreamSynchronize(c->stream) != hipSuccess) rc = fail(c, BPVO_ERR_DEVICE, "ensure_saliency: saliency kernel failed");
+  }
+  if(rc) f.sal_state[level] = FrameSlot::SAL_ON_DEMAND;
+  return rc;
+}
+
 }
 
 extern "C" {
@@ -420,6 +460,7 @@
   CHECK_CTX(c); CHECK_SLOT(c, slot); CHECK_LEVEL(c, level);
   if(!c->frames[slot].has_template) return fail(c, BPVO_ERR_NO_TEMPLATE, "no template");
   (void) hipSetDevice(c->device);
+  if(int rc = ensure_saliency(c, slot, level)) return rc;
   HIP_CK(c, hipMemcpyAsync(out, c->frames[slot].sal[level], c->geom[level].npix * sizeof(float), hipMemcpyDeviceToHost, c->stream));
   HIP_CK(c, hipStreamSynchronize(c->stream));
   return BPVO_OK;
diff --git a/bpvo_amd/csrc/host_ctx.h b/bpvo_amd/csrc/host_ctx.h
--- a/bpvo_amd/csrc/host_ctx.h
+++ b/bpvo_amd/csrc/host_ctx.h
@@ -50,7 +50,9 @@
   uint8_t* img[kMaxLevels] = {};
   uint8_t* cen[kMaxLevels] = {};
   float* ch0[kMaxLevels] = {};
-  bool lazy[kMaxLevels] = {};
+  uint8_t lazy[kMaxLevels] = {};
+  enum : uint8_t { SAL_STORED = 0, SAL_ON_DEMAND = 1, SAL_GONE = 2 };
+  uint8_t sal_state[kMaxLevels] = {};
   bool ch0_valid = true;
   float* desc[kMaxLevels] = {};
   float* disp = nullptr;
@@ -258,6 +260,7 @@
   double up_plan[2] = {0.19, 0.50};
   int points_from_compact = 0;
   int lazy_template = 1;
+  int lazy_saliency = 1;
   int keep_current_disparity = 0;
   double up_last_seconds = 0.0;
   size_t up_last_bytes = 0;
@@ -453,6 +456,7 @@
 int check_template_not_empty(bpvo_hip_ctx* c, int ref_slot);
 int ensure_lanes(bpvo_hip_ctx* c, int n);
 int lanes_for(bpvo_hip_ctx* c, int n, int cap);
+int ensure_saliency(bpvo_hip_ctx* c, int slot, int level);
 int ensure_dense_descriptor(bpvo_hip_ctx* c, int slot);
 int pose_cov_pass(bpvo_hip_ctx* c, int n_records, int members, const int* wss, const int* refs, const int* curs, const float* X, int level,
                   const float* T, const float* sigma, const bpvo_hip_params* const* prms, bpvo_hip_pose_covariance* out);
diff --git a/bpvo_amd/csrc/kernels.h b/bpvo_amd/csrc/kernels.h
--- a/bpvo_amd/csrc/kernels.h
+++ b/bpvo_amd/csrc/kernels.h
@@ -59,9 +59,13 @@
                   const GaussTaps& after);
 void launch_laplacian(hipStream_t s, const FrameJob* jobs, int W, int R, int nframes, int ksize );
 void launch_census(hipStream_t s, const FrameJob* jobs, int W, int R, int nframes, const int* blur_taps , int nlevels = 1, int job_pitch = 0);
+void launch_bitplanes_pairs(hipStream_t s, const FrameJob* jobs, int W, int R, int nframes, const float k[3]);
+void launch_census_templates(hipStream_t s, const FrameJob* jobs, int W, int R, int nframes, int nlevels = 1, int job_pitch = 0);
 void launch_bitplanes(hipStream_t s, const FrameJob* jobs, int W, int R, int nframes, float sigma, const float k[3], int from_image, int nlevels = 1,
                       int job_pitch = 0);
-void launch_saliency_select(hipStream_t s, const FrameJob* jobs, int C, int W, int R, int nframes, int nms_radius, int border, int nlevels = 1, int job_pitch = 0);
+void launch_saliency_select(hipStream_t s, const FrameJob* jobs, int C, int W, int R, int nframes, int nms_radius, int border, const float gauss_k[3], int nlevels = 1,
+                            int job_pitch = 0);
+void launch_saliency(hipStream_t s, const FrameJob* jobs, int C, int W, int R, int nframes);
 void launch_copy_rows(hipStream_t s, void* dst, const void* src_host_pinned, size_t pitch_bytes, size_t width_bytes, int rows);
 void launch_gather_counts(hipStream_t s, const FrameJob* jobs , int job_pitch, int nframes, int first_level, int num_levels,
                           int* out );
diff --git a/bpvo_amd/csrc/kernels_frame.hip b/bpvo_amd/csrc/kernels_frame.hip
--- a/bpvo_amd/csrc/kernels_frame.hip
+++ b/bpvo_amd/csrc/kernels_frame.hip
@@ -5,10 +5,10 @@
 
 namespace bpvo_hip {
 
-__device__ __forceinline__ const FrameJob& level_job(const FrameJob* jobs, unsigned z, int nframes, int job_pitch)
+__device__ __forceinline__ const FrameJob& level_job(const FrameJob* jobs, unsigned z, int nframes, int job_pitch, int job_step = 1)
 {
   const unsigned lvl = z / (unsigned) nframes;
-  return jobs[(size_t) lvl * job_pitch + (z - lvl * (unsigned) nframes)];
+  return jobs[(size_t) lvl * job_pitch + (size_t) (z - lvl * (unsigned) nframes) * job_step];
 }
 
 template <bool AT>
@@ -256,6 +256,56 @@
   }
 }
 
+typedef unsigned int u32_unaligned __attribute__((aligned(1)));
+typedef unsigned short u16_unaligned __attribute__((aligned(1)));
+constexpr int CT_ROWS = 8, CT_PX = 4;
+__global__ __launch_bounds__(256) void census_templates_kernel(const FrameJob* jobs, int nframes, int job_pitch)
+{
+  const FrameJob& j = level_job(jobs, blockIdx.z, nframes, job_pitch, 2);
+  if(j.lazy != 2) return;
+  const int W = j.cols, R = j.rows;
+  const int x = (blockIdx.x * 64 + (threadIdx.x & 63)) * CT_PX;
+  const int y0 = (blockIdx.y * 4 + (threadIdx.x >> 6)) * CT_ROWS;
+  if(x >= W || y0 >= R) return;
+  const uint8_t* __restrict__ img = j.img;
+  uint8_t* __restrict__ cen = j.cen;
+  const bool inner = x >= 1 && x + CT_PX < W;
+  unsigned long long w[CT_ROWS + 2];
+#pragma unroll
+  for(int k = 0; k < CT_ROWS + 2; ++k) {
+    const uint8_t* p = img + (size_t) min(max(y0 - 1 + k, 0), R - 1) * W;
+    if(inner) {
+      w[k] = (unsigned long long) *reinterpret_cast<const u32_unaligned*>(p + x - 1) |
+             ((unsigned long long) *reinterpret_cast<const u16_unaligned*>(p + x + 3) << 32);
+    } else {
+      unsigned long long v = 0;
+#pragma unroll
+      for(int q = 0; q < CT_PX + 2; ++q) v |= (unsigned long long) p[min(max(x - 1 + q, 0), W - 1)] << (8 * q);
+      w[k] = v;
+    }
+  }
+#pragma unroll
+  for(int k = 0; k < CT_ROWS; ++k) {
+    const int y = y0 + k;
+    if(y >= R) break;
+    const bool yin = y > 0 && y < R - 1;
+    unsigned out4 = 0;
+#pragma unroll
+    for(int q = 0; q < CT_PX; ++q) {
+      const unsigned a = (unsigned) (w[k] >> (8 * q)), b = (unsigned) (w[k + 1] >> (8 * q)), c = (unsigned) (w[k + 2] >> (8 * q));
+      const unsigned ctr = (b >> 8) & 0xffu;
+      unsigned out = (((a & 0xffu) >= ctr) << 0) | ((((a >> 8) & 0xffu) >= ctr) << 1) | ((((a >> 16) & 0xffu) >= ctr) << 2) | (((b & 0xffu) >= ctr) << 3) |
+                     ((((b >> 16) & 0xffu) >= ctr) << 4) | (((c & 0xffu) >= ctr) << 5) | ((((c >> 8) & 0xffu) >= ctr) << 6) | ((((c >> 16) & 0xffu) >= ctr) << 7);
+      if(!(yin && x + q > 0 && x + q < W - 1)) out = 0;
+      out4 |= out << (8 * q);
+    }
+    uint8_t* o = cen + (size_t) y * W + x;
+    if(x + CT_PX <= W) *reinterpret_cast<u32_unaligned*>(o) = out4;
+    else
+      for(int q = 0; q < W - x; ++q) o[q] = (uint8_t) (out4 >> (8 * q));
+  }
+}
+
 constexpr int CB_TW = 64, CB_TH = 4;
 __global__ __launch_bounds__(256) void census_blur_kernel(const FrameJob* jobs, int kc, int ks, int nframes, int job_pitch)
 {
@@ -306,16 +356,9 @@
 #endif
 constexpr int BP_TW = BP_TW_VALUE, BP_TH = BP_TH_VALUE, BP_HALO = 2;
 constexpr int BP_PLANE = (BP_TH + 2 * BP_HALO) * BP_TW + 8;
-__device__ __forceinline__ uint2 spread_planes(unsigned c)
-{
-  unsigned lo = c & 0xFu, hi = (c >> 4) & 0xFu;
-  lo = (lo | (lo << 14)) & 0x00030003u; lo = (lo | (lo << 7)) & 0x01010101u;
-  hi = (hi | (hi << 14)) & 0x00030003u; hi = (hi | (hi << 7)) & 0x01010101u;
-  return make_uint2(lo, hi);
-}
-
 template <bool FROM_IMAGE>
-__global__ __launch_bounds__(256) void bitplanes_blur_kernel(const FrameJob* jobs, float k0, float k1, float k2, int stack, int nframes, int job_pitch)
+__global__ __launch_bounds__(256) void bitplanes_blur_kernel(const FrameJob* jobs, float k0, float k1, float k2, int stack, int nframes, int job_pitch, int job_step,
+                                                             int dense_columns)
 {
   constexpr int CR = BP_TH + 2 * BP_HALO, CC = BP_TW + 2 * BP_HALO;
   constexpr int CW = CC + 4;
@@ -326,20 +369,23 @@
   __shared__ uint8_t s_img[FROM_IMAGE ? IR * IW : 4];
   __shared__ float s_row[(BP_PLANE + CR * BP_TW) * 4];
   __shared__ float s_lut[18];
-  const FrameJob& j = level_job(jobs, blockIdx.z, nframes, job_pitch);
+  const FrameJob& j = level_job(jobs, blockIdx.z, nframes, job_pitch, job_step);
   const int W = j.cols, R = j.rows;
-  const int x0 = blockIdx.x * BP_TW;
+  int bx = blockIdx.x;
+  if(dense_columns && !(bx == 0 && !bp_tile_column_is_lazy(0, W))) bx += (W + BP_TW - 1) / BP_TW - (int) gridDim.x;
+  const int x0 = bx * BP_TW;
   if(x0 >= W || (int) blockIdx.y * BP_TH * stack >= R) return;
   const int tid = threadIdx.x;
   const uint8_t* __restrict__ cen = FROM_IMAGE ? j.img : j.cen;
   float* __restrict__ const desc = j.desc;
   float* __restrict__ const ch0 = j.ch0;
-  const bool lazy_level = FROM_IMAGE && j.lazy != 0;
-  const bool lazy = lazy_level && x0 + BP_TW + 8 <= (W & ~3) && !(x0 == 0 && (W & 3) == 0);
+  static_assert(BP_TW == 64, "bp_tile_column_is_lazy speaks of 64-pixel tile columns");
+  const bool lazy = FROM_IMAGE && j.lazy != 0 && bp_tile_column_is_lazy(x0, W);
+  if(lazy && j.lazy == 2) return;
+  const bool lazy_level = FROM_IMAGE && j.lazy == 1;
   uint8_t* __restrict__ const cen_out = j.cen;
   if(tid < 18) {
-    const float S0 = (float) (tid / 9), A = (float) (tid % 3), B = (float) ((tid / 3) % 3);
-    s_lut[tid] = S0 * k0 + A * k1 + B * k2;
+    s_lut[tid] = bp_row_entry(tid, k0, k1, k2);
   }
 
   uint8_t pre[NPRE];
@@ -353,7 +399,7 @@
         pre[k] = cen[(size_t) gy * W + gx];
       } else {
         const int ly = i / CC, lx = i - ly * CC;
-        const int gy = reflect101(min(y0 + ly - BP_HALO, R + 1), R), gx = reflect101(min(x0 + lx - BP_HALO, W + 1), W);
+        const int gy = bp_census_coord(y0 + ly - BP_HALO, R), gx = bp_census_coord(x0 + lx - BP_HALO, W);
         pre[k] = cen[(size_t) gy * W + gx];
       }
     }
@@ -379,7 +425,7 @@
     if constexpr(FROM_IMAGE) {
       for(int i = tid; i < CR * CC; i += 256) {
         const int ly = i / CC, lx = i - ly * CC;
-        const int gy = reflect101(min(y0 + ly - BP_HALO, R + 1), R), gx = reflect101(min(x0 + lx - BP_HALO, W + 1), W);
+        const int gy = bp_census_coord(y0 + ly - BP_HALO, R), gx = bp_census_coord(x0 + lx - BP_HALO, W);
         uint8_t out = 0;
         if(gx > 0 && gx < W - 1 && gy > 0 && gy < R - 1) {
           const uint8_t* p = s_img + (gy - (y0 - BP_HALO - 1)) * IW + (gx - (x0 - BP_HALO - 1));
@@ -400,7 +446,7 @@
       for(int i = tid; i < CR * BP_TW; i += 256) {
         const int ly = i / BP_TW, lx = i - ly * BP_TW;
         const uint2* c = s_cen + ly * CW + lx;
-        const unsigned ilo = (c[1].x + c[3].x) + 3u * (c[0].x + c[4].x) + 9u * c[2].x;
+        const unsigned ilo = bp_row_index(c[0].x, c[1].x, c[2].x, c[3].x, c[4].x);
         s_row[i] = s_lut[ilo & 0xffu];
       }
       __syncthreads();
@@ -411,8 +457,7 @@
         if(gx >= W || gy >= R) continue;
         const float* Th = s_row + ly * BP_TW + lx;
         constexpr int pitch = BP_TW;
-        float o = k0 * Th[2 * pitch]; o += k1 * (Th[3 * pitch] + Th[pitch]); o += k2 * (Th[4 * pitch] + Th[0]);
-        ch0[(size_t) gy * W + gx] = o;
+        ch0[(size_t) gy * W + gx] = bp_col(Th[0], Th[pitch], Th[2 * pitch], Th[3 * pitch], Th[4 * pitch], k0, k1, k2);
       }
       __syncthreads();
       continue;
@@ -421,8 +466,8 @@
       const int ly = i / BP_TW, lx = i - ly * BP_TW;
       const uint2* c = s_cen + ly * CW + lx;
       const uint2 cm2 = c[0], cm1 = c[1], c0 = c[2], cp1 = c[3], cp2 = c[4];
-      const unsigned ilo = (cm1.x + cp1.x) + 3u * (cm2.x + cp2.x) + 9u * c0.x;
-      const unsigned ihi = (cm1.y + cp1.y) + 3u * (cm2.y + cp2.y) + 9u * c0.y;
+      const unsigned ilo = bp_row_index(cm2.x, cm1.x, c0.x, cp1.x, cp2.x);
+      const unsigned ihi = bp_row_index(cm2.y, cm1.y, c0.y, cp1.y, cp2.y);
       float tt[8];
 #pragma unroll
       for(int b = 0; b < 4; ++b) {
@@ -445,10 +490,10 @@
       constexpr int pitch = BP_TW;
       const float4 Tm2 = Th[0], Tm1 = Th[pitch], T0 = Th[2 * pitch], Tp1 = Th[3 * pitch], Tp2 = Th[4 * pitch];
       float4 o4;
-      o4.x = k0 * T0.x; o4.x += k1 * (Tp1.x + Tm1.x); o4.x += k2 * (Tp2.x + Tm2.x);
-      o4.y = k0 * T0.y; o4.y += k1 * (Tp1.y + Tm1.y); o4.y += k2 * (Tp2.y + Tm2.y);
-      o4.z = k0 * T0.z; o4.z += k1 * (Tp1.z + Tm1.z); o4.z += k2 * (Tp2.z + Tm2.z);
-      o4.w = k0 * T0.w; o4.w += k1 * (Tp1.w + Tm1.w); o4.w += k2 * (Tp2.w + Tm2.w);
+      o4.x = bp_col(Tm2.x, Tm1.x, T0.x, Tp1.x, Tp2.x, k0, k1, k2);
+      o4.y = bp_col(Tm2.y, Tm1.y, T0.y, Tp1.y, Tp2.y, k0, k1, k2);
+      o4.z = bp_col(Tm2.z, Tm1.z, T0.z, Tp1.z, Tp2.z, k0, k1, k2);
+      o4.w = bp_col(Tm2.w, Tm1.w, T0.w, Tp1.w, Tp2.w, k0, k1, k2);
       store_stream(reinterpret_cast<float4*>(desc + ((size_t) gy * W + gx) * 8) + h, o4);
       if(h == 0 && ch0) ch0[(size_t) gy * W + gx] = o4.x;
     }
@@ -704,12 +749,20 @@
 constexpr int ST_CH_ROWS = ST_H + 4, ST_CH_COLS = ST_W + 5, ST_CH_PITCH = 72;
 constexpr int ST_S_ROWS = ST_H + 2, ST_S_COLS = ST_W + 3, ST_S_PITCH = 68;
 
+constexpr int ST_CEN_ROWS = ST_CH_ROWS + 4, ST_CEN_PITCH = 76;
+static_assert(ST_CEN_PITCH >= ST_CH_COLS + 4, "a staged census row holds the window's columns and the halo");
+struct CensusStage {
+  uint8_t bit[ST_CEN_ROWS * ST_CEN_PITCH];
+  uint8_t idx[ST_CEN_ROWS * ST_CH_PITCH];
+  float lut[18];
+};
+static_assert(sizeof(CensusStage) <= sizeof(float) * ST_S_ROWS * ST_S_PITCH, "the census staging fits the saliency tile's storage");
+
 template <int C>
-__device__ __forceinline__ float saliency_generic(const FrameJob& j, int x, int y)
-{
-  const int W = j.cols, R = j.rows, n = W & ~3;
+__device__ __forceinline__ float saliency_generic(const float* __restrict__ I , int W, int R, int x, int y)
+{
+  const int n = W & ~3;
   if(!(y >= 1 && y <= R - 2 && x != W - 1)) return 0.0f;
-  const float* __restrict__ I = j.desc;
   const size_t row = (size_t) y * W;
   if(x >= n) {
     float S = grad_tail<C>(I, row + x, W, 0);
@@ -723,10 +776,11 @@
 }
 
 template <int C>
-__global__ __launch_bounds__(256) void saliency_select_tile_kernel(const FrameJob* jobs, int border, int nframes, int job_pitch)
+__global__ __launch_bounds__(256) void saliency_select_tile_kernel(const FrameJob* jobs, int border, int nframes, int job_pitch, float k0, float k1, float k2)
 {
   __shared__ float s_ch[ST_CH_ROWS][ST_CH_PITCH];
-  __shared__ float s_sal[ST_S_ROWS][ST_S_PITCH];
+  __shared__ union { float sal[ST_S_ROWS][ST_S_PITCH]; CensusStage cs; } s_u;
+  float (&s_sal)[ST_S_ROWS][ST_S_PITCH] = s_u.sal;
   const FrameJob& j = level_job(jobs, blockIdx.z, nframes, job_pitch);
   const int W = j.cols, R = j.rows, n = W & ~3;
   const int x0 = blockIdx.x * ST_W, y0 = blockIdx.y * ST_H;
@@ -735,11 +789,50 @@
   const bool compact = C == 8 && j.ch0;
   const float* __restrict__ ch = compact ? j.ch0.get() : j.desc.get();
   const int CS = compact ? 1 : C;
-  for(int i = threadIdx.x; i < ST_CH_ROWS * ST_CH_PITCH; i += 256) {
-    const int r = i / ST_CH_PITCH, cc = i - r * ST_CH_PITCH;
-    if(cc < ST_CH_COLS) {
-      const int y = min(max(y0 - 2 + r, 0), R - 1), xx = min(max(x0 - 2 + cc, 0), W - 1);
-      s_ch[r][cc] = ch[((size_t) y * W + xx) * CS];
+  const float* __restrict__ const recs = j.desc;
+  const float* __restrict__ const disp = j.disp;
+  const int radius = j.nms_radius, dstep = 1 << j.level, disp_cols = j.disp_cols;
+  const float min_saliency = j.min_saliency, min_disp = j.min_disp, max_disp = j.max_disp;
+  unsigned long long* __restrict__ const words_out = j.words;
+  float* __restrict__ const sal_out = j.sal;
+  if(C == 8 && j.lazy == 2) {
+    constexpr int NR = ST_CEN_ROWS, NP = ST_CEN_PITCH;
+    CensusStage& cs = s_u.cs;
+    if(threadIdx.x < 18) cs.lut[threadIdx.x] = bp_row_entry(threadIdx.x, k0, k1, k2);
+    const uint8_t* __restrict__ cen = j.cen;
+    constexpr int NPRE = (NR * NP + 255) / 256;
+    uint8_t pre[NPRE];
+#pragma unroll
+    for(int q = 0; q < NPRE; ++q) {
+      const int i = min((int) threadIdx.x + q * 256, NR * NP - 1);
+      const int r = i / NP, k = i - r * NP;
+      pre[q] = cen[(size_t) bp_census_coord(y0 - 4 + r, R) * W + bp_census_coord(x0 - 4 + k, W)];
+    }
+#pragma unroll
+    for(int q = 0; q < NPRE; ++q) {
+      const int i = threadIdx.x + q * 256;
+      if(i < NR * NP) cs.bit[i] = pre[q] & 1u;
+    }
+    __syncthreads();
+    for(int i = threadIdx.x; i < NR * ST_CH_PITCH; i += 256) {
+      const int r = i / ST_CH_PITCH, cc = i - r * ST_CH_PITCH;
+      const uint8_t* b = cs.bit + r * NP + cc;
+      if(cc < ST_CH_COLS) cs.idx[i] = (uint8_t) bp_row_index(b[0], b[1], b[2], b[3], b[4]);
+    }
+    __syncthreads();
+    for(int i = threadIdx.x; i < ST_CH_ROWS * ST_CH_PITCH; i += 256) {
+      const int r = i / ST_CH_PITCH, cc = i - r * ST_CH_PITCH;
+      const uint8_t* t = cs.idx + i;
+      if(cc < ST_CH_COLS)
+        s_ch[r][cc] = bp_col(cs.lut[t[0]], cs.lut[t[ST_CH_PITCH]], cs.lut[t[2 * ST_CH_PITCH]], cs.lut[t[3 * ST_CH_PITCH]], cs.lut[t[4 * ST_CH_PITCH]], k0, k1, k2);
+    }
+  } else {
+    for(int i = threadIdx.x; i < ST_CH_ROWS * ST_CH_PITCH; i += 256) {
+      const int r = i / ST_CH_PITCH, cc = i - r * ST_CH_PITCH;
+      if(cc < ST_CH_COLS) {
+        const int y = min(max(y0 - 2 + r, 0), R - 1), xx = min(max(x0 - 2 + cc, 0), W - 1);
+        s_ch[r][cc] = ch[((size_t) y * W + xx) * CS];
+      }
     }
   }
   __syncthreads();
@@ -749,12 +842,11 @@
     const int y = y0 - 1 + r, xx = x0 - 1 + cc;
     float S = fabsf(s_ch[r + 1][cc] - s_ch[r + 1][cc + 2]) + fabsf(s_ch[r][cc + 1] - s_ch[r + 2][cc + 1]);
     const bool inside = xx >= 0 && xx < W && y >= 0 && y < R;
-    if(!(xx >= 4 && xx < n && xx != W - 1 && y >= 1 && y <= R - 2)) S = (inside && (xx < 4 || xx >= n)) ? saliency_generic<C>(j, xx, y) : 0.0f;
+    if(!(xx >= 4 && xx < n && xx != W - 1 && y >= 1 && y <= R - 2)) S = (inside && (xx < 4 || xx >= n)) ? saliency_generic<C>(recs, W, R, xx, y) : 0.0f;
     s_sal[r][cc] = S;
   }
   __syncthreads();
   const int x = x0 + lane, c = lane + 1;
-  const int radius = j.nms_radius;
   const bool col_ok = x >= border && x < W - border - 1;
   const int ry0 = wave * ST_ROWS_PER_WAVE;
   float vrow[ST_ROWS_PER_WAVE + 2], side[ST_ROWS_PER_WAVE + 2], full[ST_ROWS_PER_WAVE + 2];
@@ -766,7 +858,6 @@
     full[q] = fmaxf(side[q], t[1]);
   }
   bool ok[ST_ROWS_PER_WAVE];
-  const float min_saliency = j.min_saliency;
 #pragma unroll
   for(int q = 0; q < ST_ROWS_PER_WAVE; ++q) {
     const int y = y0 + ry0 + q;
@@ -778,18 +869,16 @@
   float dv[ST_ROWS_PER_WAVE];
 #pragma unroll
   for(int q = 0; q < ST_ROWS_PER_WAVE; ++q)
-    dv[q] = ok[q] ? j.disp[(size_t) (1 << j.level) * ((size_t) (y0 + ry0 + q) * j.disp_cols + x)] : 0.0f;
+    dv[q] = ok[q] ? disp[(size_t) dstep * ((size_t) (y0 + ry0 + q) * disp_cols + x)] : 0.0f;
   unsigned long long words = 0;
-  const float min_disp = j.min_disp, max_disp = j.max_disp;
 #pragma unroll
   for(int q = 0; q < ST_ROWS_PER_WAVE; ++q) {
     const unsigned long long m = __ballot(ok[q] && dv[q] >= min_disp && dv[q] <= max_disp);
     if(lane == q) words = m;
   }
   const int y = y0 + ry0 + lane;
-  if(lane < ST_ROWS_PER_WAVE && y < R) j.words[(size_t) y * ((W + 63) / 64) + blockIdx.x] = words;
-  if(x < W) {
-    float* __restrict__ sal_out = j.sal;
+  if(lane < ST_ROWS_PER_WAVE && y < R) words_out[(size_t) y * ((W + 63) / 64) + blockIdx.x] = words;
+  if(x < W && sal_out) {
 #pragma unroll
     for(int q = 0; q < ST_ROWS_PER_WAVE; ++q) {
       const int yy = y0 + ry0 + q;
@@ -1161,8 +1250,8 @@
   const uint8_t* row = cen + (size_t) reflect101(r, R) * W;
   const uint2 cm2 = spread_planes(row[reflect101(px - 2, W)]), cm1 = spread_planes(row[reflect101(px - 1, W)]), c0 = spread_planes(row[reflect101(px, W)]),
               cp1 = spread_planes(row[reflect101(px + 1, W)]), cp2 = spread_planes(row[reflect101(px + 2, W)]);
-  const unsigned ilo = (cm1.x + cp1.x) + 3u * (cm2.x + cp2.x) + 9u * c0.x;
-  const unsigned ihi = (cm1.y + cp1.y) + 3u * (cm2.y + cp2.y) + 9u * c0.y;
+  const unsigned ilo = bp_row_index(cm2.x, cm1.x, c0.x, cp1.x, cp2.x);
+  const unsigned ihi = bp_row_index(cm2.y, cm1.y, c0.y, cp1.y, cp2.y);
 #pragma unroll
   for(int b = 0; b < 4; ++b) {
     T[b] = lut[(ilo >> (8 * b)) & 0xffu];
@@ -1173,12 +1262,7 @@
                                             float k0, float k1, float k2, float (&out)[8])
 {
 #pragma unroll
-  for(int c = 0; c < 8; ++c) {
-    float o = k0 * T0[c];
-    o += k1 * (Tp1[c] + Tm1[c]);
-    o += k2 * (Tp2[c] + Tm2[c]);
-    out[c] = o;
-  }
+  for(int c = 0; c < 8; ++c) out[c] = bp_col(Tm2[c], Tm1[c], T0[c], Tp1[c], Tp2[c], k0, k1, k2);
 }
 
 template <int C>
@@ -1187,10 +1271,7 @@
   const FrameJob& j = level_job(jobs, blockIdx.z, nframes, job_pitch);
   __shared__ float s_lut[18];
   if(C == 8 && j.lazy) {
-    if(threadIdx.x < 18) {
-      const float S0 = (float) (threadIdx.x / 9), A = (float) (threadIdx.x % 3), B = (float) ((threadIdx.x / 3) % 3);
-      s_lut[threadIdx.x] = S0 * k0 + A * k1 + B * k2;
-    }
+    if(threadIdx.x < 18) s_lut[threadIdx.x] = bp_row_entry(threadIdx.x, k0, k1, k2);
     __syncthreads();
   }
   const int N = *j.n_out;
@@ -1396,25 +1477,47 @@
   else
     hipLaunchKernelGGL(census_kernel, dim3((W + 63) / 64, (R + 4 * CENSUS_ROWS - 1) / (4 * CENSUS_ROWS), nframes), dim3(256), 0, s, jobs);
 }
+void launch_census_templates(hipStream_t s, const FrameJob* jobs, int W, int R, int nframes, int nlevels, int job_pitch)
+{
+  const int na = (nframes + 1) / 2;
+  hipLaunchKernelGGL(census_templates_kernel, dim3((W + 64 * CT_PX - 1) / (64 * CT_PX), (R + 4 * CT_ROWS - 1) / (4 * CT_ROWS), na * nlevels), dim3(256), 0, s, jobs, na,
+                     job_pitch);
+}
 void launch_bitplanes(hipStream_t s, const FrameJob* jobs, int W, int R, int nframes, float sigma, const float k[3], int from_image, int nlevels,
                       int job_pitch)
 {
   const int stack = nframes >= 16 ? 8 : (nframes > 4 ? 4 : 1);
   const dim3 grid((W + BP_TW - 1) / BP_TW, (R + BP_TH * stack - 1) / (BP_TH * stack), nframes * nlevels);
   if(sigma > 0.0f && from_image)
-    hipLaunchKernelGGL(bitplanes_blur_kernel<true>, grid, dim3(256), 0, s, jobs, k[0], k[1], k[2], stack, nframes, job_pitch);
+    hipLaunchKernelGGL(bitplanes_blur_kernel<true>, grid, dim3(256), 0, s, jobs, k[0], k[1], k[2], stack, nframes, job_pitch, 1, 0);
   else if(sigma > 0.0f)
-    hipLaunchKernelGGL(bitplanes_blur_kernel<false>, grid, dim3(256), 0, s, jobs, k[0], k[1], k[2], stack, nframes, job_pitch);
+    hipLaunchKernelGGL(bitplanes_blur_kernel<false>, grid, dim3(256), 0, s, jobs, k[0], k[1], k[2], stack, nframes, job_pitch, 1, 0);
   else
     hipLaunchKernelGGL(bitplanes_noblur_kernel, dim3((W * R + 255) / 256, 1, nframes), dim3(256), 0, s, jobs);
 }
-void launch_saliency_select(hipStream_t s, const FrameJob* jobs, int C, int W, int R, int nframes, int nms_radius, int border, int nlevels, int job_pitch)
+void launch_bitplanes_pairs(hipStream_t s, const FrameJob* jobs, int W, int R, int nframes, const float k[3])
+{
+  const int stack = nframes >= 16 ? 8 : (nframes > 4 ? 4 : 1);
+  const int ncols = (W + BP_TW - 1) / BP_TW, nrows = (R + BP_TH * stack - 1) / (BP_TH * stack);
+  int dense = 0;
+  for(int cx = 0; cx < ncols; ++cx) dense += bp_tile_column_is_lazy(cx * BP_TW, W) ? 0 : 1;
+  const int na = (nframes + 1) / 2, nb = nframes / 2;
+  if(nb > 0) hipLaunchKernelGGL(bitplanes_blur_kernel<true>, dim3(ncols, nrows, nb), dim3(256), 0, s, jobs + 1, k[0], k[1], k[2], stack, nb, 0, 2, 0);
+  if(dense > 0) hipLaunchKernelGGL(bitplanes_blur_kernel<true>, dim3(dense, nrows, na), dim3(256), 0, s, jobs, k[0], k[1], k[2], stack, na, 0, 2, 1);
+}
+void launch_saliency(hipStream_t s, const FrameJob* jobs, int C, int W, int R, int nframes)
+{
+  auto plain = [&](auto c) { hipLaunchKernelGGL(saliency_kernel<decltype(c)::value>, grid2d_rows(W, R, nframes), dim3(256), 0, s, jobs); };
+  if(C <= 48 || !dispatch_wide_channels(C, plain)) dispatch_channels(C, plain);
+}
+void launch_saliency_select(hipStream_t s, const FrameJob* jobs, int C, int W, int R, int nframes, int nms_radius, int border, const float gauss_k[3], int nlevels,
+                            int job_pitch)
 {
   if(nms_radius <= 1) {
     const int WPR = (W + 63) / 64, nw = R * WPR;
     auto tile = [&](auto c) {
       hipLaunchKernelGGL(saliency_select_tile_kernel<decltype(c)::value>, dim3(WPR, (R + ST_H - 1) / ST_H, nframes * nlevels), dim3(256), 0, s, jobs,
-                         border, nframes, job_pitch);
+                         border, nframes, job_pitch, gauss_k[0], gauss_k[1], gauss_k[2]);
     };
     if(C <= 48 || !dispatch_wide_channels(C, tile)) dispatch_channels(C, tile);
     hipLaunchKernelGGL(select_words_scan_kernel, dim3(nframes * nlevels), dim3(1024), 0, s, jobs, nframes, job_pitch);
@@ -1422,8 +1525,7 @@
                        job_pitch);
     return;
   }
-  auto plain = [&](auto c) { hipLaunchKernelGGL(saliency_kernel<decltype(c)::value>, grid2d_rows(W, R, nframes), dim3(256), 0, s, jobs); };
-  if(C <= 48 || !dispatch_wide_channels(C, plain)) dispatch_channels(C, plain);
+  launch_saliency(s, jobs, C, W, R, nframes);
   const int nblk = (W * R + SEL_BLOCK_PX - 1) / SEL_BLOCK_PX;
   hipLaunchKernelGGL(select_flag_kernel, dim3(nblk, 1, nframes), dim3(256), 0, s, jobs, border);
   hipLaunchKernelGGL(select_scan_kernel, dim3(nframes), dim3(1024), 0, s, jobs);
```

After: 1.347 million GN iterations/s, median of 6. 1.9% higher.
